# lab-oak/oak

Measured on AMD Instinct MI355X. Metric: turn-steps/s (batched playouts), higher is better.
Workload: dtype u16

## Files before the change

### include/oakgpu.h

```cpp
#ifndef OAKGPU_H
#define OAKGPU_H
#include <stddef.h>
#include <stdint.h>

#ifdef __cplusplus
extern "C" {
#endif

#define OAKGPU_BATTLE_SIZE 384
#define OAKGPU_DURATIONS_SIZE 8
#define OAKGPU_ACTIONS_SIZE 16
#define OAKGPU_MAX_CHOICES 9
#define OAKGPU_TEAMS_SIZE 60

typedef struct oakgpu_ctx oakgpu_ctx;
typedef struct oakgpu_net oakgpu_net;

int oakgpu_create(oakgpu_ctx **out, int device);
void oakgpu_destroy(oakgpu_ctx *ctx);
const char *oakgpu_last_error(void);
int oakgpu_set_stream(oakgpu_ctx *ctx, void *hip_stream);
void *oakgpu_get_stream(oakgpu_ctx *ctx);
int oakgpu_synchronize(oakgpu_ctx *ctx);
int oakgpu_set_kernel_timing(oakgpu_ctx *ctx, int on);
int oakgpu_get_leaf_kernel_ms(oakgpu_ctx *ctx, float ms[3]);
int oakgpu_set_playouts_per_lane(oakgpu_ctx *ctx, int k);
int oakgpu_set_regroup(oakgpu_ctx *ctx, int rounds, int suspend_below, int shrink);
int oakgpu_set_tail_pack(oakgpu_ctx *ctx, int below, int waves, int lanes);
int oakgpu_set_queue_order(oakgpu_ctx *ctx, int on);
int oakgpu_set_spread(oakgpu_ctx *ctx, int lanes);
int oakgpu_set_migration(oakgpu_ctx *ctx, int mode, int long_steps, int adopters);
int oakgpu_set_migration_window(oakgpu_ctx *ctx, int window);
int oakgpu_set_standstill_skip(oakgpu_ctx *ctx, int on);
#define OAKGPU_MOVE_CARRY_DEFAULT 32
int oakgpu_set_move_carry(oakgpu_ctx *ctx, int below);
#define OAKGPU_MOVE_CARRY_DRY_DEFAULT 0
int oakgpu_set_move_carry_dry(oakgpu_ctx *ctx, int below);
#define OAKGPU_CTL_FAST_FORWARDED 44
#define OAKGPU_CTL_SKIPPED_STEPS 45
int oakgpu_get_queue_counters(oakgpu_ctx *ctx, uint32_t *out64);
int oakgpu_device_count(void);

int oakgpu_rollout_dev(oakgpu_ctx *ctx, const uint8_t *battles, const uint8_t *durations,
                       const uint8_t *results_in, uint8_t *prng_state, uint32_t n, uint32_t max_steps,
                       int prep, uint8_t *results_out, uint32_t *steps_out, float *values_out,
                       uint8_t *battles_out, uint8_t *durations_out);
int oakgpu_rollout(oakgpu_ctx *ctx, const uint8_t *battles, const uint8_t *durations,
                   const uint8_t *results_in, uint8_t *prng_state, uint32_t n, uint32_t max_steps, int prep,
                   uint8_t *results_out, uint32_t *steps_out, float *values_out, uint8_t *battles_out,
                   uint8_t *durations_out);

typedef struct {
  const uint8_t *battles, *durations, *results_in;
  uint8_t *prng_state;
  uint32_t n;
  uint8_t *results_out;
  uint32_t *steps_out;
  float *values_out;
  uint8_t *battles_out, *durations_out;
} oakgpu_rollout_batch;
int oakgpu_rollout_group_dev(oakgpu_ctx *ctx, const oakgpu_rollout_batch *batches, uint32_t count, uint32_t max_steps,
                             int prep);
int oakgpu_rollout_group(oakgpu_ctx *ctx, const oakgpu_rollout_batch *batches, uint32_t count, uint32_t max_steps, int prep);
int oakgpu_queue_order(oakgpu_ctx *ctx, const oakgpu_rollout_batch *batches, uint32_t count, uint32_t *order_out, uint32_t *suspects_out);

int oakgpu_mt19937_fill(uint32_t seed, uint64_t skip, uint64_t *out, size_t count);
int oakgpu_rollout_draws_dev(oakgpu_ctx *ctx, const uint8_t *battles, uint32_t battle_stride, const uint8_t *durations,
                             uint32_t durations_stride, const uint8_t *results_in, uint32_t results_stride,
                             const uint64_t *draws, uint32_t n_draws, const uint32_t *offsets, uint32_t n,
                             uint32_t max_steps, int prep, uint8_t *results_out, uint32_t *steps_out, float *values_out,
                             uint8_t *battles_out, uint8_t *durations_out, uint32_t *used_out);
int oakgpu_rollout_shared_device(oakgpu_ctx *ctx, const uint8_t *battle, const uint8_t *durations, uint8_t result,
                                 const uint64_t *draws, uint32_t n_draws, uint32_t n, uint32_t max_steps, int prep,
                                 uint8_t *results_out, uint32_t *steps_out, float *values_out, uint8_t *battles_out,
                                 uint8_t *durations_out, uint32_t *offsets_out, uint64_t *draws_consumed);

int oakgpu_update_dev(oakgpu_ctx *ctx, uint8_t *battles, const uint8_t *c1, const uint8_t *c2,
                      uint8_t *durations, uint8_t *actions, const uint8_t *overrides, uint32_t n,
                      uint8_t *results);
int oakgpu_update(oakgpu_ctx *ctx, uint8_t *battles, const uint8_t *c1, const uint8_t *c2, uint8_t *durations,
                  uint8_t *actions, const uint8_t *overrides, uint32_t n, uint8_t *results);

int oakgpu_choices_dev(oakgpu_ctx *ctx, const uint8_t *battles, const uint8_t *results, int player,
                       uint8_t *out, uint8_t *counts, uint32_t n);
int oakgpu_choices(oakgpu_ctx *ctx, const uint8_t *battles, const uint8_t *results, int player, uint8_t *out,
                   uint8_t *counts, uint32_t n);

int oakgpu_poke_engine_eval_dev(oakgpu_ctx *ctx, const uint8_t *battles, uint32_t n, float root_score, float *values,
                                float *scores);
int oakgpu_poke_engine_eval(oakgpu_ctx *ctx, const uint8_t *battles, uint32_t n, float root_score, float *values,
                            float *scores);

int oakgpu_tree_step_dev(oakgpu_ctx *ctx, uint8_t *battles, uint8_t *durations, uint8_t *results, const uint8_t *c1,
                         const uint8_t *c2, uint32_t n, uint32_t rolls, uint8_t *actions, uint8_t *p1_choices,
                         uint8_t *p1_counts, uint8_t *p2_choices, uint8_t *p2_counts);

typedef struct {
  uint64_t iterations;
  uint32_t batch;
  float ucb_c;
  int32_t bandit;
  int32_t eval;
  uint32_t max_depth;
  uint32_t root_rolls;
  uint32_t other_rolls;
  uint64_t seed;
  int32_t matrix_ucb;
  uint32_t mucb_delay;
  uint32_t mucb_minimum;
  float mucb_c;
  float exp3_alpha;
  uint64_t duration_us;
} oakgpu_search_params;
#define OAKGPU_E_ROOT_MISMATCH (-2)
#define OAKGPU_EXP3_ALPHA_DEFAULT (-1.0f)
#define OAKGPU_SEARCH_PARAMS_INIT {0, 0, 0.0f, 0, 0, 0, 3, 1, 0, 0, 0, 0, 0.0f, OAKGPU_EXP3_ALPHA_DEFAULT, 0}
typedef struct {
  uint8_t m, n;
  uint8_t p1_choices[9], p2_choices[9];
  uint64_t visit_matrix[81];
// ... 557 lines not shown
```

### oak_amd/_lib.py

```python
import ctypes as C
import os

_HERE = os.path.dirname(os.path.abspath(__file__))
LIB_PATH = os.environ.get("OAKGPU_LIB") or os.path.join(_HERE, "liboakgpu.so")

SYMBOLS = [
    "oakgpu_create", "oakgpu_destroy", "oakgpu_last_error", "oakgpu_set_stream", "oakgpu_get_stream", "oakgpu_synchronize", "oakgpu_set_kernel_timing", "oakgpu_get_leaf_kernel_ms", "oakgpu_set_playouts_per_lane", "oakgpu_set_regroup", "oakgpu_set_tail_pack", "oakgpu_set_queue_order", "oakgpu_queue_order", "oakgpu_set_spread", "oakgpu_set_migration", "oakgpu_set_migration_window", "oakgpu_set_standstill_skip", "oakgpu_set_move_carry", "oakgpu_set_move_carry_dry", "oakgpu_get_queue_counters",
    "oakgpu_device_count", "oakgpu_rollout_dev", "oakgpu_rollout", "oakgpu_rollout_group_dev", "oakgpu_rollout_group",
    "oakgpu_mt19937_fill", "oakgpu_rollout_draws_dev", "oakgpu_rollout_shared_device", "oakgpu_update_dev", "oakgpu_update",
    "oakgpu_choices_dev", "oakgpu_choices", "oakgpu_init_battles_dev", "oakgpu_init_battles",
    "oakgpu_set_ou_pools", "oakgpu_random_ou_battles_dev",
    "oakgpu_net_load", "oakgpu_net_load_memory", "oakgpu_net_free", "oakgpu_net_shape", "oakgpu_net_set_main_precision", "oakgpu_net_main_precision", "oakgpu_net_policy_form",
    "oakgpu_net_load_discrete", "oakgpu_net_load_discrete_memory", "oakgpu_net_is_discrete", "oakgpu_leaf_eval_discrete_raw_dev",
    "oakgpu_leaf_eval_dev", "oakgpu_leaf_eval", "oakgpu_leaf_eval_cached_dev", "oakgpu_leaf_cache_last_count", "oakgpu_leaf_embed_forms", "oakgpu_leaf_eval_policy_dev", "oakgpu_leaf_eval_policy",
    "oakgpu_heap_create", "oakgpu_heap_destroy", "oakgpu_heap_empty", "oakgpu_heap_clear", "oakgpu_heap_kind", "oakgpu_heap_nodes", "oakgpu_heap_update",
    "oakgpu_heap_root_stats", "oakgpu_heap_child_stats", "oakgpu_search_heap", "oakgpu_search_agent_heap", "oakgpu_heap_check_shards", "oakgpu_heap_selftest",
    "oakgpu_tree_step_dev", "oakgpu_search", "oakgpu_search_many", "oakgpu_search_agent", "oakgpu_agent_networks_clear", "oakgpu_bandit_replay", "oakgpu_bandit_select_run", "oakgpu_solve_matrix",
    "oakgpu_segment_mean_dev", "oakgpu_comm_unique_id", "oakgpu_comm_create", "oakgpu_comm_destroy", "oakgpu_all_gather_dev",
    "oakgpu_root_steps_create", "oakgpu_root_steps_destroy", "oakgpu_root_steps_launch_dev", "oakgpu_root_steps_capacity", "oakgpu_root_steps_reserve",
    "oakgpu_endless_battle_check", "oakgpu_frames_size", "oakgpu_frames_write", "oakgpu_frames_read", "oakgpu_selfplay_game", "oakgpu_selfplay_games", "oakgpu_poke_engine_eval_dev", "oakgpu_poke_engine_eval",
    "oakgpu_replay_index", "oakgpu_replay_records_dev", "oakgpu_replay_records", "oakgpu_engine_switches",
    "oakgpu_corpus_create", "oakgpu_corpus_destroy", "oakgpu_corpus_info", "oakgpu_frames_encode_dev", "oakgpu_frames_sample_dev", "oakgpu_encode_battles_dev",
    "oakgpu_frames_encode", "oakgpu_frames_sample",
    "oakgpu_corpus_frame_bases", "oakgpu_corpus_chunks", "oakgpu_corpus_states_dev", "oakgpu_corpus_states", "oakgpu_corpus_inference_dev", "oakgpu_corpus_loss_dev",
    "oakgpu_corpus_inference", "oakgpu_corpus_evaluate",
    "oakgpu_party_table_create", "oakgpu_party_table_destroy", "oakgpu_party_table_fill_dev", "oakgpu_party_table_fill", "oakgpu_leaf_eval_table_dev",
    "oakgpu_leaf_eval_policy_table_dev", "oakgpu_party_table_last_misses", "oakgpu_party_table_rows", "oakgpu_party_table_width", "oakgpu_party_key", "oakgpu_party_variant",
    "oakgpu_set_search_party_table", "oakgpu_search_party_table_stats", "oakgpu_leaf_eval_table", "oakgpu_leaf_eval_policy_table",
    "oakgpu_policy_games_dev", "oakgpu_policy_games", "oakgpu_policy_games_last_stats",
    "oakgpu_forest_create", "oakgpu_forest_destroy", "oakgpu_forest_check", "oakgpu_forest_search_dev", "oakgpu_forest_search", "oakgpu_forest_nodes",
    "oakgpu_forest_last_stats", "oakgpu_search_stream", "oakgpu_agent_params",
    "oakgpu_forest_selfplay_check", "oakgpu_forest_selfplay_dev", "oakgpu_forest_selfplay_records", "oakgpu_forest_selfplay", "oakgpu_forest_selfplay_last_stats",
    "oakgpu_selfplay_pick_host",
    "oakgpu_forest_match_check", "oakgpu_forest_match_dev", "oakgpu_forest_match", "oakgpu_forest_match_last_stats", "oakgpu_match_pick_host",
    "oakgpu_forest_match_set_records", "oakgpu_forest_match_records",
    "oakgpu_forest_create_kept", "oakgpu_forest_create_kept_check", "oakgpu_forest_kept_tree_bytes", "oakgpu_forest_advance_dev", "oakgpu_forest_advance",
    "oakgpu_forest_search_kept_dev", "oakgpu_forest_search_kept", "oakgpu_forest_keep_stats", "oakgpu_forest_mismatch", "oakgpu_forest_node_counts",
    "oakgpu_forest_selfplay_nodes_kept", "oakgpu_forest_selfplay_keep_stats",
    "oakgpu_nash_solve_dev", "oakgpu_solve_matrices", "oakgpu_nash_soft_host", "oakgpu_nash_round_host", "oakgpu_nash_width4_max_entry",
    "oakgpu_forest_selfplay_last_traffic",
    "oakgpu_forest_budgets_check", "oakgpu_forest_search_budgets_dev", "oakgpu_forest_search_budgets", "oakgpu_forest_search_budgets_kept_dev",
    "oakgpu_forest_search_budgets_kept", "oakgpu_forest_last_rows", "oakgpu_forest_selfplay_fast_stats", "oakgpu_forest_selfplay_set_partition",
    "oakgpu_selfplay_prelude_host",
    "oakgpu_frames_symmetries_dev", "oakgpu_trainer_check", "oakgpu_trainer_create", "oakgpu_trainer_destroy", "oakgpu_trainer_shape",
    "oakgpu_trainer_forward_dev", "oakgpu_trainer_gradients_dev", "oakgpu_trainer_adam_dev", "oakgpu_trainer_step_dev", "oakgpu_trainer_report",
    "oakgpu_trainer_read", "oakgpu_trainer_set_gradients", "oakgpu_trainer_net_bytes", "oakgpu_trainer_forward", "oakgpu_trainer_gradients",
    "oakgpu_trainer_step",
    "oakgpu_build_tables", "oakgpu_build_net_check", "oakgpu_build_net_load", "oakgpu_build_net_destroy", "oakgpu_build_net_shape", "oakgpu_build_teams_check",
    "oakgpu_build_provide_check", "oakgpu_build_rollout_dev", "oakgpu_build_provide_dev", "oakgpu_build_records_dev", "oakgpu_build_rollout",
    "oakgpu_build_provide", "oakgpu_build_records",
    "oakgpu_build_traj_check", "oakgpu_build_corpus_create", "oakgpu_build_corpus_destroy", "oakgpu_build_corpus_scan_dev", "oakgpu_build_corpus_info",
    "oakgpu_build_traj_dev", "oakgpu_build_traj_sample_dev", "oakgpu_build_targets_dev", "oakgpu_build_state_dense_dev", "oakgpu_build_traj",
    "oakgpu_build_traj_sample", "oakgpu_build_targets", "oakgpu_build_state_dense",
    "oakgpu_build_trainer_check", "oakgpu_build_trainer_create", "oakgpu_build_trainer_destroy", "oakgpu_build_trainer_shape", "oakgpu_build_trainer_forward_dev",
    "oakgpu_build_trainer_accumulate_dev", "oakgpu_build_trainer_zero_gradients_dev", "oakgpu_build_trainer_adam_dev", "oakgpu_build_trainer_average_dev",
    "oakgpu_build_trainer_report", "oakgpu_build_trainer_read", "oakgpu_build_trainer_set_gradients", "oakgpu_build_trainer_net_bytes",
]


def nash_mode(solve_nash):
    if isinstance(solve_nash, str):
        if solve_nash not in ("host", "device"):
            raise ValueError("solve_nash: True / False, \"host\", \"device\" or 0 / 1 / 2")
        return 2 if solve_nash == "device" else 1
    return 2 if (not isinstance(solve_nash, bool) and solve_nash == 2) else int(bool(solve_nash))


class RolloutBatch(C.Structure):
    _fields_ = [("battles", C.c_void_p), ("durations", C.c_void_p), ("results_in", C.c_void_p), ("prng_state", C.c_void_p),
                ("n", C.c_uint32), ("results_out", C.c_void_p), ("steps_out", C.c_void_p), ("values_out", C.c_void_p),
                ("battles_out", C.c_void_p), ("durations_out", C.c_void_p)]


class SearchParams(C.Structure):
    _fields_ = [("iterations", C.c_uint64), ("batch", C.c_uint32), ("ucb_c", C.c_float), ("bandit", C.c_int32),
                ("eval", C.c_int32), ("max_depth", C.c_uint32), ("root_rolls", C.c_uint32), ("other_rolls", C.c_uint32),
                ("seed", C.c_uint64), ("matrix_ucb", C.c_int32), ("mucb_delay", C.c_uint32), ("mucb_minimum", C.c_uint32),
                ("mucb_c", C.c_float), ("exp3_alpha", C.c_float), ("duration_us", C.c_uint64)]


class Agent(C.Structure):
    _fields_ = [("budget", C.c_char_p), ("bandit", C.c_char_p), ("eval", C.c_char_p), ("matrix_ucb", C.c_char_p),
                ("discrete", C.c_int), ("table", C.c_int)]


class SearchOutput(C.Structure):
    _fields_ = [("m", C.c_uint8), ("n", C.c_uint8), ("p1_choices", C.c_uint8 * 9), ("p2_choices", C.c_uint8 * 9),
                ("visit_matrix", C.c_uint64 * 81), ("value_matrix", C.c_double * 81), ("iterations", C.c_uint64),
                ("empirical_value", C.c_double), ("initial_value", C.c_double), ("p1_empirical", C.c_double * 9),
                ("p2_empirical", C.c_double * 9), ("nodes", C.c_uint64), ("total_depth", C.c_uint64),
# ... 100 lines not shown
    _fields_ = [("p1", Seat), ("p2", Seat), ("max_turns", C.c_uint32), ("poll", C.c_uint32), ("compact_below", C.c_float),
                ("log_turns", C.c_uint32)]


class MatchSeat(C.Structure):
    _fields_ = [("search", SearchParams), ("net", C.c_void_p), ("policy_mode", C.c_char * 16), ("policy_temp", C.c_double), ("policy_min", C.c_double)]


class ForestMatchParams(C.Structure):
    _fields_ = [("p1", MatchSeat), ("p2", MatchSeat), ("max_turns", C.c_uint32), ("early_stop", C.c_double), ("log_turns", C.c_uint32),
                ("solve_nash", C.c_int32)]


class MatchTurn(C.Structure):
    _fields_ = [("c1", C.c_uint8), ("c2", C.c_uint8), ("m", C.c_uint8), ("n", C.c_uint8), ("zero", C.c_uint32), ("ev_p1", C.c_double),
                ("ev_p2", C.c_double)]


class ForestOutputs(C.Structure):
    _fields_ = [(name, C.c_void_p) for name in ("m", "n", "p1_choices", "p2_choices", "visit_matrix", "value_matrix", "iterations", "nodes",
                                                "total_depth", "initial_value", "p1_logit", "p2_logit", "p1_prior", "p2_prior", "stream")]


class ForestBandit(C.Structure):
    _fields_ = [("scores", C.c_float * 9), ("priors", C.c_float * 9), ("visits", C.c_uint32 * 9), ("k", C.c_uint8), ("pad", C.c_uint8 * 3)]


class ForestNode(C.Structure):
    _fields_ = [("p1", ForestBandit), ("p2", ForestBandit)]


class ForestTraceHead(C.Structure):
    _fields_ = [("levels", C.c_uint32), ("leaf", C.c_uint32), ("initialised", C.c_uint8), ("result_type", C.c_uint8), ("pad", C.c_uint8 * 2),
                ("value", C.c_float), ("logits", C.c_float * 18)]


class ForestTraceLevel(C.Structure):
    _fields_ = [("node", C.c_uint32), ("i", C.c_uint8), ("j", C.c_uint8), ("pad", C.c_uint8 * 2)]


PKMN_SYMBOLS = [
    "pkmn_gen1_battle_update", "pkmn_gen1_battle_choices", "pkmn_gen1_battle_options_set",
    "pkmn_gen1_battle_options_chance_actions", "pkmn_gen1_battle_options_chance_durations",
    "pkmn_result_type", "pkmn_result_p1", "pkmn_result_p2",
]

_lib = None


class OakGpuError(RuntimeError):
    pass


def load():
    global _lib
    if _lib is not None:
        return _lib
    if not os.path.exists(LIB_PATH):
        raise OakGpuError("liboakgpu.so not built: run `python -c 'import __graft_entry__ as g; g.build()'` "
                          "(hipcc --offload-arch=gfx950); there is no CPU fallback")
    lib = C.CDLL(LIB_PATH)
    vp, u32, u64, i32 = C.c_void_p, C.c_uint32, C.c_uint64, C.c_int
    lib.oakgpu_create.argtypes = [C.POINTER(vp), i32]
    lib.oakgpu_destroy.argtypes = [vp]
    lib.oakgpu_destroy.restype = None
    lib.oakgpu_last_error.restype = C.c_char_p
    lib.oakgpu_set_stream.argtypes = [vp, vp]
    lib.oakgpu_get_stream.argtypes = [vp]
    lib.oakgpu_get_stream.restype = vp
    lib.oakgpu_synchronize.argtypes = [vp]
    lib.oakgpu_set_kernel_timing.argtypes = [vp, i32]
    lib.oakgpu_get_leaf_kernel_ms.argtypes = [vp, C.POINTER(C.c_float)]
    lib.oakgpu_set_playouts_per_lane.argtypes = [vp, i32]
    lib.oakgpu_set_regroup.argtypes = [vp, i32, i32, i32]
    lib.oakgpu_set_tail_pack.argtypes = [vp, i32, i32, i32]
    lib.oakgpu_set_queue_order.argtypes = [vp, i32]
    lib.oakgpu_queue_order.argtypes = [vp, C.POINTER(RolloutBatch), u32, vp, C.POINTER(u32)]
    lib.oakgpu_set_spread.argtypes = [vp, i32]
    lib.oakgpu_set_migration.argtypes = [vp, i32, i32, i32]
    lib.oakgpu_set_migration_window.argtypes = [vp, i32]
    lib.oakgpu_set_standstill_skip.argtypes = [vp, i32]
    lib.oakgpu_set_move_carry.argtypes = [vp, i32]
    lib.oakgpu_set_move_carry_dry.argtypes = [vp, i32]
    lib.oakgpu_get_queue_counters.argtypes = [vp, vp]
    lib.oakgpu_rollout_dev.argtypes = [vp, vp, vp, vp, vp, u32, u32, i32, vp, vp, vp, vp, vp]
    lib.oakgpu_rollout.argtypes = [vp, vp, vp, vp, vp, u32, u32, i32, vp, vp, vp, vp, vp]
    lib.oakgpu_rollout_group_dev.argtypes = [vp, C.POINTER(RolloutBatch), u32, u32, i32]
    lib.oakgpu_rollout_group.argtypes = [vp, C.POINTER(RolloutBatch), u32, u32, i32]
    lib.oakgpu_mt19937_fill.argtypes = [u32, u64, vp, C.c_size_t]
    lib.oakgpu_rollout_draws_dev.argtypes = [vp, vp, u32, vp, u32, vp, u32, vp, u32, vp, u32, u32, i32, vp, vp, vp, vp, vp, vp]
    lib.oakgpu_rollout_shared_device.argtypes = [vp, vp, vp, C.c_uint8, vp, u32, u32, u32, i32, vp, vp, vp, vp, vp, vp, vp]
    lib.oakgpu_poke_engine_eval_dev.argtypes = [vp, vp, u32, C.c_float, vp, vp]
    lib.oakgpu_poke_engine_eval.argtypes = [vp, vp, u32, C.c_float, vp, vp]
    lib.oakgpu_tree_step_dev.argtypes = [vp, vp, vp, vp, vp, vp, u32, u32, vp, vp, vp, vp, vp]
    lib.oakgpu_search.argtypes = [vp, vp, vp, vp, C.c_uint8, C.POINTER(SearchParams), C.POINTER(SearchOutput)]
    lib.oakgpu_heap_create.argtypes = [C.POINTER(vp)]
    lib.oakgpu_heap_destroy.argtypes = [vp]
    lib.oakgpu_heap_destroy.restype = None
    lib.oakgpu_heap_empty.argtypes = [vp]
    lib.oakgpu_heap_clear.argtypes = [vp]
    lib.oakgpu_heap_clear.restype = None
    lib.oakgpu_heap_kind.argtypes = [vp]
    lib.oakgpu_heap_nodes.argtypes = [vp]
    lib.oakgpu_heap_nodes.restype = u64
    lib.oakgpu_heap_update.argtypes = [vp, C.c_uint8, C.c_uint8, vp]
    lib.oakgpu_heap_root_stats.argtypes = [vp, i32, vp, vp, vp, vp]
    lib.oakgpu_heap_check_shards.argtypes = [vp]
    lib.oakgpu_heap_check_shards.restype = u64
    lib.oakgpu_heap_selftest.argtypes = [u32, u32, u64, i32, C.POINTER(u64 * 4)]
    lib.oakgpu_heap_child_stats.argtypes = [vp, C.c_uint8, C.c_uint8, vp, i32, vp, vp, vp, vp]
    lib.oakgpu_search_heap.argtypes = [vp, vp, vp, vp, vp, C.c_uint8, C.POINTER(SearchParams), C.POINTER(SearchOutput), C.POINTER(SearchOutput)]
    lib.oakgpu_search_many.argtypes = [C.POINTER(vp), vp, C.POINTER(vp), vp, vp, vp, C.POINTER(SearchParams), u32, i32, C.POINTER(SearchOutput)]
    lib.oakgpu_search_agent_heap.argtypes = [vp, vp, vp, vp, C.c_uint8, C.POINTER(Agent), u32, u64, C.POINTER(SearchOutput), C.POINTER(SearchOutput)]
    lib.oakgpu_segment_mean_dev.argtypes = [vp, vp, u32, u32, vp]
    lib.oakgpu_root_steps_create.argtypes = [vp, u32, u32, u32, u32, C.POINTER(vp)]
    lib.oakgpu_root_steps_destroy.argtypes = [vp]
    lib.oakgpu_root_steps_destroy.restype = None
    lib.oakgpu_root_steps_launch_dev.argtypes = [vp, vp, vp, vp, vp, C.c_int, vp]
    lib.oakgpu_root_steps_capacity.argtypes = [vp, C.POINTER(u32)]
    lib.oakgpu_root_steps_reserve.argtypes = [vp, u64]
    lib.oakgpu_comm_unique_id.argtypes = [vp]
    lib.oakgpu_comm_create.argtypes = [vp, vp, i32, i32, C.POINTER(vp)]
    lib.oakgpu_comm_destroy.argtypes = [vp]
    lib.oakgpu_comm_destroy.restype = None
    lib.oakgpu_all_gather_dev.argtypes = [vp, vp, vp, vp, C.c_size_t]
    lib.oakgpu_endless_battle_check.argtypes = [vp]
    lib.oakgpu_frames_size.restype = C.c_size_t
    lib.oakgpu_frames_size.argtypes = [C.POINTER(FrameUpdate), u32]
    lib.oakgpu_frames_write.argtypes = [vp, C.c_uint8, C.POINTER(FrameUpdate), u32, vp, C.c_size_t, C.POINTER(C.c_size_t)]
    lib.oakgpu_frames_read.argtypes = [vp, C.c_size_t, vp, C.POINTER(C.c_uint8), C.POINTER(FrameUpdate), u32, C.POINTER(u32), C.POINTER(C.c_size_t)]
    lib.oakgpu_replay_index.argtypes = [vp, C.c_size_t, vp, vp, vp, u32, C.POINTER(u32), C.POINTER(C.c_size_t)]
    lib.oakgpu_replay_records_dev.argtypes = [vp, vp, vp, vp, vp, u32, vp, vp, vp]
    lib.oakgpu_replay_records.argtypes = [vp, vp, C.c_size_t, vp, u32, C.POINTER(u32), C.POINTER(C.c_size_t), vp, vp]
    lib.oakgpu_engine_switches.argtypes = [C.POINTER(C.c_int * 4)]
    lib.oakgpu_corpus_create.argtypes = [vp, vp, C.c_size_t, C.POINTER(vp)]
    lib.oakgpu_corpus_destroy.argtypes = [vp]
    lib.oakgpu_corpus_destroy.restype = None
    lib.oakgpu_corpus_info.argtypes = [vp, C.POINTER(CorpusStats)]
    lib.oakgpu_frames_encode_dev.argtypes = [vp, vp, vp, u32, C.POINTER(EncodedFrames)]
    lib.oakgpu_frames_sample_dev.argtypes = [vp, vp, u32, u64, u32, u32, vp, C.POINTER(EncodedFrames)]
    lib.oakgpu_encode_battles_dev.argtypes = [vp, vp, vp, vp, u32, vp, vp, vp, vp, vp]
    lib.oakgpu_frames_encode.argtypes = [vp, vp, vp, u32, C.POINTER(EncodedFrames), C.POINTER(u32)]
    lib.oakgpu_frames_sample.argtypes = [vp, vp, u32, u64, u32, u32, vp, C.POINTER(EncodedFrames), C.POINTER(u32)]
    lib.oakgpu_corpus_frame_bases.argtypes = [vp, vp]
    lib.oakgpu_corpus_chunks.argtypes = [vp, vp, u32, u32, vp, u32, C.POINTER(u32)]
    lib.oakgpu_corpus_states_dev.argtypes = [vp, vp, u32, u32, u32, vp, vp, vp, vp, vp, vp, vp, vp, vp]
    lib.oakgpu_corpus_states.argtypes = [vp, vp, u32, u32, u32, vp, vp, vp, vp, vp, vp, vp, vp, vp]
    lib.oakgpu_corpus_inference_dev.argtypes = [vp, vp, vp, u32, u32, u32, C.POINTER(CorpusEval)]
    lib.oakgpu_corpus_loss_dev.argtypes = [vp, vp, vp, u32, u32, u32, C.POINTER(LossParams), C.POINTER(CorpusEval), C.POINTER(CorpusTerms)]
    lib.oakgpu_corpus_inference.argtypes = [vp, vp, vp, u32, u32, u32, C.POINTER(CorpusEval)]
    lib.oakgpu_corpus_evaluate.argtypes = [vp, vp, vp, C.POINTER(LossParams), u32, C.POINTER(CorpusLosses), C.POINTER(CorpusLosses)]
    lib.oakgpu_selfplay_game.argtypes = [vp, vp, vp, u64, C.POINTER(SelfplayParams), vp, C.c_size_t, C.POINTER(C.c_size_t), C.POINTER(u32),
                                         C.POINTER(C.c_uint8)]
    lib.oakgpu_selfplay_games.argtypes = [C.POINTER(vp), vp, vp, C.POINTER(u64), C.POINTER(SelfplayParams), u32, i32, vp, C.c_size_t, C.POINTER(C.c_size_t),
                                          C.POINTER(u32), C.POINTER(C.c_uint8)]
    lib.oakgpu_search_agent.argtypes = [vp, vp, vp, C.c_uint8, C.POINTER(Agent), u32, u64, C.POINTER(SearchOutput)]
    lib.oakgpu_agent_networks_clear.argtypes = [vp]
    lib.oakgpu_agent_networks_clear.restype = None
    lib.oakgpu_solve_matrix.argtypes = [vp, i32, i32, i32, vp, vp, vp]
    lib.oakgpu_nash_solve_dev.argtypes = [vp, vp, u32, vp]
    lib.oakgpu_solve_matrices.argtypes = [vp, vp, vp, vp, u32, i32, vp, vp, vp]
    lib.oakgpu_nash_soft_host.argtypes = [vp, vp, vp, u32, i32, vp, vp, vp, vp]
    lib.oakgpu_nash_round_host.argtypes = [vp, vp, vp, u32, vp, vp]
    lib.oakgpu_nash_width4_max_entry.argtypes = []
    lib.oakgpu_bandit_select_run.argtypes = [i32, C.c_float, C.c_float, u32, vp, vp, vp, u32, vp, vp, vp, vp]
    lib.oakgpu_bandit_replay.argtypes = [i32, C.c_float, C.c_float, u32, vp, u32, vp, vp, vp, vp, vp, vp]
# ... 167 lines not shown
```

### oak_amd/csrc/gen1_regs.hpp

```cpp
#pragma once
#include "gen1_device.hpp"

namespace oak {

#ifdef OAKGPU_SITE_PROFILE
static __device__ unsigned long long g_site_prof[32 * 4];
__device__ __forceinline__ unsigned long long *site_lds() {
  __shared__ unsigned long long s_prof[32 * 4];
  return s_prof;
}
__device__ __forceinline__ void site_zero() {
  unsigned long long *p = site_lds();
  for (int i = threadIdx.x; i < 32 * 4; i += blockDim.x) p[i] = 0;
  __syncthreads();
}
__device__ __forceinline__ void site_flush() {
  __syncthreads();
  unsigned long long *p = site_lds();
  for (int i = threadIdx.x; i < 32 * 4; i += blockDim.x) if (p[i]) atomicAdd(&g_site_prof[i], p[i]);
}
__device__ __forceinline__ void site_add(int id, long long dt) {
  const uint64_t ex = __ballot(1);
  const uint32_t lane = __lane_id();
  if ((ex & ((1ull << lane) - 1)) == 0) {
    unsigned long long *p = site_lds();
    __hip_atomic_fetch_add(&p[id * 4 + 0], 1ull, __ATOMIC_RELAXED, __HIP_MEMORY_SCOPE_WORKGROUP);
    __hip_atomic_fetch_add(&p[id * 4 + 1], (unsigned long long)__popcll(ex), __ATOMIC_RELAXED, __HIP_MEMORY_SCOPE_WORKGROUP);
    __hip_atomic_fetch_add(&p[id * 4 + 2], (unsigned long long)dt, __ATOMIC_RELAXED, __HIP_MEMORY_SCOPE_WORKGROUP);
    __hip_atomic_fetch_add(&p[id * 4 + 3], (unsigned long long)dt * __popcll(ex), __ATOMIC_RELAXED, __HIP_MEMORY_SCOPE_WORKGROUP);
  }
}
struct SiteScope {
  int id; long long t0;
  __device__ __forceinline__ SiteScope(int i) : id(i), t0(clock64()) {}
  __device__ __forceinline__ ~SiteScope() { site_add(id, clock64() - t0); }
};
#define OAK_SCOPE(id) SiteScope oak_scope_##id(id)
#define OAK_T0(v) long long v = clock64()
#define OAK_T1(id, v) site_add(id, clock64() - v)
#define OAK_T1K(id, v) site_add(id + prof_k, clock64() - v)
#define OAK_SET_K(eng, k) (eng).prof_k = (int)(k)
#define OAK_PROF_ZERO() site_zero()
#define OAK_PROF_FLUSH() site_flush()
#else
#define OAK_SCOPE(id)
#define OAK_T0(v)
#define OAK_T1(id, v)
#define OAK_T1K(id, v)
#define OAK_SET_K(eng, k)
#define OAK_PROF_ZERO()
#define OAK_PROF_FLUSH()
#endif
enum { PS_REFILL = 0, PS_STEP, PS_LEGAL_DRAW, PS_ORDER, PS_EXEC_MOVE, PS_SWITCH_IN, PS_BEFORE_MOVE, PS_EXEC_SELECTED_PRE,
       PS_RUN_MOVE, PS_GATES_HIT, PS_STATUS_BODIES, PS_DAMAGE, PS_SECONDARY_APPLY, PS_FAINT_RESIDUAL, PS_PUBLISH,
       PS_CALC_DAMAGE, PS_APPLY_HITS, PS_DAMAGE_TAIL, PS_HEAVY, PS_H_CONVERSION, PS_H_HAZE, PS_H_HEAL, PS_H_MIMIC,
       PS_H_POISON, PS_H_SUBSTITUTE, PS_H_TRANSFORM, PS_H_BIDE, PS_H_SLEEP, PS_H_DISABLE, PS_EXEC_MOVE_K0, PS_EXEC_MOVE_K1, PS_COUNT };

struct SideR {
  uint32_t a0, a1, a2;
  uint32_t bo;
  uint32_t vlo, vhi;
  uint32_t m01, m23;
  uint32_t p0, p1, p2, p3, p4, p5;
  uint32_t o0, o1;
  uint32_t dur;
  uint32_t misc;
};

#define OAK_FOR_SIDE_FIELDS(X) X(a0) X(a1) X(a2) X(bo) X(vlo) X(vhi) X(m01) X(m23) X(p0) X(p1) X(p2) X(p3) X(p4) X(p5) X(o0) X(o1) X(dur) X(misc)

__device__ __forceinline__ void swap_sides(SideR &a, SideR &b) {
#define X(f) asm("v_swap_b32 %0, %1" : "+v"(a.f), "+v"(b.f));
  OAK_FOR_SIDE_FIELDS(X)
#undef X
}
__device__ __forceinline__ void cswap_sides(bool c, SideR &a, SideR &b) {
#define X(f) { uint32_t t = c ? b.f : a.f; b.f = c ? a.f : b.f; a.f = t; }
  OAK_FOR_SIDE_FIELDS(X)
#undef X
}
__device__ __forceinline__ void sides_by_player(bool c, const SideR &a, const SideR &b, SideR &p1, SideR &p2) {
#define X(f) p1.f = c ? b.f : a.f; p2.f = c ? a.f : b.f;
  OAK_FOR_SIDE_FIELDS(X)
#undef X
}

template <int STRIDE, bool TRACK_ACTIONS, bool GIN_LDS = false>
struct EngineR {
  lds_u32 *m;
  Tables T;
  SideR S, F;
  uint64_t actS, actF;
#ifdef OAKGPU_SITE_PROFILE
  int prof_k = 0;
#endif
  uint64_t rng;
  uint32_t turn, last_damage;
  uint32_t lm;

  static constexpr int PARTY_WORDS = 24;
  template <bool L, class Dummy = void> struct GinPtr { typedef const uint32_t *type; };
  template <class Dummy> struct GinPtr<true, Dummy> { typedef const lds_u32 *type; };
  typedef typename GinPtr<GIN_LDS>::type gin_t;
  gin_t gin;
  __device__ __forceinline__ uint4 gin4(int off) const {
    typedef uint32_t v4 __attribute__((ext_vector_type(4)));
    if constexpr (GIN_LDS) { const v4 t = *(const OAK_LDS v4 *)(gin + off); return make_uint4(t.x, t.y, t.z, t.w); }
    else return *(const uint4 *)(gin + off);
  }
  __device__ __forceinline__ uint32_t pw(uint32_t side, uint32_t i, int k) const { return m[((side * 6 + i) * 2 + k) * STRIDE]; }
  __device__ __forceinline__ void set_pw(uint32_t side, uint32_t i, int k, uint32_t v) { m[((side * 6 + i) * 2 + k) * STRIDE] = v; }
  __device__ __forceinline__ uint32_t gdw(uint32_t side, uint32_t i, int k) const { return gin[side * 46 + i * 6 + k]; }
  static __device__ __forceinline__ uint32_t pack_pp(uint32_t d2, uint32_t d3, uint32_t d4) {
    return (d2 >> 24) | (((d3 >> 8) & 0xFF) << 8) | ((d3 >> 24) << 16) | (((d4 >> 8) & 0xFF) << 24);
  }
  static __device__ __forceinline__ uint32_t absp(const SideR &x) { return (x.misc >> 8) & 1; }
  static __device__ __forceinline__ uint32_t hp(const SideR &x) { return x.p4 >> 16; }
  static __device__ __forceinline__ void set_hp(SideR &x, uint32_t v) { x.p4 = (x.p4 & 0xFFFF) | (v << 16); }
  static __device__ __forceinline__ uint32_t maxhp(const SideR &x) { return x.p0 & 0xFFFF; }
  static __device__ __forceinline__ uint32_t status(const SideR &x) { return x.p5 & 0xFF; }
  static __device__ __forceinline__ void set_status(SideR &x, uint32_t v) { x.p5 = (x.p5 & ~0xFFu) | (v & 0xFF); }
  static __device__ __forceinline__ uint32_t level(const SideR &x) { return x.p5 >> 24; }
  static __device__ __forceinline__ uint32_t species_stored(const SideR &x) { return (x.p5 >> 8) & 0xFF; }
  static __device__ __forceinline__ uint32_t types(const SideR &x) { return x.a2 >> 24; }
  static __device__ __forceinline__ uint32_t spe(const SideR &x) { return x.a1 >> 16; }
  static __device__ __forceinline__ uint32_t last_sel(const SideR &x) { return (x.o1 >> 16) & 0xFF; }
  static __device__ __forceinline__ void set_last_sel(SideR &x, uint32_t v) { x.o1 = (x.o1 & ~(0xFFu << 16)) | ((v & 0xFF) << 16); }
  static __device__ __forceinline__ uint32_t last_used(const SideR &x) { return x.o1 >> 24; }
  static __device__ __forceinline__ void set_last_used(SideR &x, uint32_t v) { x.o1 = (x.o1 & 0x00FFFFFFu) | (v << 24); }
  static __device__ __forceinline__ uint32_t order0(const SideR &x) { return x.o0 & 0xFF; }
  static __device__ __forceinline__ uint64_t amoves(const SideR &x) { return (uint64_t)x.m01 | ((uint64_t)x.m23 << 32); }
  static __device__ __forceinline__ void set_amoves(SideR &x, uint64_t v) { x.m01 = (uint32_t)v; x.m23 = (uint32_t)(v >> 32); }
  static __device__ __forceinline__ uint32_t active_move(const SideR &x, uint32_t slot) {
    return (uint32_t)(amoves(x) >> (16 * (slot - 1))) & 0xFFFF;
  }
  static __device__ __forceinline__ uint64_t smoves(const SideR &x) {
    return (uint64_t)(x.p2 >> 16) | ((uint64_t)x.p3 << 16) | ((uint64_t)(x.p4 & 0xFFFF) << 48);
  }
  static __device__ __forceinline__ void set_smoves(SideR &x, uint64_t v) {
    x.p2 = (x.p2 & 0xFFFF) | ((uint32_t)(v & 0xFFFF) << 16);
    x.p3 = (uint32_t)(v >> 16);
    x.p4 = (x.p4 & 0xFFFF0000u) | (uint32_t)(v >> 48);
  }
  static __device__ __forceinline__ uint32_t astat(const SideR &x, int idx) {
    return idx == 0 ? x.a0 >> 16 : idx == 1 ? x.a1 & 0xFFFF : idx == 2 ? x.a1 >> 16 : x.a2 & 0xFFFF;
  }
  static __device__ __forceinline__ void set_astat(SideR &x, int idx, uint32_t v) {
    if (idx == 0) x.a0 = (x.a0 & 0xFFFF) | (v << 16);
    else if (idx == 1) x.a1 = (x.a1 & 0xFFFF0000u) | v;
    else if (idx == 2) x.a1 = (x.a1 & 0xFFFF) | (v << 16);
    else x.a2 = (x.a2 & 0xFFFF0000u) | v;
  }
  static __device__ __forceinline__ uint32_t conf_left(const SideR &x) { return (x.vlo >> 18) & 7; }
  static __device__ __forceinline__ void set_conf_left(SideR &x, uint32_t v) { x.vlo = (x.vlo & ~(7u << 18)) | ((v & 7) << 18); }
  static __device__ __forceinline__ uint32_t attacks(const SideR &x) { return (x.vlo >> 21) & 7; }
  static __device__ __forceinline__ void set_attacks(SideR &x, uint32_t v) { x.vlo = (x.vlo & ~(7u << 21)) | ((v & 7) << 21); }
  static __device__ __forceinline__ uint32_t vstate(const SideR &x) { return (x.vlo >> 24) | ((x.vhi & 0xFF) << 8); }
  static __device__ __forceinline__ void set_vstate(SideR &x, uint32_t v) {
    x.vlo = (x.vlo & 0x00FFFFFFu) | ((v & 0xFF) << 24);
    x.vhi = (x.vhi & ~0xFFu) | ((v >> 8) & 0xFF);
  }
  static __device__ __forceinline__ uint32_t sub_hp(const SideR &x) { return (x.vhi >> 8) & 0xFF; }
  static __device__ __forceinline__ void set_sub_hp(SideR &x, uint32_t v) { x.vhi = (x.vhi & ~(0xFFu << 8)) | ((v & 0xFF) << 8); }
  static __device__ __forceinline__ uint32_t transform_id(const SideR &x) { return (x.vhi >> 16) & 15; }
  static __device__ __forceinline__ void set_transform_id(SideR &x, uint32_t v) { x.vhi = (x.vhi & ~(15u << 16)) | ((v & 15) << 16); }
  static __device__ __forceinline__ uint32_t disable_left(const SideR &x) { return (x.vhi >> 20) & 15; }
  static __device__ __forceinline__ void set_disable_left(SideR &x, uint32_t v) { x.vhi = (x.vhi & ~(15u << 20)) | ((v & 15) << 20); }
  static __device__ __forceinline__ uint32_t disable_move(const SideR &x) { return (x.vhi >> 24) & 7; }
  static __device__ __forceinline__ void set_disable_move(SideR &x, uint32_t v) { x.vhi = (x.vhi & ~(7u << 24)) | ((v & 7) << 24); }
  static __device__ __forceinline__ uint32_t toxic_ctr(const SideR &x) { return x.vhi >> 27; }
  static __device__ __forceinline__ void set_toxic_ctr(SideR &x, uint32_t v) { x.vhi = (x.vhi & ~(31u << 27)) | ((v & 31) << 27); }
  static __device__ __forceinline__ int boost_get(const SideR &x, int idx) {
    uint32_t n = (x.bo >> (4 * idx)) & 15;
    return (int)((n ^ 8) - 8);
  }
  static __device__ __forceinline__ void boost_put(SideR &x, int idx, int v) {
    x.bo = (x.bo & ~(15u << (4 * idx))) | (((uint32_t)v & 15) << (4 * idx));
  }
  static __device__ __forceinline__ uint32_t dget(const SideR &x, int sh, int bits) { return (x.dur >> sh) & ((1u << bits) - 1); }
  static __device__ __forceinline__ void dset(SideR &x, int sh, int bits, uint32_t v) {
    uint32_t mask = ((1u << bits) - 1) << sh;
    x.dur = (x.dur & ~mask) | ((v << sh) & mask);
  }
  static __device__ __forceinline__ void clear_binding(SideR &x) { x.vlo &= ~V_BINDING; dset(x, 28, 3, 0); }
  static __device__ __forceinline__ void status_modify(uint32_t st, SideR &x) {
    if (st & ST_PAR) { uint32_t s = (x.a1 >> 16) / 4; set_astat(x, 2, s < 1 ? 1 : s); }
    else if (st & ST_BRN) { uint32_t a = (x.a0 >> 16) / 2; set_astat(x, 0, a < 1 ? 1 : a); }
  }

  __device__ __forceinline__ void act_set(bool self, int sh, int bits, uint32_t v) {
    if constexpr (TRACK_ACTIONS) {
      uint64_t mask = ((1ull << bits) - 1) << sh;
      uint64_t &a = self ? actS : actF;
      a = (a & ~mask) | (((uint64_t)v << sh) & mask);
    }
  }
  __device__ __forceinline__ void act_bool(bool self, int sh, bool v) { act_set(self, sh, 2, v ? 2u : 1u); }

  __device__ __forceinline__ uint32_t rng_next() {
    rng = 0x5D588B656C078965ull * rng + 0x0000000000269EC3ull;
    return (uint32_t)(rng >> 32);
  }
  __device__ __forceinline__ uint32_t rng_range(uint32_t from, uint32_t to) {
    return from + __umulhi(rng_next(), to - from);
  }
  __device__ __forceinline__ bool rng_chance(uint32_t num) { return (rng_next() >> 24) < num; }

  __device__ __forceinline__ Move move_data(uint32_t id) const { return Move{T.mv[id]}; }
  __device__ __forceinline__ uint32_t chart(uint32_t atk_type, uint32_t def_type) const { return T.chart[atk_type * 15 + def_type]; }
  static __device__ __forceinline__ bool has_type(uint32_t ty, uint32_t t) { return (ty & 15) == t || (ty >> 4) == t; }
  __device__ __forceinline__ uint32_t fast_div24(uint32_t x, uint32_t d) const { return d == 1 ? x : __umulhi(x, T.rcp[d]); }
  __device__ __forceinline__ uint32_t fast_mod(uint32_t x, uint32_t n) const {
    return n == 1 ? 0 : mod_rcp(x, n, T.rcp[n]);
  }
  static __device__ __forceinline__ uint32_t mod_rcp(uint32_t x, uint32_t n, uint32_t rc) {
    const uint32_t r = x - __umulhi(x, rc) * n;
    return r < r + n ? r : r + n;
  }
  __device__ __forceinline__ uint32_t scale_boost(uint32_t x, int stage) const { return __umulhi(x << 3, T.boost[stage + 6]); }

  __device__ __forceinline__ uint32_t unmodified_stat(const SideR &x, int idx) {
    if (!(x.vlo & V_TRANSFORM))
      return idx == 0 ? x.p0 >> 16 : idx == 1 ? x.p1 & 0xFFFF : idx == 2 ? x.p1 >> 16 : x.p2 & 0xFFFF;
    const uint32_t id = transform_id(x), sd = id >> 3, pi = (id & 7) - 1;
    const uint32_t d = gdw(sd, pi, idx == 0 ? 0 : idx == 3 ? 2 : 1);
    return (idx == 0 || idx == 2) ? d >> 16 : d & 0xFFFF;
  }

  __device__ __forceinline__ void writeback_stored(const SideR &x) {
    const uint32_t sd = absp(x), pi = order0(x) - 1;
    set_pw(sd, pi, 0, pack_pp(x.p2, x.p3, x.p4));
    set_pw(sd, pi, 1, (x.p4 >> 16) | ((x.p5 & 0xFF) << 16));
  }
  __device__ __forceinline__ void alive_from_lds(SideR &x) {
    const uint32_t sd = absp(x);
    uint32_t hpmask = 0;
#pragma unroll
    for (int i = 0; i < 6; ++i) hpmask |= ((pw(sd, i, 1) & 0xFFFF) != 0 ? 1u : 0u) << i;
    const uint64_t ord = (uint64_t)x.o0 | ((uint64_t)(x.o1 & 0xFFFF) << 32);
    uint32_t alive = 0;
#pragma unroll
    for (int k = 0; k < 6; ++k) {
      const uint32_t id = (uint32_t)(ord >> (8 * k)) & 0xFF;
      alive |= (id != 0 ? (hpmask >> ((id - 1) & 7)) & 1u : 0u) << k;
    }
    x.misc = (x.misc & ~63u) | alive;
  }
  __device__ __forceinline__ void load_stored(SideR &x) {
    const uint32_t id = order0(x);
    const uint32_t keep = id != 0 ? 0xFFFFFFFFu : 0u;
    const uint32_t sd = absp(x), pi = (id != 0 ? id : 1u) - 1;
    const uint32_t pp = pw(sd, pi, 0), hs = pw(sd, pi, 1);
    x.p0 = gdw(sd, pi, 0) & keep;
    x.p1 = gdw(sd, pi, 1) & keep;
    x.p2 = ((gdw(sd, pi, 2) & 0x00FFFFFFu) | ((pp & 0xFF) << 24)) & keep;
    x.p3 = ((gdw(sd, pi, 3) & 0x00FF00FFu) | (((pp >> 8) & 0xFF) << 8) | (((pp >> 16) & 0xFF) << 24)) & keep;
    x.p4 = ((gdw(sd, pi, 4) & 0x000000FFu) | ((pp >> 24) << 8) | ((hs & 0xFFFF) << 16)) & keep;
    x.p5 = ((gdw(sd, pi, 5) & 0xFFFFFF00u) | ((hs >> 16) & 0xFF)) & keep;
  }
  __device__ __forceinline__ void load_battle_global(const uint8_t *battle384, uint32_t dur0, uint32_t dur1) {
    gin = (gin_t)battle384;
#pragma unroll
    for (uint32_t sd = 0; sd < 2; ++sd)
#pragma unroll
      for (uint32_t i = 0; i < 6; ++i) {
        const uint32_t d2 = gdw(sd, i, 2), d3 = gdw(sd, i, 3), d4 = gdw(sd, i, 4), d5 = gdw(sd, i, 5);
        set_pw(sd, i, 0, pack_pp(d2, d3, d4));
        set_pw(sd, i, 1, (d4 >> 16) | ((d5 & 0xFF) << 16));
      }
    { const uint4 v = gin4(36); S.a0 = v.x; S.a1 = v.y; S.a2 = v.z; S.bo = v.w; }
    { const uint4 v = gin4(40); S.vlo = v.x; S.vhi = v.y; S.m01 = v.z; S.m23 = v.w; }
    S.o0 = gin[44]; S.o1 = gin[45];
    F.a0 = gin[82]; F.a1 = gin[83];
    { const uint4 v = gin4(84); F.a2 = v.x; F.bo = v.y; F.vlo = v.z; F.vhi = v.w; }
    { const uint4 v = gin4(88); F.m01 = v.x; F.m23 = v.y; F.o0 = v.z; F.o1 = v.w; }
    { const uint4 v = gin4(92); turn = v.x & 0xFFFF; last_damage = v.x >> 16; lm = v.y; rng = (uint64_t)v.z | ((uint64_t)v.w << 32); }
    S.dur = dur0; F.dur = dur1;
    S.misc = 0; F.misc = 1u << 8;
    actS = actF = 0;
    alive_from_lds(S);
    alive_from_lds(F);
    load_stored(S);
    load_stored(F);
  }
  __device__ __forceinline__ void store_battle_global(uint8_t *battle384) { store_battle_global(battle384, S, F); }
  __device__ __forceinline__ void store_battle_global(uint8_t *battle384, const SideR &S, const SideR &F) {
    if (order0(S) != 0) writeback_stored(S);
    if (order0(F) != 0) writeback_stored(F);
    uint32_t *g = (uint32_t *)battle384;
#pragma unroll
    for (uint32_t sd = 0; sd < 2; ++sd)
#pragma unroll
      for (uint32_t i = 0; i < 6; ++i) {
        const uint32_t pp = pw(sd, i, 0), hs = pw(sd, i, 1);
        uint32_t *d = g + sd * 46 + i * 6;
        d[0] = gdw(sd, i, 0);
        d[1] = gdw(sd, i, 1);
        d[2] = (gdw(sd, i, 2) & 0x00FFFFFFu) | ((pp & 0xFF) << 24);
        d[3] = (gdw(sd, i, 3) & 0x00FF00FFu) | (((pp >> 8) & 0xFF) << 8) | (((pp >> 16) & 0xFF) << 24);
        d[4] = (gdw(sd, i, 4) & 0x000000FFu) | ((pp >> 24) << 8) | ((hs & 0xFFFF) << 16);
        d[5] = (gdw(sd, i, 5) & 0xFFFFFF00u) | ((hs >> 16) & 0xFF);
      }
    *(uint4 *)(g + 36) = make_uint4(S.a0, S.a1, S.a2, S.bo);
    *(uint4 *)(g + 40) = make_uint4(S.vlo, S.vhi, S.m01, S.m23);
    g[44] = S.o0; g[45] = S.o1;
    g[82] = F.a0; g[83] = F.a1;
    *(uint4 *)(g + 84) = make_uint4(F.a2, F.bo, F.vlo, F.vhi);
    *(uint4 *)(g + 88) = make_uint4(F.m01, F.m23, F.o0, F.o1);
    *(uint4 *)(g + 92) = make_uint4(turn | (last_damage << 16), lm, (uint32_t)rng, (uint32_t)(rng >> 32));
  }
  __device__ __forceinline__ void randomize_hidden_side(SideR &x) {
    const uint32_t hi = (uint32_t)(rng >> 32), lo = (uint32_t)rng;
    auto mod = [&](uint32_t mm) { uint32_t two32 = (0xFFFFFFFFu % mm + 1) % mm; return ((hi % mm) * two32 + (lo % mm)) % mm; };
    const uint32_t d = x.dur;
    const uint32_t confusion = (d >> 18) & 7, disable = (d >> 21) & 15, attacking = (d >> 25) & 7, binding = (d >> 28) & 7;
    if (confusion) {
      const uint32_t one = confusion == 1;
      set_conf_left(x, (mod((6 - (confusion + one)) & 0xFF) + 1 + one) & 0xFF);
    }
    if (disable) set_disable_left(x, (mod((9 - disable) & 0xFF) + 1) & 0xFF);
    if (attacking && (x.vlo & (V_BIDE | V_THRASHING))) set_attacks(x, attacking == 3 ? 1u : 4u - (attacking + mod(2)));
    if (binding) {
      const uint32_t idx = mod(40);
      uint32_t a;
      if (binding == 1) a = idx < 15 ? 1 : idx < 30 ? 2 : idx < 36 ? 3 : 4;
      else if (binding == 2) a = idx < 24 ? 1 : idx < 32 ? 2 : 3;
      else if (binding == 3) a = idx < 20 ? 1 : 2;
      else a = 1;
      set_attacks(x, a);
    }
    const uint64_t ord = (uint64_t)x.o0 | ((uint64_t)(x.o1 & 0xFFFF) << 32);
    for (int i = 0; i < 6; ++i) {
      const uint32_t sleep = (d >> (3 * i)) & 7;
      if (!sleep) continue;
      const uint32_t draw = (mod((8 - sleep) & 0xFF) + 1) & 0xFF;
      if (i == 0) {
        const uint32_t st = status(x);
        if ((st & 7) && !(st & 0x80)) set_status(x, (st & 0xF8) | draw);
      } else {
        const uint32_t id = (uint32_t)(ord >> (8 * i)) & 0xFF;
        const uint32_t hs = pw(absp(x), id - 1, 1), st = (hs >> 16) & 0xFF;
        if ((st & 7) && !(st & 0x80)) set_pw(absp(x), id - 1, 1, (hs & 0xFFFF) | (((st & 0xF8) | draw) << 16));
      }
    }
  }
  __device__ __forceinline__ void randomize_hidden() { randomize_hidden_side(S); randomize_hidden_side(F); }
  __device__ __forceinline__ uint32_t lm_index(uint32_t ap) const { return (lm >> (16 * ap)) & 0xFF; }
  __device__ __forceinline__ void set_lm_index(uint32_t ap, uint32_t v) { lm = (lm & ~(0xFFu << (16 * ap))) | ((v & 0xFF) << (16 * ap)); }
  __device__ __forceinline__ uint32_t lm_counterable(uint32_t ap) const { return (lm >> (16 * ap + 8)) & 0xFF; }
  __device__ __forceinline__ void set_lm_counterable(uint32_t ap, uint32_t v) { lm = (lm & ~(0xFFu << (16 * ap + 8))) | ((v & 0xFF) << (16 * ap + 8)); }

  __device__ __forceinline__ void switch_in(SideR &x, SideR &y, uint32_t slot) {
    if (order0(x) != 0) {
      if (status(x) == ST_TOX) set_status(x, ST_PSN);
      writeback_stored(x);
    }
    uint64_t o = (uint64_t)x.o0 | ((uint64_t)(x.o1 & 0xFFFF) << 32);
    const uint32_t sh = 8 * (slot - 1);
    const uint64_t b0 = o & 0xFF, bk = (o >> sh) & 0xFF;
    o = (o & ~(0xFFull << sh)) | (b0 << sh);
    o = (o & ~0xFFull) | bk;
    x.o0 = (uint32_t)o;
    x.o1 = (x.o1 & 0xFFFF0000u) | (uint32_t)(o >> 32);
    const uint32_t al = x.misc & 63, a0b = al & 1, akb = (al >> (slot - 1)) & 1;
    uint32_t nal = (al & ~(1u | (1u << (slot - 1)))) | akb | (a0b << (slot - 1));
    if (slot == 1) nal = al;
    x.misc = (x.misc & ~63u) | nal;
    uint32_t d = x.dur;
    const uint32_t s0 = d & 7, sk = (d >> (3 * (slot - 1))) & 7;
    d = (d & ~7u) | sk;
    if (slot != 1) d = (d & ~(7u << (3 * (slot - 1)))) | (s0 << (3 * (slot - 1)));
    x.dur = d & ((1u << 18) - 1);
    set_last_used(x, 0);
    set_last_used(y, 0);
    load_stored(x);
    x.a0 = x.p0;
    x.a1 = x.p1;
    x.a2 = (x.p2 & 0xFFFF) | (((x.p5 >> 8) & 0xFF) << 16) | (((x.p5 >> 16) & 0xFF) << 24);
    x.bo = 0;
    x.vlo = 0;
    x.vhi = 0;
    x.m01 = (x.p2 >> 16) | (x.p3 << 16);
    x.m23 = (x.p3 >> 16) | (x.p4 << 16);
    status_modify(x.p5 & 0xFF, x);
    clear_binding(y);
  }

  __device__ __forceinline__ void select_move(SideR &x, uint32_t choice) {
    if ((choice & 3) == C_PASS) return;
    if (x.vlo & (V_RECHARGING | V_RAGE)) return;
    x.vlo &= ~V_FLINCH;
    if (x.vlo & (V_THRASHING | V_CHARGING)) return;
    if ((choice & 3) == C_SWITCH) return;
    if (x.vlo & (V_BIDE | V_BINDING)) return;
    const uint32_t data = choice >> 2;
    set_last_sel(x, data == 0 ? (uint32_t)M_Struggle : active_move(x, data) & 0xFF);
    set_lm_index(absp(x), data);
  }

  __device__ __forceinline__ bool check_crit(Move mv) {
    uint32_t chance = (T.sp0[species_stored(S)] >> 24) / 2;
    if (S.vlo & V_FOCUSENERGY) chance = chance / 2;
    else { chance *= 2; if (chance > 255) chance = 255; }
    if (mv.effect() == E_HighCritical) { chance *= 4; if (chance > 255) chance = 255; }
    else chance = chance / 2;
    bool crit = rng_chance(chance);
    act_bool(true, AC_CRIT, crit);
    return crit;
  }

  __device__ __forceinline__ bool calc_damage(const SideR &tgt, uint32_t bp, uint32_t type, bool explode, bool crit) {
    const bool special = type >= 8;
    uint32_t atk, def;
    if (crit) {
      atk = unmodified_stat(S, special ? 3 : 0);
      def = unmodified_stat(tgt, special ? 3 : 1);
    } else {
      atk = special ? S.a2 & 0xFFFF : S.a0 >> 16;
      def = (special ? tgt.a2 & 0xFFFF : tgt.a1 & 0xFFFF) * ((tgt.vlo & (special ? V_LIGHTSCREEN : V_REFLECT)) ? 2u : 1u);
    }
    if (atk > 255 || def > 255) {
      atk = (atk / 4) & 255; if (atk < 1) atk = 1;
      def = (def / 4) & 255; if (def < 1) def = 1;
    }
    uint32_t lvl = level(S) * (crit ? 2u : 1u);
    if (explode) { def = def / 2; if (def < 1) def = 1; }
    if (def == 0) return false;
    uint32_t d = (lvl * 2 / 5) + 2;
    d *= bp;
    d *= atk;
    d = fast_div24(d, def);
    d /= 50;
    if (d > 997) d = 997;
    d += 2;
    last_damage = d;
    return true;
  }

  __device__ __forceinline__ void adjust_damage(Move mv) {
    const uint32_t ft = types(F), t1 = ft & 15, t2 = ft >> 4;
    uint32_t d = last_damage;
    if (has_type(types(S), mv.type())) d = (d + d / 2) & 0xFFFF;
    const uint32_t e1 = chart(mv.type(), t1), e2 = chart(mv.type(), t2);
    if (e1 != 2) d = (d * e1 / 2) & 0xFFFF;
    if (t1 != t2 && e2 != 2) d = (d * e2 / 2) & 0xFFFF;
    last_damage = d;
  }

  __device__ __forceinline__ void randomize_damage() {
    if (last_damage <= 1) return;
    uint32_t roll = (S.misc >> 16) & 0xFF;
    if (roll == 0) roll = rng_range(217, 256);
    act_set(true, AC_DAMAGE, 8, roll);
    last_damage = last_damage * roll / 255;
  }
// ... 724 lines not shown
  }
  __device__ __forceinline__ void hand_over(uint32_t &pc, uint32_t &qc) {
    next_actor();
    const uint32_t t = pc; pc = qc; qc = t;
  }
  __device__ __forceinline__ uint32_t turn_finish(uint32_t r) { return r ? r : turn_epilogue(); }

  __device__ uint32_t update_frame(uint32_t cS, uint32_t cF) {
    uint32_t pc = 0, qc = 0;
    uint32_t r = turn_prologue(cS, cF, pc, qc);
    if (r) return r;
#pragma unroll 1
    for (int k = 0; k < 2; ++k) {
      OAK_SET_K(*this, k);
      r = act(pc);
      const bool last = r != 0 || (qc & 3) == C_PASS;
      hand_over(pc, qc);
      if (last) break;
    }
    return turn_finish(r);
  }
  __device__ __forceinline__ uint32_t update(uint32_t c1, uint32_t c2) {
    const uint32_t r = update_frame(c1, c2);
    normalize();
    return r;
  }

  struct Legal { uint32_t n, sw, mv, forced; };
  __device__ __forceinline__ Legal legal(const SideR &x, uint32_t request) const {
    const uint32_t sw = (x.misc >> 1) & 31;
    if (request == C_PASS) return Legal{1, 0, 0, 0};
    if (request == C_SWITCH) {
      const uint32_t n = (uint32_t)__popc(sw);
      return n ? Legal{n, sw, 0, 0} : Legal{1, 0, 0, 0};
    }
    if (x.vlo & (V_RECHARGING | V_RAGE | V_THRASHING | V_CHARGING)) return Legal{1, 0, 0, C_MOVE};
    const uint64_t am = amoves(x);
    if (x.vlo & (V_BIDE | V_BINDING)) {
      const uint32_t sel = last_sel(x);
      uint32_t forced = C_MOVE;
#pragma unroll
      for (int i = 3; i >= 0; --i) {
        const uint32_t id = (uint32_t)(am >> (16 * i)) & 0xFF;
        if (id != 0 && id == sel) forced = ((uint32_t)(i + 1) << 2) | C_MOVE;
      }
      return Legal{1, 0, 0, forced};
    }
    const uint32_t dm = disable_move(x);
    uint32_t mv = 0;
    bool open = true;
#pragma unroll
    for (uint32_t i = 0; i < 4; ++i) {
      const uint32_t ms = (uint32_t)(am >> (16 * i)) & 0xFFFF;
      open = open && (ms & 0xFF) != 0;
      mv |= (open && (ms >> 8) != 0 && dm != i + 1 ? 1u : 0u) << i;
    }
    const uint32_t nm = (uint32_t)__popc(mv);
    return Legal{(uint32_t)__popc(sw) + (nm ? nm : 1u), sw, mv, C_MOVE};
  }
  __device__ __forceinline__ uint32_t nth_choice(const Legal &L, uint32_t r) const {
    static_assert(C_MOVE == 1 && C_SWITCH == 2, "the choice bytes below");
    const uint32_t nsw = (uint32_t)__popc(L.sw);
    const uint32_t list = (uint32_t)T.bits[L.sw] | ((uint32_t)T.bits[L.mv] << (3 * nsw));
    const uint32_t c = (((list >> (3 * r)) & 7) << 2) + (r < nsw ? 10u : 5u);
    return (r >= nsw && L.mv == 0) ? L.forced : c;
  }
  __device__ __forceinline__ uint32_t draw_p2(uint32_t hi, uint32_t n) const { return fast_mod(hi, n); }
  __device__ __forceinline__ uint32_t draw_p1(uint32_t hi, uint32_t lo, uint32_t n) const {
    constexpr uint32_t TWO32 = (1u << 9) | (1u << 15) | (4u << 18) | (4u << 21) | (4u << 27);
    const uint32_t rc = T.rcp[n];
    const uint32_t t = mod_rcp(hi, n, rc) * ((TWO32 >> (3 * n)) & 7) + mod_rcp(lo, n, rc);
    return n == 1 ? 0 : t - __umulhi(t, rc) * n;
  }
  __device__ __forceinline__ bool inert_side(const SideR &x, const SideR &y, uint32_t &sel, bool &sel_forced, bool &par) const {
    constexpr uint32_t locked = V_RECHARGING | V_RAGE | V_THRASHING | V_CHARGING | V_BIDE;
    const uint32_t st = status(x);
    const Legal L = legal(x, C_MOVE);
    const bool struggle = !(x.vlo & (locked | V_BINDING)) && L.sw == 0 && L.mv == 0;
    sel = struggle ? (uint32_t)M_Struggle : last_sel(x);
    sel_forced = struggle || (x.vlo & locked) != 0;
    par = false;
    if (st == ST_FRZ) return (x.misc & 63) == 1 || (x.vlo & locked) != 0;
    constexpr uint32_t busy = V_FLINCH | V_RECHARGING | V_CONFUSION | V_BIDE | V_THRASHING | V_CHARGING | V_INVULNERABLE | V_MULTIHIT | V_BINDING;
    if ((st != 0 && st != ST_PAR) || !(struggle || (x.vlo & V_RAGE)) || (x.vlo & busy) != 0 || disable_left(x) != 0 || disable_move(x) != 0 ||
        dget(x, 25, 3) != 0 || dget(x, 28, 3) != 0) return false;
    const Move mv = move_data(sel);
    const uint32_t eff = mv.effect(), ft = types(y);
    const bool plain = mv.bp() != 0 && sel != M_Counter && eff != E_SpecialDamage && eff != E_SuperFang && eff != E_OHKO && eff != E_Charge &&
                       eff != E_Metronome && eff != E_MirrorMove && eff != E_Thrashing && eff != E_Explode && eff != E_JumpKick;
    const bool type_immune = chart(mv.type(), ft & 15) == 0 || chart(mv.type(), ft >> 4) == 0;
    par = st == ST_PAR;
    return plain && type_immune && last_used(x) == sel && lm_counterable(absp(x)) == 0 && (!par || last_damage == 0);
  }
  __device__ __forceinline__ int inert_standstill(uint32_t result) const {
    if (!(result == mk_result(0, C_MOVE, C_MOVE) && turn >= 1 && turn < 1000 && (S.misc & 1) && (F.misc & 1) && hp(S) > 0 && hp(F) > 0 &&
          ((S.vlo | F.vlo) & (V_BINDING | V_LEECHSEED)) == 0)) return -1;
    uint32_t mS, mF;
    bool fS, fF, pS, pF;
    if (!inert_side(S, F, mS, fS, pS) || !inert_side(F, S, mF, fF, pF)) return -1;
    bool tie = false;
    if (spe(S) == spe(F)) {
      if (!(fS && fF)) return -1;
      tie = (mS == M_QuickAttack) == (mF == M_QuickAttack) && (mS == M_Counter) == (mF == M_Counter);
    }
    return (int)tie + (int)pS + (int)pF;
  }
  __device__ __forceinline__ void rng_jump(uint32_t n) {
    uint64_t accA = 1, accC = 0, curA = 0x5D588B656C078965ull, curC = 0x0000000000269EC3ull;
    for (; n; n >>= 1) {
      if (n & 1) { accA *= curA; accC = accC * curA + curC; }
      curC *= curA + 1;
      curA *= curA;
    }
    rng = accA * rng + accC;
  }
  __device__ __forceinline__ void random_choices(uint32_t result, uint32_t hi, uint32_t lo, uint32_t &cS, uint32_t &cF) const {
    const bool s_p1 = absp(S) == 0;
    const uint32_t req1 = (result >> 4) & 3, req2 = (result >> 6) & 3;
    const Legal LS = legal(S, s_p1 ? req1 : req2), LF = legal(F, s_p1 ? req2 : req1);
    const uint32_t r1 = draw_p1(hi, lo, s_p1 ? LS.n : LF.n), r2 = draw_p2(hi, s_p1 ? LF.n : LS.n);
    cS = nth_choice(LS, s_p1 ? r1 : r2);
    cF = nth_choice(LF, s_p1 ? r2 : r1);
  }
  __device__ __forceinline__ uint32_t random_step(uint32_t result, uint32_t hi, uint32_t lo) {
    OAK_SCOPE(PS_STEP);
    OAK_T0(t_ld);
    uint32_t cS, cF;
    random_choices(result, hi, lo, cS, cF);
    OAK_T1(PS_LEGAL_DRAW, t_ld);
    return update_frame(cS, cF);
  }

  struct Choices { uint32_t n; uint64_t lo; uint32_t hi;
    __device__ __forceinline__ void push(uint32_t c) {
      lo |= n < 8 ? (uint64_t)c << (8 * n) : 0ull;
      hi |= n >= 8 ? c : 0u;
      ++n;
    }
    __device__ __forceinline__ uint32_t get(uint32_t i) const {
      const uint32_t a = (uint32_t)(lo >> (8 * (i & 7))) & 0xFF;
      return i < 8 ? a : hi;
    }
  };
  __device__ __forceinline__ Choices choices(const SideR &x, uint32_t request) const {
    Choices c{0, 0, 0};
    if (request == C_PASS) { c.push(0); return c; }
    const uint32_t alive = x.misc & 63;
    if (request == C_SWITCH) {
#pragma unroll
      for (uint32_t slot = 2; slot <= 6; ++slot)
        if ((alive >> (slot - 1)) & 1) c.push((slot << 2) | C_SWITCH);
      if (c.n == 0) c.push(0);
      return c;
    }
    if (x.vlo & (V_RECHARGING | V_RAGE | V_THRASHING | V_CHARGING)) { c.push(C_MOVE); return c; }
    if (x.vlo & (V_BIDE | V_BINDING)) {
      const uint32_t sel = last_sel(x);
#pragma unroll
      for (uint32_t i = 1; i <= 4; ++i) {
        const uint32_t ms = active_move(x, i);
        if ((ms & 0xFF) && (ms & 0xFF) == sel) { c.push((i << 2) | C_MOVE); return c; }
      }
      c.push(C_MOVE);
      return c;
    }
#pragma unroll
    for (uint32_t slot = 2; slot <= 6; ++slot)
      if ((alive >> (slot - 1)) & 1) c.push((slot << 2) | C_SWITCH);
// ... 15 lines not shown
```

### oak_amd/csrc/oakgpu.hip

```cpp
#include <hip/hip_runtime.h>
#include <stdint.h>
#include <stdio.h>
#include <stdlib.h>
#include <string.h>
#include <algorithm>
#include <random>
#include <mutex>
#include <string>
#include <type_traits>
#include <vector>

#include "../../include/oakgpu.h"
#include "gen1_device.hpp"
#include "gen1_regs.hpp"
#include "record_walk.hpp"
#include "oakgpu_internal.h"
#include "fast_prng.hpp"

namespace oak {
using namespace walk;

constexpr int STATE_WORDS = 96;
constexpr int TABLE_LDS_PAD = TABLE_PAD;

// ... 304 lines not shown
__device__ __forceinline__ const BatchDesc *find_batch(const lds_u32 *cold, uint32_t idx) {
  const uint32_t count = cold[(offsetof(ColdArgs, g) + offsetof(GroupArgs, count)) / 4];
  const lds_u32 *starts = cold + offsetof(ColdArgs, starts) / 4;
  uint32_t lo = 0, hi = count;
  while (hi - lo > 1) {
    const uint32_t mid = (lo + hi) >> 1;
    if (starts[mid] <= idx) lo = mid; else hi = mid;
  }
  return cold_ptr<const BatchDesc *>(cold, offsetof(ColdArgs, g) + offsetof(GroupArgs, table)) + lo;
}

#ifdef OAKGPU_TIMELINE
static __device__ unsigned long long g_timeline[5 * 16384];
#define OAK_TL(slot, v) do { const unsigned long long tl_v = (v); if (wl == 0 && blockIdx.x < 16384) g_timeline[5 * blockIdx.x + (slot)] = tl_v; } while (0)
#else
#define OAK_TL(slot, v)
#endif

constexpr uint32_t QUEUE_MAX_ROUNDS = 16;
__device__ __forceinline__ void clear_launch_words(uint32_t *ctl, uint32_t *heads, uint32_t keep, uint32_t tid, uint32_t threads) {
  for (uint32_t i = tid; i < 63; i += threads) if ((i & ~1u) != keep) ctl[i] = 0;
  for (uint32_t i = tid; i < QUEUE_MAX_ROUNDS * QUEUE_HEADS; i += threads) heads[i * QUEUE_HEAD_STRIDE] = 0;
}
__global__ __launch_bounds__(256) void k_clear_launch_words(uint32_t *ctl, uint32_t *heads) { clear_launch_words(ctl, heads, 64, threadIdx.x, 256); }

constexpr uint32_t ORDER_BLOCK = 256, ORDER_PER_BLOCK = 1024;
__global__ __launch_bounds__(ORDER_BLOCK) void k_queue_order(GroupArgs g, uint32_t *order, uint32_t *ctl, uint32_t *heads, uint32_t pair) {
  constexpr uint32_t PER = ORDER_PER_BLOCK / ORDER_BLOCK, GROUPS = ORDER_PER_BLOCK / 64;
  __shared__ uint32_t starts[MAX_GROUP + 1];
  __shared__ uint32_t wave_s[GROUPS], wave_o[GROUPS], base_s, base_o;
  if (blockIdx.x == 0) clear_launch_words(ctl, heads, pair, threadIdx.x, ORDER_BLOCK);
  for (uint32_t i = threadIdx.x; i < g.count; i += ORDER_BLOCK) starts[i] = g.table[i].start;
  if (threadIdx.x == 0) starts[g.count] = 0xFFFFFFFFu;
  __syncthreads();
  const uint32_t wl = threadIdx.x & 63, wib = threadIdx.x >> 6;
  uint64_t ms[PER], mo[PER];
#pragma unroll
  for (uint32_t j = 0; j < PER; ++j) {
    const uint32_t idx = blockIdx.x * ORDER_PER_BLOCK + j * ORDER_BLOCK + threadIdx.x;
    bool suspect = false;
    if (idx < g.total) {
      uint32_t lo = 0, hi = g.count;
      while (hi - lo > 1) { const uint32_t mid = (lo + hi) >> 1; if (starts[mid] <= idx) lo = mid; else hi = mid; }
      const BatchDesc &bd = g.table[lo];
      const uint32_t *b = (const uint32_t *)(bd.battles + (size_t)(idx - bd.start) * 384);
      uint32_t w[12];
#pragma unroll
      for (int k = 0; k < 12; ++k) w[k] = b[((k / 6) * SIDE_SZ + (k % 6) * PK_SZ + P_STATUS) / 4];
#pragma unroll
      for (int k = 0; k < 12; ++k) {
        const uint32_t sp = (w[k] >> 8) & 0xFF, ty = (w[k] >> 16) & 0xFF;
        suspect |= sp != 0 && ((ty & 15) == T_Ghost || (ty >> 4) == T_Ghost || sp == 132 );
      }
    }
    ms[j] = __ballot(suspect);
    mo[j] = __ballot(idx < g.total && !suspect);
    if (wl == 0) { wave_s[j * (ORDER_BLOCK / 64) + wib] = (uint32_t)__popcll(ms[j]); wave_o[j * (ORDER_BLOCK / 64) + wib] = (uint32_t)__popcll(mo[j]); }
  }
  __syncthreads();
  if (threadIdx.x == 0) {
    uint32_t ts = 0, to = 0;
    for (uint32_t q = 0; q < GROUPS; ++q) { const uint32_t a = wave_s[q], c = wave_o[q]; wave_s[q] = ts; wave_o[q] = to; ts += a; to += c; }
    base_s = ts ? atomicAdd(ctl + pair, ts) : 0;
    base_o = to ? atomicAdd(ctl + pair + 1, to) : 0;
  }
  __syncthreads();
  const uint64_t below = (1ull << wl) - 1;
#pragma unroll
  for (uint32_t j = 0; j < PER; ++j) {
    const uint32_t idx = blockIdx.x * ORDER_PER_BLOCK + j * ORDER_BLOCK + threadIdx.x, grp = j * (ORDER_BLOCK / 64) + wib;
    if ((ms[j] >> wl) & 1) order[base_s + wave_s[grp] + (uint32_t)__popcll(ms[j] & below)] = idx;
    else if ((mo[j] >> wl) & 1) order[g.total - 1 - (base_o + wave_o[grp] + (uint32_t)__popcll(mo[j] & below))] = idx;
  }
}

#ifndef OAK_LONG_STEPS
#define OAK_LONG_STEPS 200
#endif
constexpr uint32_t LONG_STEPS = OAK_LONG_STEPS;
#ifndef OAK_PRIO_STILL
#define OAK_PRIO_STILL 24
#endif
constexpr uint32_t PRIO_STILL = OAK_PRIO_STILL;
template <int BLK, int WPS>
__global__ __launch_bounds__(BLK, WPS) void k_rollout_queue(GroupArgs g_in, RoundArgs q_in) {
  extern __shared__ __align__(16) uint8_t smem[];
  lds_u32 *party = (lds_u32 *)smem;
  using ER = EngineR<BLK, false>;
  Tables T = stage_default_tables((lds_u8 *)smem + ER::PARTY_WORDS * BLK * 4);
  lds_u32 *cold = (lds_u32 *)((lds_u8 *)smem + ER::PARTY_WORDS * BLK * 4 + TABLE_LDS_PAD);
  if (threadIdx.x == 0) {
    struct { GroupArgs g; RoundArgs q; } c{g_in, q_in};
    const uint32_t *src = (const uint32_t *)&c;
#pragma unroll
    for (uint32_t i = 0; i < offsetof(ColdArgs, starts) / 4; ++i) cold[i] = src[i];
  }
  for (uint32_t i = threadIdx.x; i < g_in.count; i += BLK) cold[offsetof(ColdArgs, starts) / 4 + i] = g_in.table[i].start;
  __syncthreads();
  const uint32_t tid = threadIdx.x, wl = tid & 63;
  constexpr uint32_t NONE = 0xFFFFFFFFu, DONE = 0xFFFFFFFEu;
#define COLD_U32(off) ((uint32_t)__builtin_amdgcn_readfirstlane((int)cold[(off) / 4]))
#define COLD_QU(field) COLD_U32(offsetof(ColdArgs, q) + offsetof(RoundArgs, field))
#define COLD_GU(field) COLD_U32(offsetof(ColdArgs, g) + offsetof(GroupArgs, field))
  constexpr uint32_t U_RESUME = 1, U_PREP = 2, U_ADOPTER = 4, U_DRY = 8, U_ADOPTING = 16, U_ANY_PLAYING = 32, U_NO_SKIP = 64, U_CARRIED = 128, U_MIGRATE = 1u << 11;
  uint32_t ust = (COLD_QU(list_in) | COLD_U32(offsetof(ColdArgs, q) + offsetof(RoundArgs, list_in) + 4)) != 0 ? U_RESUME : 0u;
#define IS_RESUME ((ust & U_RESUME) != 0)
#define IS_PREP ((ust & U_PREP) != 0)
  const uint32_t total = IS_RESUME ? (uint32_t)__builtin_amdgcn_readfirstlane((int)*COLD_Q(n_in, const uint32_t *)) : COLD_GU(total);
  const uint32_t max_steps = COLD_GU(max_steps), suspend_below = COLD_QU(suspend_below);
  if (!IS_RESUME && COLD_GU(prep) != 0) ust |= U_PREP;
  ust |= (blockIdx.x & 7u) << 8;
  if (COLD_QU(no_skip) != 0) ust |= U_NO_SKIP;
  if (!IS_RESUME && COLD_QU(lanes) == 0) ust |= (COLD_QU(move_carry) & 0xFFu) << 24;
  ER e;
  e.m = party + tid;
  e.T = T;
  FastPrng g;
  g.s0 = g.s1 = 0;
  uint32_t idx = NONE, result = 0, steps = 0;
  { const uint32_t lanes = COLD_QU(lanes); if (lanes && wl >= lanes) idx = DONE; }
#define IS_DRY ((ust & U_DRY) != 0)
  const uint32_t long_steps = COLD_QU(long_steps);
  uint32_t stale = 0;
  { const uint32_t n_adopt = COLD_QU(n_adopters); if (n_adopt != 0) ust |= blockIdx.x < n_adopt ? U_MIGRATE | U_ADOPTER : U_MIGRATE; }
#define IS_ADOPTER ((ust & U_ADOPTER) != 0)
#define IS_ADOPTING ((ust & U_ADOPTING) != 0)
#define ANY_PLAYING ((ust & U_ANY_PLAYING) != 0)
  uint32_t idle_polls = 0, poll_tick = 15;
  constexpr uint32_t SPIN_CAP = 1u << 22;
  constexpr int ERR_WORD = 23;
  OAK_PROF_ZERO();
  OAK_TL(0, wall_clock64());
#ifdef OAKGPU_TIMELINE
  bool tl_dry = false;
  unsigned long long tl_steps = 0;
#endif
  for (;;) {
    bool need = idx == NONE, load = false, from_scratch = IS_RESUME;
    uint64_t mask = __ballot(need);
    if (mask && IS_ADOPTER && ((++poll_tick & 15u) == 0 || !ANY_PLAYING)) {
      uint32_t *ctl = COLD_Q(adopt_ctl, uint32_t *);
      uint32_t h = 0, k = 0, closed = 0;
      if (wl == 0) {
        for (int tries = 0; tries < 8; ++tries) {
          const uint32_t hh = __hip_atomic_load(ctl + 1, __ATOMIC_ACQUIRE, __HIP_MEMORY_SCOPE_AGENT);
          const uint32_t t = __hip_atomic_load(ctl + 0, __ATOMIC_ACQUIRE, __HIP_MEMORY_SCOPE_AGENT);
          if (t) closed |= 2;
          const uint32_t kk = t > hh ? min(t - hh, (uint32_t)__popcll(mask)) : 0u;
          if (!kk) {
            if (__hip_atomic_load(ctl + 2, __ATOMIC_ACQUIRE, __HIP_MEMORY_SCOPE_AGENT) == gridDim.x - COLD_QU(n_adopters) &&
                __hip_atomic_load(ctl + 0, __ATOMIC_ACQUIRE, __HIP_MEMORY_SCOPE_AGENT) == hh &&
                __hip_atomic_load(ctl + 1, __ATOMIC_ACQUIRE, __HIP_MEMORY_SCOPE_AGENT) == hh) closed |= 1;
            break;
          }
          if (atomicCAS(ctl + 1, hh, hh + kk) == hh) { h = hh; k = kk; break; }
        }
      }
      h = (uint32_t)__builtin_amdgcn_readfirstlane((int)h); k = (uint32_t)__builtin_amdgcn_readfirstlane((int)k); closed = (uint32_t)__builtin_amdgcn_readfirstlane((int)closed);
      if (closed & 2) ust |= U_ADOPTING;
      const uint32_t rank = (uint32_t)__popcll(mask & ((1ull << wl) - 1));
      const bool take = need && rank < k;
      uint32_t got = 0;
      if (take && h + rank < COLD_GU(total)) {
        const uint64_t *slot = COLD_Q(adopt_list, const uint64_t *) + h + rank;
        const uint32_t epoch = COLD_QU(epoch);
        uint32_t spins = 0;
        uint64_t tk;
        while ((uint32_t)((tk = __hip_atomic_load(slot, __ATOMIC_RELAXED, __HIP_MEMORY_SCOPE_AGENT)) >> 32) != epoch && ++spins < SPIN_CAP) __builtin_amdgcn_s_sleep(2);
        if ((uint32_t)(tk >> 32) == epoch) got = (uint32_t)tk;
        if (!got) atomicOr(ctl + ERR_WORD, 1u);
      }
      if (k) __builtin_amdgcn_fence(__ATOMIC_ACQUIRE, "agent");
      if (take && got) { idx = got - 1; load = true; from_scratch = true; }
      need = idx == NONE;
      if ((closed & 1) && need) idx = DONE;
      mask = (IS_ADOPTING || (closed & 1)) ? 0 : __ballot(need);
      need = need && mask != 0;
    }
    if (IS_ADOPTING) { mask = 0; need = false; }
    ust = (ust & ~0xFF0000u) | ((ust + 0x10000u) & 0xFF0000u);
    if (mask && !IS_DRY && (REFILL_EVERY <= 1 || ((ust >> 16) & (REFILL_EVERY - 1)) == 0 || (uint32_t)__popcll(mask) >= REFILL_LANES || !ANY_PLAYING)) {
      OAK_SCOPE(PS_REFILL);
      uint64_t rem = mask;
      bool got = false;
      uint32_t my = 0;
      for (;;) {
        const uint32_t shard = (ust >> 8) & 7u, need_n = (uint32_t)__popcll(rem);
        const uint32_t lim = total > shard ? (total - shard + 7u) >> 3 : 0u;
        uint32_t base = 0;
        if (wl == 0) base = atomicAdd(COLD_Q(queue, uint32_t *) + shard * QUEUE_HEAD_STRIDE, need_n);
        base = (uint32_t)__builtin_amdgcn_readfirstlane((int)base);
        const uint32_t avail = base < lim ? (lim - base < need_n ? lim - base : need_n) : 0u;
        const uint32_t rank = (uint32_t)__popcll(rem & ((1ull << wl) - 1));
        if (((rem >> wl) & 1) && rank < avail) { my = shard + ((base + rank) << 3); got = true; }
        if (avail == need_n) break;
        rem = __ballot(need && !got);
        ust = (ust & ~(7u << 8)) | (((shard + 1u) & 7u) << 8);
        ust += 1u << 12;
        if (((ust >> 12) & 15u) >= 8u) { ust |= U_DRY; break; }
      }
#ifdef OAKGPU_TIMELINE
      if (IS_DRY && !tl_dry) { tl_dry = true; OAK_TL(1, wall_clock64()); }
#endif
      if (need) {
        if (got) {
          const uint32_t *order = COLD_Q(order, const uint32_t *);
          idx = IS_RESUME ? COLD_Q(list_in, const uint32_t *)[my] : order ? order[my] : my;
          load = true;
        } else idx = IS_ADOPTER ? NONE : DONE;
      }
    } else if (mask && IS_DRY && !IS_ADOPTER) {
      if (need) idx = DONE;
    }
    if (__ballot(load)) {
      OAK_SCOPE(PS_REFILL);
      if (load) {
        const BatchDesc *bd = find_batch(cold, idx);
        const uint32_t k = idx - bd->start;
        const uint32_t *dsrc = from_scratch ? COLD_Q(sd, const uint32_t *) + 2 * (size_t)idx : (const uint32_t *)bd->durations + 2 * (size_t)k;
        const uint32_t *psrc = (const uint32_t *)bd->prng + 2 * (size_t)k;
        g.s0 = psrc[0];
        g.s1 = psrc[1];
        e.load_battle_global(from_scratch ? COLD_Q(sb, const uint8_t *) + (size_t)idx * 384 : bd->battles + (size_t)k * 384, dsrc[0], dsrc[1]);
        if (IS_PREP && !from_scratch) {
          const uint32_t hi = g.next32(), lo = g.next32();
          e.rng = ((uint64_t)hi << 32) | lo;
          e.randomize_hidden();
        }
        result = from_scratch ? COLD_Q(sres, const uint8_t *)[idx] : bd->results_in[k];
        steps = from_scratch ? bd->steps_out[k] : 0;
        stale = 0;
      }
    }
    if (__ballot(idx != DONE) == 0) break;
    constexpr uint32_t T_PEND = 0x100u, T_DONE = 0x200u;
    const bool mid = (result & T_PEND) != 0;
    bool playing = idx != DONE && idx != NONE && (result & 15) == 0 && steps < max_steps;
    const bool start = playing && !mid;
#ifdef OAKGPU_TIMELINE
    tl_steps += (unsigned long long)__popcll(__ballot(start));
#endif
    if (start && stale >= (8u << 24) && !(ust & U_NO_SKIP)) {
      const int draws = e.inert_standstill(result);
      const uint32_t by_steps = max_steps - steps, by_turn = 1000u - e.turn;
      const uint32_t skip = (by_steps < by_turn ? by_steps : by_turn) - 1u;
      if (draws >= 0 && skip != 0) {
        for (uint32_t k = 0; k < skip; ++k) { (void)g.next32(); (void)g.next32(); }
        e.rng_jump((uint32_t)draws * skip);
        e.turn += skip;
        steps += skip;
        atomicAdd((unsigned long long *)COLD_Q(stats, uint32_t *), 1ull | ((unsigned long long)skip << 32));
      }
    }
    {
      OAK_SCOPE(PS_STEP);
      if (start) {
        OAK_T0(t_ld);
        const uint32_t hi = g.next32(), lo = g.next32();
        uint32_t cS, cF, pc = 0, qc = 0;
        e.random_choices(result, hi, lo, cS, cF);
        OAK_T1(PS_LEGAL_DRAW, t_ld);
        const uint32_t r = e.turn_prologue(cS, cF, pc, qc);
        result = r ? (r | T_DONE) : (T_PEND | (pc << 16) | (qc << 24));
      }
      if ((ust >> 24) != 0 && !(ust & (U_DRY | U_ADOPTING))) ust |= U_CARRIED; else ust &= ~U_CARRIED;
      if ((ust >> 24) != 0 && IS_DRY && !IS_ADOPTER) {
        const uint32_t dry_below = COLD_QU(move_carry_dry);
        if (dry_below != 0 && (uint32_t)__popcll(__ballot(playing)) >= dry_below) ust |= U_CARRIED;
      }
#define CARRYING ((ust & U_CARRIED) != 0)
#pragma unroll 1
      for (uint32_t walk = CARRYING ? 0u : 1u;; ++walk) {
        const uint32_t c = (result >> 16) & 0xFFu;
        if ((result & T_PEND) && (walk != 0 || (c & 3) != C_MOVE)) {
          OAK_SET_K(e, walk ? walk - 1 : 0);
          const uint32_t r = e.act(c);
          e.next_actor();
          const uint32_t next = T_PEND | ((result >> 8) & 0xFF0000u);
          result = (r != 0 || ((next >> 16) & 3) == C_PASS) ? (r | T_DONE) : next;
        }
        if (walk == 2) break;
        if (walk == 1) {
          const uint32_t want = (uint32_t)__popcll(__ballot((result & T_PEND) != 0));
          if (want == 0 || (CARRYING && want < (ust >> 24))) break;
        }
      }
      if (result & T_DONE) {
        result = e.turn_finish(result & 0xFFu);
        ++steps;
        playing = (result & 15) == 0 && steps < max_steps;
        const uint32_t sg = ((e.S.p4 ^ e.F.p4) >> 16) | (((e.S.o0 + e.F.o0) & 0xFFu) << 16);
        stale = sg != (stale & 0xFFFFFFu) ? sg : stale + (stale < 0xFF000000u ? 0x01000000u : 0u);
      }
    }
    if (IS_ADOPTING || __ballot(playing && (steps > LONG_STEPS || stale >= (PRIO_STILL << 24)))) __builtin_amdgcn_s_setprio(3); else __builtin_amdgcn_s_setprio(0);
    if (__ballot(playing) != 0) ust |= U_ANY_PLAYING; else ust &= ~U_ANY_PLAYING;
    if (IS_ADOPTER && !ANY_PLAYING) {
      __builtin_amdgcn_s_sleep(100);
      if (++idle_polls > SPIN_CAP) { if (wl == 0) atomicOr(COLD_Q(adopt_ctl, uint32_t *) + ERR_WORD, 2u); break; }
    }
    const uint64_t still = __ballot(playing);
    const bool suspend = IS_DRY && !(ust & U_CARRIED) && still != 0 && (uint32_t)__popcll(still) < suspend_below;
    const bool lng = (ust & U_MIGRATE) != 0 && !IS_ADOPTER && playing && !(result & T_PEND) && (steps >= (long_steps & 0xFFFFu) || (stale >> 24) >= (long_steps >> 16));
    if (idx != DONE && idx != NONE && (!playing || suspend || lng)) {
      OAK_SCOPE(PS_PUBLISH);
      const bool fin = !playing;
      SideR P1, P2;
      sides_by_player(ER::absp(e.S) != 0, e.S, e.F, P1, P2);
      const BatchDesc *bd = find_batch(cold, idx);
      const uint32_t k = idx - bd->start;
      if (fin) bd->results_out[k] = (uint8_t)result; else COLD_Q(sres, uint8_t *)[idx] = (uint8_t)result;
      bd->steps_out[k] = steps;
      const uint32_t t = result & 15;
      if (fin) bd->values_out[k] = t == R_WIN ? 1.0f : t == R_LOSE ? 0.0f : 0.5f;
      uint32_t *pdst = (uint32_t *)bd->prng + 2 * (size_t)k;
      pdst[0] = g.s0;
      pdst[1] = g.s1;
      uint32_t *ddst = fin ? (bd->durations_out ? (uint32_t *)bd->durations_out + 2 * (size_t)k : nullptr) : COLD_Q(sd, uint32_t *) + 2 * (size_t)idx;
      if (ddst) {
        ddst[0] = P1.dur;
        ddst[1] = P2.dur;
      }
      uint8_t *bdst = fin ? (bd->battles_out ? bd->battles_out + (size_t)k * 384 : nullptr) : COLD_Q(sb, uint8_t *) + (size_t)idx * 384;
      if (bdst) e.store_battle_global(bdst, P1, P2);
      idx = fin ? NONE : idx;
    }
    const uint64_t dm = __ballot(lng);
    if (dm) {
      __builtin_amdgcn_fence(__ATOMIC_RELEASE, "agent");
      uint32_t *ctl = COLD_Q(adopt_ctl, uint32_t *);
      const uint32_t leader = (uint32_t)__ffsll((unsigned long long)dm) - 1;
      uint32_t base = 0;
      if (wl == leader) base = atomicAdd(ctl + 0, (uint32_t)__popcll(dm));
      base = (uint32_t)__builtin_amdgcn_readlane((int)base, (int)leader);
      if (lng) {
        __hip_atomic_store(COLD_Q(adopt_list, uint64_t *) + base + (uint32_t)__popcll(dm & ((1ull << wl) - 1)), (uint64_t)(idx + 1) | ((uint64_t)COLD_QU(epoch) << 32),
                           __ATOMIC_RELAXED, __HIP_MEMORY_SCOPE_AGENT);
        idx = NONE;
      }
    }
    if (suspend) {
      const uint32_t leader = (uint32_t)__ffsll((unsigned long long)still) - 1;
      uint32_t base = 0;
      if (wl == leader) base = atomicAdd(COLD_Q(count_out, uint32_t *), (uint32_t)__popcll(still));
      base = (uint32_t)__builtin_amdgcn_readlane((int)base, (int)leader);
      if (playing) COLD_Q(list_out, uint32_t *)[base + (uint32_t)__popcll(still & ((1ull << wl) - 1))] = idx;
      break;
    }
  }
  if ((ust & U_MIGRATE) != 0 && !IS_ADOPTER && wl == 0) atomicAdd(COLD_Q(adopt_ctl, uint32_t *) + 2, 1u);
  OAK_TL(2, wall_clock64());
#ifdef OAKGPU_TIMELINE
  OAK_TL(4, tl_steps);
#endif
  OAK_PROF_FLUSH();
}
#undef COLD_Q
#undef COLD_U32
#undef COLD_QU
#undef COLD_GU
#undef IS_RESUME
#undef IS_PREP
#undef IS_DRY
#undef IS_ADOPTER
#undef IS_ADOPTING
#undef ANY_PLAYING
#undef CARRYING

struct RootStepArgs {
  const uint8_t *root_battles, *root_durations, *root_results;
  uint8_t *lane_prng;
  const uint4 *cin_state;
  const uint32_t *cin_count;
  uint4 *cout_state;
  uint32_t *cout_count;
  unsigned long long *acc;
  unsigned long long *turn_steps;
  uint32_t *queue;
  uint32_t *err;
  uint32_t n_fresh, reps, seg, slice_mask, max_steps, fper;
  uint32_t acc_stride, pad;
};
#ifndef OAK_ROOT_REFILL_EVERY
#define OAK_ROOT_REFILL_EVERY 8
#endif
#ifndef OAK_ROOT_REFILL_LANES
#define OAK_ROOT_REFILL_LANES 16
#endif
constexpr uint32_t ROOT_REFILL_EVERY = OAK_ROOT_REFILL_EVERY, ROOT_REFILL_LANES = OAK_ROOT_REFILL_LANES;
constexpr int ROOT_SHARDS = 8;
constexpr int CTL_STRIDE = 64;
constexpr int CARRY_VEC = 18;
constexpr int ROOT_STEP_COLD_BYTES = ((sizeof(RootStepArgs) + 15) & ~15) + ROOT_SHARDS * 4;
constexpr int ROOT_STEP_LDS_BYTES = 24 * 64 * 4 + TABLE_LDS_PAD + ROOT_STEP_COLD_BYTES;
template <int WPS>
__global__ __launch_bounds__(64, WPS) void k_root_step(RootStepArgs a_in) {
  extern __shared__ __align__(16) uint8_t smem[];
  lds_u32 *party = (lds_u32 *)smem;
  using ER = EngineR<64, false>;
  Tables T = stage_default_tables((lds_u8 *)smem + ER::PARTY_WORDS * 64 * 4);
  lds_u32 *cold = (lds_u32 *)((lds_u8 *)smem + ER::PARTY_WORDS * 64 * 4 + TABLE_LDS_PAD);
  if (threadIdx.x == 0) {
    const uint32_t *src = (const uint32_t *)&a_in;
#pragma unroll
    for (uint32_t i = 0; i < sizeof(RootStepArgs) / 4; ++i) cold[i] = src[i];
  }
  lds_u32 *sh_carry = cold + ((sizeof(RootStepArgs) + 15) & ~15) / 4;
  if (threadIdx.x < ROOT_SHARDS) {
    const uint32_t c = a_in.cin_count[threadIdx.x * CTL_STRIDE];
    sh_carry[threadIdx.x] = c < a_in.seg ? c : a_in.seg;
  }
  __syncthreads();
#define RS_PTR(field, type) cold_ptr<type>(cold, offsetof(RootStepArgs, field))
#define RS_U32(field) ((uint32_t)__builtin_amdgcn_readfirstlane((int)cold[offsetof(RootStepArgs, field) / 4]))
  const uint32_t wl = threadIdx.x;
  constexpr uint32_t NONE = 0xFFFFFFFFu, DONE = 0xFFFFFFFEu;
  const uint32_t seg = RS_U32(seg), max_steps = RS_U32(max_steps), slice_mask = RS_U32(slice_mask);
  const uint32_t home = blockIdx.x & (ROOT_SHARDS - 1);
  uint32_t shard = home, exhausted = 0, iter = 0xFFFFFFFFu;
  bool any_playing = false;
  ER e;
  e.m = party + wl;
  e.T = T;
  FastPrng g;
  g.s0 = g.s1 = 0;
  uint32_t root = NONE, result = 0, steps = 0, executed = 0;
  bool dry = false;
  for (;;) {
    bool load = false;
    uint32_t my = 0, my_carry = 0, my_shard = 0;
    const uint64_t mask = __ballot(root == NONE);
    ++iter;
    if (mask && !dry && (ROOT_REFILL_EVERY <= 1 || (iter & (ROOT_REFILL_EVERY - 1)) == 0 || (uint32_t)__popcll(mask) >= ROOT_REFILL_LANES || !any_playing)) {
      uint64_t rem = mask;
      while (rem) {
        const uint32_t need = (uint32_t)__popcll(rem);
        const uint32_t carry_s = (uint32_t)__builtin_amdgcn_readfirstlane((int)sh_carry[shard]);
        const uint32_t n_fresh = RS_U32(n_fresh), fper = RS_U32(fper), flo = shard * fper;
        const uint32_t fresh_s = flo < n_fresh ? (n_fresh - flo < fper ? n_fresh - flo : fper) : 0u;
        const uint32_t tot = carry_s + fresh_s;
        uint32_t base = 0;
        if (wl == 0) base = atomicAdd(RS_PTR(queue, uint32_t *) + shard * CTL_STRIDE, need);
        base = (uint32_t)__builtin_amdgcn_readfirstlane((int)base);
        const uint32_t avail = base < tot ? (tot - base < need ? tot - base : need) : 0u;
        const uint32_t rank = (uint32_t)__popcll(rem & ((1ull << wl) - 1));
        if (((rem >> wl) & 1) && rank < avail) { my = base + rank; my_carry = carry_s; my_shard = shard; load = true; }
        if (avail == need) break;
        rem = __ballot(root == NONE && !load);
        shard = (shard + 1) & (ROOT_SHARDS - 1);
        if (++exhausted >= (uint32_t)ROOT_SHARDS) { dry = true; break; }
      }
    }
    if (dry && root == NONE && !load) root = DONE;
    if (__ballot(load)) {
      if (load && my < my_carry) {
        const uint4 *rec = RS_PTR(cin_state, const uint4 *) + (size_t)CARRY_VEC * ((size_t)my_shard * seg + my);
        uint4 v[CARRY_VEC];
#pragma unroll
        for (int q = 0; q < CARRY_VEC; ++q) v[q] = rec[q];
        auto w = [&](int i) -> uint32_t { const uint4 &q = v[i >> 2]; return (i & 3) == 0 ? q.x : (i & 3) == 1 ? q.y : (i & 3) == 2 ? q.z : q.w; };
        int o = 0;
#define X(f) e.S.f = w(o++);
        OAK_FOR_SIDE_FIELDS(X)
#undef X
#define X(f) e.F.f = w(o++);
        OAK_FOR_SIDE_FIELDS(X)
#undef X
        e.rng = (uint64_t)w(36) | ((uint64_t)w(37) << 32);
        e.turn = w(38) & 0xFFFF; e.last_damage = w(38) >> 16; e.lm = w(39);
#pragma unroll
        for (int q = 0; q < 24; ++q) e.m[q * 64] = w(40 + q);
        g.s0 = w(64); g.s1 = w(65); steps = w(66); root = w(67); result = w(68);
        e.actS = e.actF = 0;
        e.gin = (const uint32_t *)(RS_PTR(root_battles, const uint8_t *) + (size_t)root * 384);
      } else if (load) {
        const uint32_t ln = my_shard * RS_U32(fper) + (my - my_carry);
        root = ln / RS_U32(reps);
        uint32_t *ps = (uint32_t *)RS_PTR(lane_prng, uint8_t *) + 2 * (size_t)ln;
        FastPrng lane;
        lane.s0 = ps[0]; lane.s1 = ps[1];
        const uint32_t hi = lane.next32(), lo = lane.next32();
        ps[0] = lane.s0; ps[1] = lane.s1;
        g.s0 = hi; g.s1 = (hi | lo) ? lo : 1u;
        const uint32_t *dsrc = (const uint32_t *)RS_PTR(root_durations, const uint8_t *) + 2 * (size_t)root;
        e.load_battle_global(RS_PTR(root_battles, const uint8_t *) + (size_t)root * 384, dsrc[0], dsrc[1]);
        const uint32_t bh = g.next32(), bl = g.next32();
        e.rng = ((uint64_t)bh << 32) | bl;
        e.randomize_hidden();
        result = RS_PTR(root_results, const uint8_t *)[root];
        steps = 0;
      }
    }
    if (__ballot(root != DONE) == 0) break;
    bool playing = root < DONE && (result & 15) == 0 && steps < max_steps;
    bool sliced = false;
    executed += (uint32_t)__popcll(__ballot(playing));
    if (playing) {
      const uint32_t hi = g.next32(), lo = g.next32();
      result = e.random_step(result, hi, lo);
      ++steps;
      playing = (result & 15) == 0 && steps < max_steps;
      sliced = playing && (steps & slice_mask) == 0;
    }
    any_playing = __ballot(playing && !sliced) != 0;
    const uint64_t cm = __ballot(sliced);
    uint32_t slot = 0;
    if (cm) {
      const uint32_t leader = (uint32_t)__ffsll((unsigned long long)cm) - 1;
      uint32_t base = 0;
      if (wl == leader) base = atomicAdd(RS_PTR(cout_count, uint32_t *) + home * CTL_STRIDE, (uint32_t)__popcll(cm));
      slot = (uint32_t)__builtin_amdgcn_readlane((int)base, (int)leader) + (uint32_t)__popcll(cm & ((1ull << wl) - 1));
    }
    if (root < DONE && (!playing || sliced)) {
      if (!sliced) {
        const uint32_t t = result & 15;
        const unsigned long long v2 = t == R_WIN ? 2ull : t == R_LOSE ? 0ull : 1ull;
        atomicAdd(RS_PTR(acc, unsigned long long *) + (size_t)home * RS_U32(acc_stride) + root, 1ull | (v2 << 32));
      } else if (slot < seg) {
        uint32_t w[CARRY_VEC * 4];
        int o = 0;
#define X(f) w[o++] = e.S.f;
        OAK_FOR_SIDE_FIELDS(X)
#undef X
#define X(f) w[o++] = e.F.f;
        OAK_FOR_SIDE_FIELDS(X)
#undef X
        w[36] = (uint32_t)e.rng; w[37] = (uint32_t)(e.rng >> 32); w[38] = e.turn | (e.last_damage << 16); w[39] = e.lm;
#pragma unroll
        for (int q = 0; q < 24; ++q) w[40 + q] = e.m[q * 64];
        w[64] = g.s0; w[65] = g.s1; w[66] = steps; w[67] = root; w[68] = result; w[69] = w[70] = w[71] = 0;
        uint4 *rec = RS_PTR(cout_state, uint4 *) + (size_t)CARRY_VEC * ((size_t)home * seg + slot);
#pragma unroll
        for (int q = 0; q < CARRY_VEC; ++q) rec[q] = make_uint4(w[4 * q], w[4 * q + 1], w[4 * q + 2], w[4 * q + 3]);
      } else atomicOr(RS_PTR(err, uint32_t *), 1u);
      root = NONE;
    }
  }
  if (wl == 0 && executed) atomicAdd(RS_PTR(turn_steps, unsigned long long *), (unsigned long long)executed);
#undef RS_PTR
#undef RS_U32
}
__global__ __launch_bounds__(256) void k_root_step_report(const unsigned long long *acc, uint32_t acc_stride, uint32_t n_roots, const uint32_t *cout_count,
                                                          const uint32_t *err, uint32_t seg, unsigned long long *report) {
  const uint32_t r = blockIdx.x * 256 + threadIdx.x;
  if (r < n_roots) {
    unsigned long long a = 0;
#pragma unroll
    for (int s = 0; s < ROOT_SHARDS; ++s) a += acc[(size_t)s * acc_stride + r];
    report[r] = a;
  }
  if (blockIdx.x == 0 && threadIdx.x < 64) {
    uint32_t c = threadIdx.x < ROOT_SHARDS ? cout_count[threadIdx.x * CTL_STRIDE] : 0u;
    if (c > seg) c = seg;
#pragma unroll
    for (int o = 4; o > 0; o >>= 1) c += __shfl_down(c, o);
    if (threadIdx.x == 0) report[n_roots + 1] = (unsigned long long)c | ((unsigned long long)*err << 32);
  }
}

struct BoundaryWave {
  using ER = EngineR<64, true, true>;
  lds_u32 *party, *stage;
  Tables T;
  uint32_t tid, base, lane, cnt;
  __device__ __forceinline__ BoundaryWave(uint8_t *smem, uint32_t n, bool tables = true) {
    party = (lds_u32 *)smem;
    stage = staged_rows(smem);
    T = tables ? stage_default_tables((lds_u8 *)smem + ER::PARTY_WORDS * 64 * 4) : Tables{};
    tid = threadIdx.x, base = blockIdx.x * 64, lane = base + tid;
    cnt = n - base < 64 ? n - base : 64;
  }
  __device__ __forceinline__ uint8_t *row() const { return (uint8_t *)(stage + tid * STAGE_STRIDE); }
  __device__ __forceinline__ ER engine() const { ER e; e.m = party + tid; e.T = T; return e; }
};

template <bool DWORDS>
__global__ __launch_bounds__(64, 2) void k_update(uint8_t *battles, const uint8_t *c1, const uint8_t *c2, uint8_t *durations, uint8_t *actions,
                                                  const uint8_t *overrides, uint32_t n, uint8_t *results) {
  extern __shared__ __align__(16) uint8_t smem[];
  const BoundaryWave w(smem, n);
  const bool live = w.tid < w.cnt;
  uint32_t *d = (uint32_t *)durations + 2 * (size_t)w.lane;
  uint32_t d0 = 0, d1 = 0, pc1 = 0, pc2 = 0, over1 = 0, over2 = 0;
  if (live) {
    d0 = d[0], d1 = d[1], pc1 = c1[w.lane], pc2 = c2[w.lane];
    if (overrides) over1 = overrides[(size_t)w.lane * 16], over2 = overrides[(size_t)w.lane * 16 + 8];
  }
  stage_in<DWORDS>(w.stage, battles, w.base, w.cnt);
  __syncthreads();
  if (live) {
    auto e = w.engine();
    e.load_battle_global(w.row(), d0, d1);
    e.S.misc |= over1 << 16;
    e.F.misc |= over2 << 16;
    results[w.lane] = (uint8_t)e.update(pc1, pc2);
    d[0] = e.S.dur;
    d[1] = e.F.dur;
    if (actions) {
      uint64_t *ad = (uint64_t *)actions + 2 * (size_t)w.lane;
      ad[0] = e.actS;
      ad[1] = e.actF;
    }
    e.store_battle_global(w.row());
  }
  __syncthreads();
  stage_out<DWORDS>(w.stage, battles, w.base, w.cnt);
}

template <bool DWORDS>
// ... 337 lines not shown
  __syncthreads();
  if (w.tid < w.cnt) open_battle(w, mine, (uint32_t)sd, (uint32_t)(sd >> 32), first_update != 0, durations, results);
  __syncthreads();
  stage_out<DWORDS>(w.stage, battles, w.base, w.cnt);
}

template <bool DWORDS>
__global__ __launch_bounds__(64, 2) void k_random_ou(uint64_t seed0, uint32_t n, const uint8_t *legal, int n_legal, const uint8_t *pools,
                                                     const uint8_t *sizes, uint8_t *battles, uint8_t *durations, uint8_t *prng, uint8_t *results) {
  extern __shared__ __align__(16) uint8_t smem[];
  const BoundaryWave w(smem, n);
  __syncthreads();
  if (w.tid < w.cnt) {
    FastPrng g;
    g.seed(seed0 + w.lane);
    uint8_t teams[OAKGPU_TEAMS_SIZE];
    for (int i = 0; i < OAKGPU_TEAMS_SIZE; ++i) teams[i] = 0;
    for (int s = 0; s < 2; ++s)
      for (int k = 0; k < 6; ++k) {
        uint32_t sp;
        for (;;) {
          sp = legal[g.next32() % (uint32_t)n_legal];
          bool dup = false;
          for (int j = 0; j < k; ++j) dup |= teams[(s * 6 + j) * 5] == sp;
          if (!dup) break;
        }
        uint8_t *set = teams + (s * 6 + k) * 5;
        set[0] = (uint8_t)sp;
        const uint32_t psz = sizes[sp];
        const uint32_t want = psz < 4 ? psz : 4;
        for (uint32_t mi = 0; mi < want; ++mi) {
          for (;;) {
            uint32_t mvid = pools[sp * 48 + g.next32() % psz];
            bool dup = false;
            for (uint32_t j = 0; j < mi; ++j) dup |= set[1 + j] == mvid;
            if (!dup) { set[1 + mi] = (uint8_t)mvid; break; }
          }
        }
      }
    const uint32_t hi = g.next32(), lo = g.next32();
    open_battle(w, teams, lo, hi, true, durations, results);
    uint32_t *pd = (uint32_t *)prng + 2 * (size_t)w.lane;
    pd[0] = g.s0;
    pd[1] = g.s1;
  }
  __syncthreads();
  stage_out<DWORDS>(w.stage, battles, w.base, w.cnt);
}

}

struct oakgpu_ctx {
  int device;
  hipStream_t stream;
  bool own_stream;
  uint8_t *d_legal, *d_pools, *d_sizes;
  int n_legal;
  int playouts_per_lane;
  uint32_t *d_queue;
  uint32_t *d_heads;
  int rounds;
  int suspend_below;
  int round_shrink;
  uint8_t *d_scratch;
  size_t scratch_n;
  int rounds_auto;
  int concurrent_hint;
  int search_party_table;
  uint64_t search_table_fills = 0, search_table_evals = 0;
  const void *ws2_owner = nullptr;
  int tail_below;
  int tail_waves;
  int tail_lanes;
  int migrate;
  int migrate_steps;
  int migrate_adopters;
  int migrate_window;
  int migrate_used;
  int spread_lanes;
  int queue_order;
  int standstill_skip;
  int move_carry;
  int move_carry_dry;
  uint32_t *d_order;
  size_t order_n;
  uint32_t order_pair = 0;
  uint32_t ticket_epoch = 0;
  bool tickets_dirty = true;
  int n_cu;
  static constexpr int TABLE_SLOTS = 8;
  void *h_table, *d_table;
  hipEvent_t table_ev[TABLE_SLOTS];
  uint64_t table_next;
  struct Block { void *p; size_t cap; };
  std::vector<Block> stage;
  size_t stage_cursor;
  Block ws[3];
  int timing;
  hipEvent_t tev[4];
  bool tev_valid;
  Block replay_ws{nullptr, 0};
  Block games_ws{nullptr, 0};
  void *attachment = nullptr;
  void (*attachment_dtor)(void *) = nullptr;
};

static thread_local std::string g_err;
static int fail(hipError_t e, const char *what) {
  g_err = std::string(what) + ": " + hipGetErrorString(e);
  return (int)e;
}
static int bad(const char *what) {
  g_err = what;
  return -1;
}
int oakgpu_fail_hip(int e, const char *what) { return fail((hipError_t)e, what); }
int oakgpu_fail_msg(const char *what) { return bad(what); }
int oakgpu_ctx_device(const oakgpu_ctx *c) { return c->device; }
int oakgpu_ctx_enter(oakgpu_ctx *c) {
  hipError_t e = hipSetDevice(c->device);
  return e == hipSuccess ? 0 : fail(e, "hipSetDevice");
}
static void *grow_block(oakgpu_ctx *c, oakgpu_ctx::Block &b, size_t bytes) {
  if (b.cap >= bytes && b.p) return b.p;
  if (b.p) {
    (void)hipStreamSynchronize(c->stream);
    (void)hipFree(b.p);
    b.p = nullptr;
    b.cap = 0;
  }
  const size_t cap = (bytes + (1u << 20) - 1) & ~(size_t)((1u << 20) - 1);
  hipError_t e = hipMalloc(&b.p, cap);
  if (e != hipSuccess) { b.p = nullptr; fail(e, "hipMalloc(context buffer)"); return nullptr; }
  b.cap = cap;
  return b.p;
}
void **oakgpu_ctx_timing_events(oakgpu_ctx *c) { return c->timing && c->tev_valid ? (void **)c->tev : nullptr; }
void *oakgpu_ctx_workspace(oakgpu_ctx *c, int slot, size_t bytes) {
  if (slot % 3 == 2) c->ws2_owner = nullptr;
  return grow_block(c, c->ws[slot % 3], bytes ? bytes : 1);
}
void *oakgpu_ctx_games_workspace(oakgpu_ctx *c, size_t bytes) { return grow_block(c, c->games_ws, bytes ? bytes : 1); }
void oakgpu_ctx_set_ws2_owner(oakgpu_ctx *c, const void *table) { c->ws2_owner = table; }
const void *oakgpu_ctx_ws2_owner(const oakgpu_ctx *c) { return c->ws2_owner; }
void oakgpu_ctx_count_search_table(oakgpu_ctx *c, uint64_t fills, uint64_t evals) { c->search_table_fills += fills; c->search_table_evals += evals; }
void oakgpu_stage_begin(oakgpu_ctx *c) { c->stage_cursor = 0; }
void oakgpu_stage_end(oakgpu_ctx *c) { (void)hipStreamSynchronize(c->stream); }
void *oakgpu_stage_get(oakgpu_ctx *c, size_t bytes) {
  if (c->stage_cursor >= c->stage.size()) c->stage.push_back(oakgpu_ctx::Block{nullptr, 0});
  return grow_block(c, c->stage[c->stage_cursor++], bytes ? bytes : 1);
}
void *oakgpu_ctx_stream(const oakgpu_ctx *c) { return (void *)c->stream; }
int oakgpu_ctx_set_concurrent_hint(oakgpu_ctx *c, int on) { const int old = c->concurrent_hint; c->concurrent_hint = on; return old; }
int oakgpu_ctx_search_party_table(const oakgpu_ctx *c) { return c->search_party_table; }
void *oakgpu_ctx_attachment(const oakgpu_ctx *c) { return c->attachment; }
void oakgpu_ctx_set_attachment(oakgpu_ctx *c, void *p, void (*dtor)(void *)) {
  if (c->attachment && c->attachment_dtor) c->attachment_dtor(c->attachment);
  c->attachment = p;
  c->attachment_dtor = dtor;
}
#undef HIPCHK
#define HIPCHK(x) do { hipError_t _e = (x); if (_e != hipSuccess) return fail(_e, #x); } while (0)

namespace {
struct DevBuf {
  void *p = nullptr;
  size_t bytes = 0;
  hipError_t alloc(size_t b, oakgpu_ctx *c) { bytes = b; p = oakgpu_stage_get(c, b); return p ? hipSuccess : hipErrorOutOfMemory; }
};
}

extern "C" {

const char *oakgpu_last_error(void) { return g_err.c_str(); }

int oakgpu_device_count(void) {
  int n = 0;
  if (hipGetDeviceCount(&n) != hipSuccess) return 0;
  return n;
}

static_assert(24 * 64 * 4 + oak::TABLE_LDS_PAD + oak::COLD_LDS_BYTES <= 160 * 1024 / 16, "k_rollout_queue<64, 4>: sixteen workgroups no longer fit in a CU's LDS");
static int set_lds_limits() {
  HIPCHK(hipFuncSetAttribute((const void *)oak::k_rollout_regs<64>, hipFuncAttributeMaxDynamicSharedMemorySize, 24 * 64 * 4 + oak::TABLE_LDS_PAD));
  HIPCHK(hipFuncSetAttribute((const void *)oak::k_rollout_staged, hipFuncAttributeMaxDynamicSharedMemorySize, oak::STAGED_LDS_BYTES));
  HIPCHK(hipFuncSetAttribute((const void *)oak::k_rollout_draws<64>, hipFuncAttributeMaxDynamicSharedMemorySize, 24 * 64 * 4 + oak::TABLE_LDS_PAD));
  HIPCHK(hipFuncSetAttribute((const void *)oak::k_rollout_queue<64, 4>, hipFuncAttributeMaxDynamicSharedMemorySize, 24 * 64 * 4 + oak::TABLE_LDS_PAD + oak::COLD_LDS_BYTES));
#define STAGED_LIMIT(kernel)                                                                                                           \
  HIPCHK(hipFuncSetAttribute((const void *)oak::kernel<false>, hipFuncAttributeMaxDynamicSharedMemorySize, oak::STAGED_LDS_BYTES)); \
  HIPCHK(hipFuncSetAttribute((const void *)oak::kernel<true>, hipFuncAttributeMaxDynamicSharedMemorySize, oak::STAGED_LDS_BYTES))
  STAGED_LIMIT(k_update);
  STAGED_LIMIT(k_choices);
  STAGED_LIMIT(k_tree_step_staged);
  STAGED_LIMIT(k_init);
  STAGED_LIMIT(k_random_ou);
#undef STAGED_LIMIT
  return 0;
}

#define LAUNCH_STAGED(kernel, battles, n, ...)                                                                                          \
  do {                                                                                                                                  \
    if (((uintptr_t)(battles) & 15) == 0) hipLaunchKernelGGL(oak::kernel<false>, dim3(((n) + 63) / 64), dim3(64), oak::STAGED_LDS_BYTES, c->stream, __VA_ARGS__); \
    else hipLaunchKernelGGL(oak::kernel<true>, dim3(((n) + 63) / 64), dim3(64), oak::STAGED_LDS_BYTES, c->stream, __VA_ARGS__);             \
    HIPCHK(hipGetLastError());                                                                                                          \
  } while (0)

int oakgpu_create(oakgpu_ctx **out, int device) {
  if (!out) return bad("oakgpu_create: null out");
  int n = 0;
  HIPCHK(hipGetDeviceCount(&n));
  if (n <= 0) return bad("oakgpu_create: no HIP device (this library has no CPU fallback)");
  if (device < 0 || device >= n) return bad("oakgpu_create: device index out of range");
  HIPCHK(hipSetDevice(device));
  {
    static std::mutex init_mu;
    static bool init_done[64] = {};
    std::lock_guard<std::mutex> lock(init_mu);
    if (device >= 64 || !init_done[device]) {
      if (int r = set_lds_limits()) return r;
      if (int r = oakgpu_leaf_set_lds_limits()) return r;
      hipStream_t s0;
      HIPCHK(hipStreamCreateWithFlags(&s0, hipStreamNonBlocking));
      hipLaunchKernelGGL(oak::k_build_table_image, dim3(1), dim3(64), oak::TABLE_LDS_PAD, s0);
      hipError_t le = hipGetLastError();
      hipError_t se = hipStreamSynchronize(s0);
      (void)hipStreamDestroy(s0);
      if (le != hipSuccess) return fail(le, "k_build_table_image launch");
      if (se != hipSuccess) return fail(se, "k_build_table_image");
      if (device < 64) init_done[device] = true;
    }
  }
  oakgpu_ctx *c = new oakgpu_ctx();
  c->device = device;
  c->own_stream = true;
  c->d_legal = c->d_pools = c->d_sizes = nullptr;
  c->n_legal = 0;
  c->playouts_per_lane = 2;
  if (const char *env = getenv("OAKGPU_PLAYOUTS_PER_LANE")) c->playouts_per_lane = atoi(env) > 0 ? atoi(env) : 1;
  c->d_queue = nullptr;
  c->d_heads = nullptr;
  c->d_scratch = nullptr;
  c->scratch_n = 0;
  c->h_table = c->d_table = nullptr;
  c->table_next = 0;
  c->stage_cursor = 0;
  c->ws[0] = c->ws[1] = c->ws[2] = oakgpu_ctx::Block{nullptr, 0};
  c->timing = 0;
  c->tev_valid = false;
  c->rounds_auto = 1;
  c->concurrent_hint = 0;
  c->search_party_table = 0;
  if (const char *env = getenv("OAKGPU_PARTY_TABLE")) c->search_party_table = atoi(env) != 0;
  if (const char *env = getenv("OAKGPU_ROUNDS_AUTO")) c->rounds_auto = atoi(env) != 0;
  {
    hipDeviceProp_t prop;
    hipError_t pe = hipGetDeviceProperties(&prop, device);
    if (pe != hipSuccess) { delete c; return fail(pe, "hipGetDeviceProperties"); }
    c->n_cu = prop.multiProcessorCount > 0 ? prop.multiProcessorCount : 256;
  }
  c->rounds = 4;
  c->suspend_below = 32;
  c->round_shrink = 3;
  c->tail_below = 0;
  c->tail_waves = 0;
  if (const char *env = getenv("OAKGPU_TAIL_BELOW")) c->tail_below = atoi(env) < 0 ? 0 : atoi(env) > 64 ? 64 : atoi(env);
  if (const char *env = getenv("OAKGPU_TAIL_WAVES")) c->tail_waves = atoi(env) < 0 ? 0 : atoi(env);
  c->spread_lanes = -1;
  if (const char *env = getenv("OAKGPU_SPREAD_LANES")) c->spread_lanes = atoi(env) < -1 ? -1 : atoi(env) > 64 ? 64 : atoi(env);
  c->queue_order = 1;
  if (const char *env = getenv("OAKGPU_QUEUE_ORDER")) c->queue_order = atoi(env) != 0;
  c->standstill_skip = 1;
  if (const char *env = getenv("OAKGPU_STANDSTILL_SKIP")) c->standstill_skip = atoi(env) != 0;
  c->move_carry = OAKGPU_MOVE_CARRY_DEFAULT;
  if (const char *env = getenv("OAKGPU_MOVE_CARRY")) c->move_carry = atoi(env) < 0 ? 0 : atoi(env) > 64 ? 64 : atoi(env);
  c->move_carry_dry = OAKGPU_MOVE_CARRY_DRY_DEFAULT;
  if (const char *env = getenv("OAKGPU_MOVE_CARRY_DRY")) c->move_carry_dry = atoi(env) < 0 ? 0 : atoi(env) > 64 ? 64 : atoi(env);
  c->migrate = 1;
  c->migrate_steps = 300;
  c->migrate_adopters = 0;
  c->migrate_window = 48;
  c->migrate_used = 0;
  if (const char *env = getenv("OAKGPU_MIGRATE")) c->migrate = atoi(env) < 0 ? 0 : atoi(env) > 2 ? 2 : atoi(env);
  if (const char *env = getenv("OAKGPU_MIGRATE_STEPS")) c->migrate_steps = atoi(env) < 1 ? 1 : atoi(env);
  if (const char *env = getenv("OAKGPU_MIGRATE_ADOPTERS")) c->migrate_adopters = atoi(env) < 0 ? 0 : atoi(env);
  if (const char *env = getenv("OAKGPU_MIGRATE_WINDOW")) c->migrate_window = atoi(env) < 0 ? 0 : atoi(env) > 255 ? 255 : atoi(env);
  c->d_order = nullptr;
  c->order_n = 0;
  c->tail_lanes = 0;
  if (const char *env = getenv("OAKGPU_TAIL_LANES")) c->tail_lanes = atoi(env) < 0 ? 0 : atoi(env) > 64 ? 64 : atoi(env);
  if (const char *env = getenv("OAKGPU_ROUNDS")) c->rounds = atoi(env) < 1 ? 1 : atoi(env) > 8 ? 8 : atoi(env);
  if (const char *env = getenv("OAKGPU_SUSPEND_BELOW")) c->suspend_below = atoi(env) < 0 ? 0 : atoi(env) > 64 ? 64 : atoi(env);
  if (const char *env = getenv("OAKGPU_ROUND_SHRINK")) c->round_shrink = atoi(env) < 1 ? 1 : atoi(env);
  hipError_t e = hipStreamCreateWithFlags(&c->stream, hipStreamNonBlocking);
  if (e != hipSuccess) { delete c; return fail(e, "hipStreamCreate"); }
  *out = c;
  return 0;
}

void oakgpu_destroy(oakgpu_ctx *c) {
  if (!c) return;
  (void)hipSetDevice(c->device);
  (void)hipStreamSynchronize(c->stream);
  if (c->attachment && c->attachment_dtor) { c->attachment_dtor(c->attachment); c->attachment = nullptr; }
  if (c->own_stream) (void)hipStreamDestroy(c->stream);
  if (c->d_legal) (void)hipFree(c->d_legal);
  if (c->d_pools) (void)hipFree(c->d_pools);
  if (c->d_sizes) (void)hipFree(c->d_sizes);
  if (c->d_queue) (void)hipFree(c->d_queue);
  if (c->d_heads) (void)hipFree(c->d_heads);
  if (c->d_scratch) (void)hipFree(c->d_scratch);
  if (c->d_order) (void)hipFree(c->d_order);
  for (auto &b : c->stage) if (b.p) (void)hipFree(b.p);
  for (auto &b : c->ws) if (b.p) (void)hipFree(b.p);
  if (c->replay_ws.p) (void)hipFree(c->replay_ws.p);
  if (c->games_ws.p) (void)hipFree(c->games_ws.p);
  if (c->tev_valid) for (auto &e : c->tev) (void)hipEventDestroy(e);
  if (c->h_table) {
    (void)hipHostFree(c->h_table);
    (void)hipFree(c->d_table);
    for (int i = 0; i < oakgpu_ctx::TABLE_SLOTS; ++i) (void)hipEventDestroy(c->table_ev[i]);
  }
  delete c;
}

int oakgpu_set_stream(oakgpu_ctx *c, void *hip_stream) {
  if (!c) return bad("null ctx");
  if (c->own_stream) { (void)hipStreamSynchronize(c->stream); (void)hipStreamDestroy(c->stream); }
  c->stream = (hipStream_t)hip_stream;
  c->own_stream = false;
  return 0;
}

int oakgpu_set_playouts_per_lane(oakgpu_ctx *c, int k) {
  if (!c || k < 1) return bad("oakgpu_set_playouts_per_lane: bad argument");
  c->playouts_per_lane = k;
  return 0;
}

int oakgpu_set_regroup(oakgpu_ctx *c, int rounds, int suspend_below, int shrink) {
  if (!c || rounds < 1 || rounds > 8 || suspend_below < 0 || suspend_below > 64 || shrink < 1)
    return bad("oakgpu_set_regroup: bad argument");
  c->rounds = rounds;
  c->suspend_below = suspend_below;
  c->round_shrink = shrink;
  c->rounds_auto = 0;
  return 0;
}

int oakgpu_set_migration(oakgpu_ctx *c, int mode, int long_steps, int adopters) {
  if (!c || mode < 0 || mode > 2 || long_steps < 1 || adopters < 0) return bad("oakgpu_set_migration: bad argument");
  c->migrate = mode;
  c->migrate_steps = long_steps;
  c->migrate_adopters = adopters;
  return 0;
}

int oakgpu_set_migration_window(oakgpu_ctx *c, int window) {
  if (!c || window < 0 || window > 255) return bad("oakgpu_set_migration_window: window must be 0 (off) .. 255 turn-steps");
  c->migrate_window = window;
  return 0;
}

int oakgpu_get_queue_counters(oakgpu_ctx *c, uint32_t *out64) {
  if (!c || !out64) return bad("oakgpu_get_queue_counters: null argument");
  if (!c->d_queue) { memset(out64, 0, 256); return 0; }
  HIPCHK(hipSetDevice(c->device));
  HIPCHK(hipMemcpyAsync(out64, c->d_queue, 256, hipMemcpyDeviceToHost, c->stream));
  HIPCHK(hipStreamSynchronize(c->stream));
  return 0;
}

int oakgpu_set_spread(oakgpu_ctx *c, int lanes) {
  if (!c || lanes < -1 || lanes > 64) return bad("oakgpu_set_spread: lanes must be -1 (automatic) or 0..64");
  c->spread_lanes = lanes;
  return 0;
}

int oakgpu_set_standstill_skip(oakgpu_ctx *c, int on) {
  if (!c) return bad("null ctx");
  c->standstill_skip = on != 0;
  return 0;
}

int oakgpu_set_move_carry(oakgpu_ctx *c, int below) {
  if (!c || below < 0 || below > 64) return bad("oakgpu_set_move_carry: below must be 0 (off) .. 64 lanes");
  c->move_carry = below;
  return 0;
}

int oakgpu_set_move_carry_dry(oakgpu_ctx *c, int below) {
  if (!c || below < 0 || below > 64) return bad("oakgpu_set_move_carry_dry: below must be 0 (off) .. 64 lanes");
  c->move_carry_dry = below;
  return 0;
}

int oakgpu_set_search_party_table(oakgpu_ctx *c, int on) {
  if (!c) return bad("null ctx");
  const int old = c->search_party_table;
  c->search_party_table = on != 0;
  return old;
}

int oakgpu_search_party_table_stats(oakgpu_ctx *c, uint64_t *fills, uint64_t *evals) {
  if (!c) return bad("null ctx");
  if (fills) *fills = c->search_table_fills;
  if (evals) *evals = c->search_table_evals;
  return 0;
}

int oakgpu_set_queue_order(oakgpu_ctx *c, int on) {
  if (!c) return bad("null ctx");
  c->queue_order = on != 0;
  return 0;
}

int oakgpu_set_tail_pack(oakgpu_ctx *c, int below, int waves, int lanes) {
  if (!c || below < 0 || below > 64 || waves < 0 || lanes < 0 || lanes > 64) return bad("oakgpu_set_tail_pack: bad argument");
  c->tail_below = below;
  c->tail_waves = waves;
  c->tail_lanes = lanes;
  return 0;
}

void *oakgpu_get_stream(oakgpu_ctx *c) { return c ? (void *)c->stream : nullptr; }

int oakgpu_set_kernel_timing(oakgpu_ctx *c, int on) {
  if (!c) return bad("null ctx");
  HIPCHK(hipSetDevice(c->device));
  if (on && !c->tev_valid) {
    for (auto &e : c->tev) HIPCHK(hipEventCreate(&e));
    c->tev_valid = true;
  }
  c->timing = on != 0;
  return 0;
}

int oakgpu_get_leaf_kernel_ms(oakgpu_ctx *c, float ms[3]) {
  if (!c || !ms) return bad("oakgpu_get_leaf_kernel_ms: null argument");
  if (!c->timing || !c->tev_valid) return bad("oakgpu_get_leaf_kernel_ms: kernel timing is off (oakgpu_set_kernel_timing)");
  HIPCHK(hipEventSynchronize(c->tev[3]));
  for (int i = 0; i < 3; ++i) HIPCHK(hipEventElapsedTime(&ms[i], c->tev[i], c->tev[i + 1]));
  return 0;
}

int oakgpu_synchronize(oakgpu_ctx *c) {
  if (!c) return bad("null ctx");
  HIPCHK(hipStreamSynchronize(c->stream));
  if (c->d_queue && c->migrate_used) {
    uint32_t err = 0;
    HIPCHK(hipMemcpy(&err, c->d_queue + 63, 4, hipMemcpyDeviceToHost));
    c->migrate_used = 0;
    if (err) { HIPCHK(hipMemsetAsync(c->d_queue + 63, 0, 4, c->stream)); HIPCHK(hipStreamSynchronize(c->stream)); }
    if (err) return bad("rollout: a bounded wait of the long-playout migration ran out (playouts were lost) -- oakgpu_set_migration(ctx, 0, ...) turns it off");
  }
  return 0;
}

#ifdef OAKGPU_SITE_PROFILE
extern "C" int oakgpu_site_profile(unsigned long long *out, int reset) {
  if (hipMemcpyFromSymbol(out, HIP_SYMBOL(oak::g_site_prof), sizeof(unsigned long long) * 32 * 4) != hipSuccess) return 1;
  if (reset) {
    unsigned long long z[32 * 4] = {};
    if (hipMemcpyToSymbol(HIP_SYMBOL(oak::g_site_prof), z, sizeof z) != hipSuccess) return 1;
  }
  return 0;
}
#endif

#ifdef OAKGPU_TIMELINE
extern "C" int oakgpu_timeline(unsigned long long *out, int waves) {
  return hipMemcpyFromSymbol(out, HIP_SYMBOL(oak::g_timeline), sizeof(unsigned long long) * 5 * (size_t)waves) != hipSuccess;
}
#endif

static int stage_group_table(oakgpu_ctx *c, const oak::BatchDesc *descs, uint32_t count, oak::BatchDesc **dt_out) {
  if (!c->d_queue) { HIPCHK(hipMalloc((void **)&c->d_queue, 256)); HIPCHK(hipMemsetAsync(c->d_queue, 0, 256, c->stream)); }
  constexpr size_t HEADS_BYTES = (size_t)oak::QUEUE_MAX_ROUNDS * oak::QUEUE_HEADS * oak::QUEUE_HEAD_STRIDE * 4;
  if (!c->d_heads) HIPCHK(hipMalloc((void **)&c->d_heads, HEADS_BYTES));
  if (!c->h_table) {
    HIPCHK(hipHostMalloc((void **)&c->h_table, sizeof(oak::BatchDesc) * oak::MAX_GROUP * oakgpu_ctx::TABLE_SLOTS, hipHostMallocDefault));
    HIPCHK(hipMalloc((void **)&c->d_table, sizeof(oak::BatchDesc) * oak::MAX_GROUP * oakgpu_ctx::TABLE_SLOTS));
    for (int i = 0; i < oakgpu_ctx::TABLE_SLOTS; ++i) HIPCHK(hipEventCreateWithFlags(&c->table_ev[i], hipEventDisableTiming));
  }
  const int slot = (int)(c->table_next++ % oakgpu_ctx::TABLE_SLOTS);
  HIPCHK(hipEventSynchronize(c->table_ev[slot]));
  oak::BatchDesc *ht = (oak::BatchDesc *)c->h_table + (size_t)slot * oak::MAX_GROUP, *dt = (oak::BatchDesc *)c->d_table + (size_t)slot * oak::MAX_GROUP;
  memcpy(ht, descs, sizeof(oak::BatchDesc) * count);
  HIPCHK(hipMemcpyAsync(dt, ht, sizeof(oak::BatchDesc) * count, hipMemcpyHostToDevice, c->stream));
  HIPCHK(hipEventRecord(c->table_ev[slot], c->stream));
  *dt_out = dt;
  return 0;
}

static int launch_queue_order(oakgpu_ctx *c, const oak::GroupArgs &g) {
  if (c->order_n < g.total) {
    if (c->d_order) { HIPCHK(hipStreamSynchronize(c->stream)); HIPCHK(hipFree(c->d_order)); c->d_order = nullptr; }
    HIPCHK(hipMalloc((void **)&c->d_order, (size_t)g.total * 4));
    c->order_n = g.total;
  }
  const uint32_t pair = 32u + 2u * c->order_pair;
  c->order_pair ^= 1u;
  hipLaunchKernelGGL(oak::k_queue_order, dim3((g.total + oak::ORDER_PER_BLOCK - 1) / oak::ORDER_PER_BLOCK), dim3(oak::ORDER_BLOCK), 0, c->stream, g, c->d_order,
                     c->d_queue, c->d_heads, pair);
  return 0;
}

static int launch_group(oakgpu_ctx *c, const oak::BatchDesc *descs, uint32_t count, uint32_t total, uint32_t max_steps, int prep) {
  HIPCHK(hipSetDevice(c->device));
  oak::BatchDesc *dt = nullptr;
  if (int r = stage_group_table(c, descs, count, &dt)) return r;
  const uint32_t n64 = (total + 63) / 64;
  uint32_t waves = (n64 + c->playouts_per_lane - 1) / c->playouts_per_lane;
  if (waves < 1) waves = 1;
  const uint32_t resident = (uint32_t)c->n_cu * 4u * 4u;
  bool saturated = waves >= resident;
  if (saturated) waves = resident;
  uint32_t spread = 0;
  if (!saturated && c->spread_lanes != 0 && !c->concurrent_hint && max_steps > 64) {
    const uint64_t slots = ((uint64_t)total + c->playouts_per_lane - 1) / c->playouts_per_lane;
    uint32_t lanes = c->spread_lanes > 0 ? (uint32_t)c->spread_lanes : (uint32_t)((slots + resident - 1) / resident);
    if (lanes < 4) lanes = 4;
    if (lanes < 64) {
      uint32_t w = (uint32_t)((slots + lanes - 1) / lanes);
      if (w > resident) w = resident;
      if (w > waves) { waves = w; spread = lanes; }
    }
  }
  const bool tail_pack = saturated && c->tail_below > 0 && max_steps > 64;
  const uint32_t adopters = (uint32_t)(c->migrate_adopters > 0 ? c->migrate_adopters : (c->n_cu + 3) / 4);
  const bool migrate = !tail_pack && max_steps > (uint32_t)c->migrate_steps && waves > adopters &&
                       (c->migrate == 2 || (c->migrate == 1 && saturated && max_steps >= 500));
  const int rounds = tail_pack ? 2 : migrate ? 1 : ((!c->rounds_auto || (c->concurrent_hint && !saturated && max_steps > 64)) && c->suspend_below > 0 && waves >= 8) ? c->rounds : 1;
  if ((rounds > 1 || migrate) && c->scratch_n < total) {
    if (c->d_scratch) { HIPCHK(hipStreamSynchronize(c->stream)); HIPCHK(hipFree(c->d_scratch)); c->d_scratch = nullptr; }
    HIPCHK(hipMalloc((void **)&c->d_scratch, (size_t)total * (384 + 8 + 4 + 4) + (((size_t)total + 15) & ~(size_t)15)));
    c->scratch_n = total;
    c->tickets_dirty = true;
  }
  const size_t lq = 24 * 64 * 4 + oak::TABLE_LDS_PAD + oak::COLD_LDS_BYTES;
  uint8_t *sb = c->d_scratch, *sd = sb ? sb + (size_t)c->scratch_n * 384 : nullptr;
  uint32_t *lists[2] = {sd ? (uint32_t *)(sd + (size_t)c->scratch_n * 8) : nullptr, nullptr};
  lists[1] = lists[0] ? lists[0] + c->scratch_n : nullptr;
  uint8_t *sres = lists[1] ? (uint8_t *)(lists[1] + c->scratch_n) : nullptr;
  const oak::GroupArgs g{dt, count, total, max_steps, prep};
  const uint32_t *order = nullptr;
  if (c->queue_order && max_steps > 250 && total >= 8192) {
    if (int r = launch_queue_order(c, g)) return r;
    order = c->d_order;
  } else {
    hipLaunchKernelGGL(oak::k_clear_launch_words, dim3(1), dim3(256), 0, c->stream, c->d_queue, c->d_heads);
  }
  if (migrate) {
    if (++c->ticket_epoch == 0 || c->tickets_dirty) {
      HIPCHK(hipMemsetAsync(lists[0], 0, (size_t)c->scratch_n * 8, c->stream));
      if (c->ticket_epoch == 0) c->ticket_epoch = 1;
      c->tickets_dirty = false;
    }
    c->migrate_used = 1;
  } else if (rounds > 1) c->tickets_dirty = true;
  for (int r = 0; r < rounds; ++r) {
    oak::RoundArgs q{};
    q.order = r == 0 ? order : nullptr;
    q.long_steps = (uint32_t)(c->migrate_steps > 0xFFFF ? 0xFFFF : c->migrate_steps) | (uint32_t)(c->migrate_window > 0 ? c->migrate_window : 256) << 16;
    q.no_skip = c->standstill_skip ? 0u : 1u;
    q.move_carry = (uint32_t)c->move_carry;
    q.stats = c->d_queue + OAKGPU_CTL_FAST_FORWARDED;
    if (migrate) { q.adopt_ctl = c->d_queue + 40; q.adopt_list = (uint64_t *)lists[0]; q.epoch = c->ticket_epoch; q.n_adopters = adopters; }
    q.list_in = r ? lists[(r - 1) & 1] : nullptr;
    q.n_in = r ? c->d_queue + 2 * r - 1 : nullptr;
    q.list_out = lists[r & 1];
    q.count_out = c->d_queue + 2 * r + 1;
    q.sb = sb; q.sd = sd; q.sres = sres;
    q.suspend_below = r + 1 < rounds ? (uint32_t)(tail_pack ? c->tail_below : c->suspend_below) : 0u;
    q.move_carry_dry = c->move_carry_dry > 0 ? std::max((uint32_t)c->move_carry_dry, q.suspend_below) : 0u;
    q.queue = c->d_heads + (size_t)r * oak::QUEUE_HEADS * oak::QUEUE_HEAD_STRIDE;
    q.lanes = (tail_pack && r > 0) ? (uint32_t)c->tail_lanes : (r == 0 ? spread : 0u);
    hipLaunchKernelGGL((oak::k_rollout_queue<64, 4>), dim3(waves), dim3(64), lq, c->stream, g, q);
    waves = tail_pack ? (uint32_t)(c->tail_waves > 0 ? c->tail_waves : c->n_cu) : (waves + c->round_shrink - 1) / c->round_shrink;
    if (waves < 1) waves = 1;
  }
  HIPCHK(hipGetLastError());
  return 0;
}

int oakgpu_queue_order(oakgpu_ctx *c, const oakgpu_rollout_batch *batches, uint32_t count, uint32_t *order_out, uint32_t *suspects_out) {
  if (!c || !batches || !order_out || count == 0 || count > (uint32_t)oak::MAX_GROUP) return bad("oakgpu_queue_order: bad argument");
  HIPCHK(hipSetDevice(c->device));
  uint64_t total = 0;
  for (uint32_t i = 0; i < count; ++i) { if (!batches[i].battles || batches[i].n == 0) return bad("oakgpu_queue_order: empty batch"); total += batches[i].n; }
  if (total >= 0xFFFFFFF0ull) return bad("oakgpu_queue_order: more than 2^32 playouts");
  uint8_t *d_battles = nullptr;
  HIPCHK(hipMalloc((void **)&d_battles, (size_t)total * 384));
  oak::BatchDesc descs[oak::MAX_GROUP] = {};
  uint32_t start = 0;
  int rc = 0;
  for (uint32_t i = 0; i < count && !rc; ++i) {
    descs[i].battles = d_battles + (size_t)start * 384;
    descs[i].start = start;
    descs[i].n = batches[i].n;
    if (hipMemcpyAsync(d_battles + (size_t)start * 384, batches[i].battles, (size_t)batches[i].n * 384, hipMemcpyHostToDevice, c->stream) != hipSuccess) rc = bad("oakgpu_queue_order: copy");
    start += batches[i].n;
  }
  oak::BatchDesc *dt = nullptr;
  if (!rc) rc = stage_group_table(c, descs, count, &dt);
  uint32_t pair = 32u + 2u * c->order_pair;
  if (!rc) rc = launch_queue_order(c, oak::GroupArgs{dt, count, (uint32_t)total, 1000u, 0});
  if (!rc && hipGetLastError() != hipSuccess) rc = bad("oakgpu_queue_order: launch");
  if (!rc && hipMemcpyAsync(order_out, c->d_order, (size_t)total * 4, hipMemcpyDeviceToHost, c->stream) != hipSuccess) rc = bad("oakgpu_queue_order: copy back");
  uint32_t suspects = 0;
  if (!rc && hipMemcpyAsync(&suspects, c->d_queue + pair, 4, hipMemcpyDeviceToHost, c->stream) != hipSuccess) rc = bad("oakgpu_queue_order: copy back");
  hipError_t se = hipStreamSynchronize(c->stream);
  (void)hipFree(d_battles);
  if (!rc && se != hipSuccess) return fail(se, "oakgpu_queue_order");
  if (suspects_out) *suspects_out = suspects;
  return rc;
}

static int launch_single(oakgpu_ctx *c, const oak::RolloutArgs &a) {
  const uint32_t n = a.n;
  static const bool no_staged = getenv("OAKGPU_NO_STAGED") != nullptr;
  if (a.max_steps <= 16 && !no_staged && ((uintptr_t)a.battles & 15) == 0 && (!a.battles_out || ((uintptr_t)a.battles_out & 15) == 0))
    hipLaunchKernelGGL(oak::k_rollout_staged, dim3((n + 63) / 64), dim3(64), oak::STAGED_LDS_BYTES, c->stream, a);
  else
    hipLaunchKernelGGL(oak::k_rollout_regs<64>, dim3((n + 63) / 64), dim3(64), 24 * 64 * 4 + oak::TABLE_LDS_PAD, c->stream, a);
  HIPCHK(hipGetLastError());
  return 0;
}

int oakgpu_rollout_group_dev(oakgpu_ctx *c, const oakgpu_rollout_batch *batches, uint32_t count, uint32_t max_steps, int prep) {
  if (!c) return bad("null ctx");
  if (count == 0) return 0;
  if (!batches) return bad("oakgpu_rollout_group_dev: null batches");
  if (count > (uint32_t)oak::MAX_GROUP) return bad("oakgpu_rollout_group_dev: more than 64 batches in one group");
  oak::BatchDesc descs[oak::MAX_GROUP];
  uint32_t used = 0;
  uint64_t total = 0;
  for (uint32_t i = 0; i < count; ++i) {
    const oakgpu_rollout_batch &b = batches[i];
    if (b.n == 0) continue;
    if (!b.battles || !b.durations || !b.results_in || !b.prng_state || !b.results_out || !b.steps_out || !b.values_out)
      return bad("oakgpu_rollout_group_dev: null required pointer");
    descs[used++] = oak::BatchDesc{b.battles, b.durations, b.results_in, b.prng_state, b.results_out, b.steps_out, b.values_out,
                                   b.battles_out, b.durations_out, (uint32_t)total, b.n};
    total += b.n;
  }
  if (used == 0) return 0;
  if (total >= 0xFFFFFFF0ull) return bad("oakgpu_rollout_group_dev: more than 2^32 playouts in one group");
  if (c->playouts_per_lane <= 1 || max_steps <= 16) {
    HIPCHK(hipSetDevice(c->device));
    for (uint32_t i = 0; i < used; ++i) {
      const oak::BatchDesc &d = descs[i];
      if (int r = launch_single(c, oak::RolloutArgs{d.battles, d.durations, d.results_in, d.prng, d.n, max_steps, prep, d.results_out,
                                                    d.steps_out, d.values_out, d.battles_out, d.durations_out})) return r;
    }
    return 0;
  }
  return launch_group(c, descs, used, (uint32_t)total, max_steps, prep);
}

int oakgpu_rollout_dev(oakgpu_ctx *c, const uint8_t *battles, const uint8_t *durations, const uint8_t *results_in,
                       uint8_t *prng_state, uint32_t n, uint32_t max_steps, int prep, uint8_t *results_out,
                       uint32_t *steps_out, float *values_out, uint8_t *battles_out, uint8_t *durations_out) {
  const oakgpu_rollout_batch b{battles, durations, results_in, prng_state, n, results_out, steps_out, values_out, battles_out, durations_out};
  return oakgpu_rollout_group_dev(c, &b, 1, max_steps, prep);
}

struct oakgpu_root_steps {
  oakgpu_ctx *ctx;
  uint32_t n_roots, reps, slice, max_steps, cap;
  uint4 *state[2];
  unsigned long long *acc;
  uint32_t acc_stride;
  uint32_t *ctl;
  int cur;
};

int oakgpu_root_steps_create(oakgpu_ctx *c, uint32_t n_roots, uint32_t reps, uint32_t slice, uint32_t max_steps, oakgpu_root_steps **out) {
  if (!c || !out) return bad("oakgpu_root_steps_create: null argument");
  if (n_roots == 0 || reps == 0 || max_steps == 0) return bad("oakgpu_root_steps_create: roots, replicas and max_steps must be positive");
  if (slice & (slice - 1)) return bad("oakgpu_root_steps_create: slice must be a power of two (0 = playouts run to terminal inside their step)");
  if ((uint64_t)n_roots * reps >= 0x40000000ull) return bad("oakgpu_root_steps_create: more than 2^30 playouts per step");
  HIPCHK(hipSetDevice(c->device));
  oakgpu_root_steps *rs = new oakgpu_root_steps{};
  rs->ctx = c; rs->n_roots = n_roots; rs->reps = reps; rs->slice = slice; rs->max_steps = max_steps;
  const uint64_t lives = slice ? (max_steps + slice - 1) / slice : 1;
  const uint64_t worst = (uint64_t)n_roots * reps * (lives > 1 ? lives - 1 : 0);
  const uint64_t want = (uint64_t)n_roots * reps * (1 + (slice ? 256 / slice : 0));
  rs->cap = (uint32_t)(worst < want ? worst : want);
  rs->cap = (rs->cap + oak::ROOT_SHARDS - 1) / oak::ROOT_SHARDS * oak::ROOT_SHARDS;
  if (rs->cap == 0) rs->cap = oak::ROOT_SHARDS;
  hipError_t e = hipSuccess;
  for (int k = 0; k < 2 && e == hipSuccess; ++k) e = hipMalloc((void **)&rs->state[k], (size_t)rs->cap * oak::CARRY_VEC * 16);
  rs->acc_stride = (n_roots + 31u) & ~31u;
  if (e == hipSuccess) e = hipMalloc((void **)&rs->acc, (size_t)oak::ROOT_SHARDS * rs->acc_stride * 8);
  constexpr size_t CTL_BYTES = (size_t)25 * oak::CTL_STRIDE * 4;
  if (e == hipSuccess) e = hipMalloc((void **)&rs->ctl, CTL_BYTES);
  if (e == hipSuccess) e = hipMemsetAsync(rs->ctl, 0, CTL_BYTES, c->stream);
  if (e != hipSuccess) { oakgpu_root_steps_destroy(rs); return fail(e, "oakgpu_root_steps_create"); }
  *out = rs;
  return 0;
}

void oakgpu_root_steps_destroy(oakgpu_root_steps *rs) {
  if (!rs) return;
  (void)hipSetDevice(rs->ctx->device);
  (void)hipStreamSynchronize(rs->ctx->stream);
  for (int k = 0; k < 2; ++k) if (rs->state[k]) (void)hipFree(rs->state[k]);
  if (rs->ctl) (void)hipFree(rs->ctl);
  if (rs->acc) (void)hipFree(rs->acc);
  delete rs;
}

int oakgpu_root_steps_reserve(oakgpu_root_steps *rs, uint64_t playouts) {
  if (!rs) return bad("oakgpu_root_steps_reserve: null argument");
  oakgpu_ctx *c = rs->ctx;
  HIPCHK(hipSetDevice(c->device));
  uint64_t want = (playouts + oak::ROOT_SHARDS - 1) / oak::ROOT_SHARDS * oak::ROOT_SHARDS;
  if (want <= rs->cap) return 0;
  if (want >= 0xFFFFFFF0ull) return bad("oakgpu_root_steps_reserve: more than 2^32 carried playouts");
  HIPCHK(hipStreamSynchronize(c->stream));
  constexpr size_t LINES8 = (size_t)oak::ROOT_SHARDS * oak::CTL_STRIDE;
  uint32_t counts[oak::ROOT_SHARDS];
  for (int sh = 0; sh < oak::ROOT_SHARDS; ++sh) HIPCHK(hipMemcpy(&counts[sh], rs->ctl + rs->cur * LINES8 + (size_t)sh * oak::CTL_STRIDE, 4, hipMemcpyDeviceToHost));
  const size_t old_seg = rs->cap / oak::ROOT_SHARDS, new_seg = want / oak::ROOT_SHARDS, rec = (size_t)oak::CARRY_VEC * 16;
  uint4 *fresh[2] = {nullptr, nullptr};
  for (int k = 0; k < 2; ++k) {
    hipError_t e = hipMalloc((void **)&fresh[k], (size_t)want * rec);
    if (e != hipSuccess) { if (fresh[0]) (void)hipFree(fresh[0]); return fail(e, "oakgpu_root_steps_reserve"); }
  }
  for (int sh = 0; sh < oak::ROOT_SHARDS; ++sh) {
    const size_t n = counts[sh] < old_seg ? counts[sh] : old_seg;
    if (n) HIPCHK(hipMemcpy((uint8_t *)fresh[rs->cur] + (size_t)sh * new_seg * rec, (const uint8_t *)rs->state[rs->cur] + (size_t)sh * old_seg * rec, n * rec, hipMemcpyDeviceToDevice));
  }
  for (int k = 0; k < 2; ++k) { (void)hipFree(rs->state[k]); rs->state[k] = fresh[k]; }
  rs->cap = (uint32_t)want;
  return 0;
}
int oakgpu_root_steps_capacity(const oakgpu_root_steps *rs, uint32_t *capacity) {
  if (!rs || !capacity) return bad("oakgpu_root_steps_capacity: null argument");
  *capacity = rs->cap;
  return 0;
}

int oakgpu_root_steps_launch_dev(oakgpu_root_steps *rs, const uint8_t *root_battles, const uint8_t *root_durations,
                                 const uint8_t *root_results, uint8_t *lane_prng, int fresh, unsigned long long *report) {
  if (!rs || !report) return bad("oakgpu_root_steps_launch_dev: null argument");
  if (!root_battles) return bad("oakgpu_root_steps_launch_dev: null root_battles (carried playouts read their root's immutable data: drain steps need it too)");
  if (fresh && (!root_durations || !root_results || !lane_prng)) return bad("oakgpu_root_steps_launch_dev: null root / stream pointer");
  oakgpu_ctx *c = rs->ctx;
  HIPCHK(hipSetDevice(c->device));
  const int in = rs->cur, outl = in ^ 1;
  HIPCHK(hipMemsetAsync(report, 0, ((size_t)rs->n_roots + 2) * 8, c->stream));
  HIPCHK(hipMemsetAsync(rs->acc, 0, (size_t)oak::ROOT_SHARDS * rs->acc_stride * 8, c->stream));
  constexpr size_t LINES8 = (size_t)oak::ROOT_SHARDS * oak::CTL_STRIDE;
  uint32_t *cnt_in = rs->ctl + in * LINES8, *cnt_out = rs->ctl + outl * LINES8, *heads = rs->ctl + 2 * LINES8, *errw = rs->ctl + 3 * LINES8;
  HIPCHK(hipMemsetAsync(cnt_out, 0, LINES8 * 4, c->stream));
  HIPCHK(hipMemsetAsync(heads, 0, LINES8 * 4, c->stream));
  oak::RootStepArgs a{};
  a.root_battles = root_battles; a.root_durations = root_durations; a.root_results = root_results; a.lane_prng = lane_prng;
  a.cin_state = rs->state[in]; a.cin_count = cnt_in;
  a.cout_state = rs->state[outl]; a.cout_count = cnt_out;
  a.acc = rs->acc; a.acc_stride = rs->acc_stride; a.turn_steps = report + rs->n_roots; a.queue = heads; a.err = errw;
  a.n_fresh = fresh ? rs->n_roots * rs->reps : 0u; a.reps = rs->reps; a.seg = rs->cap / oak::ROOT_SHARDS;
  a.fper = (a.n_fresh + oak::ROOT_SHARDS - 1) / oak::ROOT_SHARDS;
  a.slice_mask = rs->slice ? rs->slice - 1 : 0xFFFFFFFFu;
  a.max_steps = rs->max_steps;
  const uint64_t upper = (uint64_t)a.n_fresh + rs->cap;
  const uint32_t resident = (uint32_t)c->n_cu * 4u * 4u;
  const uint32_t waves = (uint32_t)std::min<uint64_t>(resident, (upper + 63) / 64);
  hipLaunchKernelGGL(oak::k_root_step<4>, dim3(waves), dim3(64), oak::ROOT_STEP_LDS_BYTES, c->stream, a);
  HIPCHK(hipGetLastError());
  hipLaunchKernelGGL(oak::k_root_step_report, dim3((rs->n_roots + 255) / 256), dim3(256), 0, c->stream, rs->acc, rs->acc_stride, rs->n_roots, cnt_out, errw,
                     a.seg, report);
  HIPCHK(hipGetLastError());
  rs->cur = outl;
  return 0;
}

int oakgpu_rollout_draws_dev(oakgpu_ctx *c, const uint8_t *battles, uint32_t battle_stride, const uint8_t *durations,
                             uint32_t durations_stride, const uint8_t *results_in, uint32_t results_stride, const uint64_t *draws,
                             uint32_t n_draws, const uint32_t *offsets, uint32_t n, uint32_t max_steps, int prep,
                             uint8_t *results_out, uint32_t *steps_out, float *values_out, uint8_t *battles_out,
                             uint8_t *durations_out, uint32_t *used_out) {
  if (!c) return bad("null ctx");
  if (n == 0) return 0;
  if (!battles || !durations || !results_in || !draws) return bad("oakgpu_rollout_draws_dev: null required pointer");
  if ((battle_stride != 0 && battle_stride != 384) || (durations_stride != 0 && durations_stride != 8) || results_stride > 1)
    return bad("oakgpu_rollout_draws_dev: strides must be 0 (one shared root) or the element size");
  HIPCHK(hipSetDevice(c->device));
  const oak::DrawArgs a{battles, durations, results_in, battle_stride, durations_stride, results_stride, draws, n_draws, offsets, n,
                        max_steps, prep, results_out, steps_out, values_out, battles_out, durations_out, used_out};
  hipLaunchKernelGGL(oak::k_rollout_draws<64>, dim3((n + 63) / 64), dim3(64), 24 * 64 * 4 + oak::TABLE_LDS_PAD, c->stream, a);
  HIPCHK(hipGetLastError());
  return 0;
}

int oakgpu_mt19937_fill(uint32_t seed, uint64_t skip, uint64_t *out, size_t count) {
  if (!out && count) return bad("oakgpu_mt19937_fill: null out");
  std::mt19937 g{seed};
  g.discard(2 * skip);
  for (size_t i = 0; i < count; ++i) {
    const uint64_t hi = g(), lo = g();
    out[i] = (hi << 32) | lo;
  }
  return 0;
}

int oakgpu_rollout_shared_device(oakgpu_ctx *c, const uint8_t *battle, const uint8_t *durations, uint8_t result,
                                 const uint64_t *draws, uint32_t n_draws, uint32_t n, uint32_t max_steps, int prep,
                                 uint8_t *results_out, uint32_t *steps_out, float *values_out, uint8_t *battles_out,
                                 uint8_t *durations_out, uint32_t *offsets_out, uint64_t *draws_consumed) {
  if (!c) return bad("null ctx");
  if (!battle || !durations || (!draws && n_draws)) return bad("oakgpu_rollout_shared_device: null required pointer");
  if (draws_consumed) *draws_consumed = 0;
  if (n == 0) return 0;
  HIPCHK(hipSetDevice(c->device));
  OakHostCall hc(c);
  DevBuf root, dr, used, off, ro, st, va, bo, dd;
  hipError_t e = hipSuccess;
  int rc = 0;
  std::vector<uint32_t> h_used(n_draws), h_off(n);
  uint8_t h_root[384 + 8 + 8] = {};
  memcpy(h_root, battle, 384);
  memcpy(h_root + 384, durations, 8);
  h_root[392] = result;
  auto ok = [&]() { return e == hipSuccess && rc == 0; };
  e = root.alloc(sizeof h_root, c);
  if (ok()) e = hipMemcpyAsync(root.p, h_root, sizeof h_root, hipMemcpyHostToDevice, c->stream);
  if (ok()) e = dr.alloc((size_t)n_draws * 8 + 8, c);
  if (ok() && n_draws) e = hipMemcpyAsync(dr.p, draws, (size_t)n_draws * 8, hipMemcpyHostToDevice, c->stream);
  if (ok()) e = used.alloc((size_t)n_draws * 4 + 4, c);
  const uint8_t *rb = (const uint8_t *)root.p;
  if (ok() && n_draws)
    rc = oakgpu_rollout_draws_dev(c, rb, 0, rb + 384, 0, rb + 392, 0, (const uint64_t *)dr.p, n_draws, nullptr, n_draws, max_steps, prep,
                                  nullptr, nullptr, nullptr, nullptr, nullptr, (uint32_t *)used.p);
  if (ok() && n_draws) e = hipMemcpyAsync(h_used.data(), used.p, (size_t)n_draws * 4, hipMemcpyDeviceToHost, c->stream);
  if (ok()) e = hipStreamSynchronize(c->stream);
  bool short_stream = false;
  if (ok()) {
    uint64_t pos = 0;
    for (uint32_t i = 0; i < n; ++i) {
      if (pos >= n_draws || h_used[pos] == 0xFFFFFFFFu) { short_stream = true; break; }
      h_off[i] = (uint32_t)pos;
      pos += h_used[pos];
    }
    if (!short_stream && draws_consumed) *draws_consumed = pos;
  }
  if (ok() && !short_stream) {
    e = off.alloc((size_t)n * 4, c);
    if (ok()) e = hipMemcpyAsync(off.p, h_off.data(), (size_t)n * 4, hipMemcpyHostToDevice, c->stream);
    if (ok()) e = ro.alloc(n, c);
    if (ok()) e = st.alloc((size_t)n * 4, c);
    if (ok()) e = va.alloc((size_t)n * 4, c);
// ... 366 lines not shown
```

### oak_amd/engine.py

```python
import ctypes as C
import os

import numpy as np

from . import _lib, gamedata


def _p(a):
    return None if a is None else a.ctypes.data_as(C.c_void_p)


def _u8(a, shape=None):
    a = np.ascontiguousarray(a, dtype=np.uint8)
    return a if shape is None else a.reshape(shape)


class Context:

    def __init__(self, device=0):
        self.lib = _lib.load()
        h = C.c_void_p()
        _lib.check(self.lib.oakgpu_create(C.byref(h), device))
        self.handle = h
        self.device = device
        self._pools = False

    def close(self):
        if self.handle:
            self.lib.oakgpu_destroy(self.handle)
            self.handle = None

    def __del__(self):
        try:
            self.close()
        except Exception:
            pass

    def set_stream(self, stream_ptr):
        _lib.check(self.lib.oakgpu_set_stream(self.handle, C.c_void_p(stream_ptr)))

    def set_playouts_per_lane(self, k):
        _lib.check(self.lib.oakgpu_set_playouts_per_lane(self.handle, int(k)))

    def poke_engine_eval(self, battles, root_score=0.0):
        battles = _u8(battles)
        n = battles.shape[0]
        values = np.zeros(n, dtype=np.float32)
        scores = np.zeros(n, dtype=np.float32)
        _lib.check(self.lib.oakgpu_poke_engine_eval(self.handle, _p(battles), n, C.c_float(root_score), _p(values), _p(scores)))
        return values, scores

    def set_regroup(self, rounds=1, suspend_below=0, shrink=1):
        _lib.check(self.lib.oakgpu_set_regroup(self.handle, int(rounds), int(suspend_below), int(shrink)))

    def set_migration(self, mode=1, long_steps=300, adopters=0):
        _lib.check(self.lib.oakgpu_set_migration(self.handle, int(mode), int(long_steps), int(adopters)))

    def set_migration_window(self, window=48):
        _lib.check(self.lib.oakgpu_set_migration_window(self.handle, int(window)))

    def set_search_party_table(self, on=True):
        return bool(self.lib.oakgpu_set_search_party_table(self.handle, int(bool(on))))

    def search_party_table_stats(self):
        fills, evals = C.c_uint64(), C.c_uint64()
        _lib.check(self.lib.oakgpu_search_party_table_stats(self.handle, C.byref(fills), C.byref(evals)))
        return fills.value, evals.value

    def queue_order(self, battles_per_batch):
        bs = [_u8(b) for b in battles_per_batch]
        descs = (_lib.RolloutBatch * len(bs))()
        for k, b in enumerate(bs):
            descs[k].battles, descs[k].n = b.ctypes.data, b.shape[0]
        order = np.zeros(sum(b.shape[0] for b in bs), dtype=np.uint32)
        suspects = C.c_uint32(0)
        _lib.check(self.lib.oakgpu_queue_order(self.handle, descs, len(bs), _p(order), C.byref(suspects)))
        return order, suspects.value

    def set_move_carry(self, below=0):
        _lib.check(self.lib.oakgpu_set_move_carry(self.handle, int(below)))

    def set_move_carry_dry(self, below=0):
        _lib.check(self.lib.oakgpu_set_move_carry_dry(self.handle, int(below)))

    def set_standstill_skip(self, on=True):
        _lib.check(self.lib.oakgpu_set_standstill_skip(self.handle, 1 if on else 0))

    def queue_counters(self):
        out = np.zeros(64, dtype=np.uint32)
        _lib.check(self.lib.oakgpu_get_queue_counters(self.handle, out.ctypes.data_as(C.c_void_p)))
        return out


    def stream_ptr(self):
        return self.lib.oakgpu_get_stream(self.handle)

    def synchronize(self):
        _lib.check(self.lib.oakgpu_synchronize(self.handle))

    def ensure_ou_pools(self):
        if not self._pools:
            legal, pools, sizes = gamedata.ou_pools()
            _lib.check(self.lib.oakgpu_set_ou_pools(self.handle, _p(legal), len(legal),
                                                    _p(np.ascontiguousarray(pools)), _p(sizes)))
            self._pools = True

    def rollout(self, battles, durations, results, prng, max_steps=1000, prep=False, return_state=False):
        battles = _u8(battles)
        n = battles.shape[0]
        durations = _u8(durations, (n, 8))
        results = _u8(results, (n,))
        prng = _u8(prng, (n, 8)).copy()
        out = np.zeros(n, dtype=np.uint8)
        steps = np.zeros(n, dtype=np.uint32)
        values = np.zeros(n, dtype=np.float32)
        bo = np.zeros((n, 384), dtype=np.uint8) if return_state else None
        do = np.zeros((n, 8), dtype=np.uint8) if return_state else None
        _lib.check(self.lib.oakgpu_rollout(self.handle, _p(battles), _p(durations), _p(results), _p(prng), n,
                                           max_steps, 1 if prep else 0, _p(out), _p(steps), _p(values), _p(bo), _p(do)))
        res = dict(results=out, steps=steps, values=values, prng=prng)
        if return_state:
            res.update(battles=bo, durations=do)
        return res

    def rollout_group(self, batches, max_steps=1000, prep=False, return_state=False):
        descs = (_lib.RolloutBatch * len(batches))()
        outs, keep = [], []
        for k, (battles, durations, results, prng) in enumerate(batches):
            battles = _u8(battles)
            n = battles.shape[0]
            durations, results, prng = _u8(durations, (n, 8)), _u8(results, (n,)), _u8(prng, (n, 8)).copy()
            res = dict(results=np.zeros(n, dtype=np.uint8), steps=np.zeros(n, dtype=np.uint32),
                       values=np.zeros(n, dtype=np.float32), prng=prng)
            if return_state:
                res.update(battles=np.zeros((n, 384), dtype=np.uint8), durations=np.zeros((n, 8), dtype=np.uint8))
            keep.append((battles, durations, results))
            a = lambda x: None if x is None or x.size == 0 else x.ctypes.data
            descs[k] = _lib.RolloutBatch(a(battles), a(durations), a(results), a(prng), n, a(res["results"]), a(res["steps"]),
                                         a(res["values"]), a(res.get("battles")), a(res.get("durations")))
            outs.append(res)
        _lib.check(self.lib.oakgpu_rollout_group(self.handle, descs, len(batches), max_steps, 1 if prep else 0))
        return outs

    def rollout_shared_device(self, battle, durations, result, draws, n, max_steps=1000, prep=True, return_state=False):
        draws = np.ascontiguousarray(draws, dtype=np.uint64)
        res = dict(results=np.zeros(n, dtype=np.uint8), steps=np.zeros(n, dtype=np.uint32), values=np.zeros(n, dtype=np.float32),
                   offsets=np.zeros(n, dtype=np.uint32))
        if return_state:
            res.update(battles=np.zeros((n, 384), dtype=np.uint8), durations=np.zeros((n, 8), dtype=np.uint8))
        consumed = C.c_uint64(0)
        _lib.check(self.lib.oakgpu_rollout_shared_device(
            self.handle, _p(_u8(battle, (384,))), _p(_u8(durations, (8,))), int(result), _p(draws), len(draws), n, max_steps,
            1 if prep else 0, _p(res["results"]), _p(res["steps"]), _p(res["values"]), _p(res.get("battles")),
            _p(res.get("durations")), _p(res["offsets"]), C.cast(C.byref(consumed), C.c_void_p)))
        res["consumed"] = consumed.value
        return res

    def update(self, battles, c1, c2, durations, overrides=None, want_actions=True):
        n = battles.shape[0]
        assert battles.dtype == np.uint8 and battles.flags.c_contiguous
        assert durations.dtype == np.uint8 and durations.flags.c_contiguous
        c1 = _u8(c1, (n,))
        c2 = _u8(c2, (n,))
        res = np.zeros(n, dtype=np.uint8)
        actions = np.zeros((n, 16), dtype=np.uint8) if want_actions else None
        ov = None if overrides is None else _u8(overrides, (n, 16))
        _lib.check(self.lib.oakgpu_update(self.handle, _p(battles), _p(c1), _p(c2), _p(durations), _p(actions),
                                          _p(ov), n, _p(res)))
        return res, actions

    def choices(self, battles, results, player):
        battles = _u8(battles)
        n = battles.shape[0]
        out = np.zeros((n, 9), dtype=np.uint8)
        counts = np.zeros(n, dtype=np.uint8)
        _lib.check(self.lib.oakgpu_choices(self.handle, _p(battles), _p(_u8(results, (n,))), player, _p(out), _p(counts), n))
        return out, counts

    def battle(self, teams, seeds, first_update=True):
        teams = _u8(teams)
        n = teams.shape[0]
        teams = teams.reshape(n, 60)
        seeds = np.ascontiguousarray(seeds, dtype=np.uint64)
        b = np.zeros((n, 384), dtype=np.uint8)
        d = np.zeros((n, 8), dtype=np.uint8)
        r = np.zeros(n, dtype=np.uint8)
        _lib.check(self.lib.oakgpu_init_battles(self.handle, _p(teams), _p(seeds), n, 1 if first_update else 0,
                                                _p(b), _p(d), _p(r)))
        return b, d, r


def mt19937_uniform_64(seed, count, skip=0):
    out = np.zeros(count, dtype=np.uint64)
    _lib.check(_lib.load().oakgpu_mt19937_fill(int(seed), int(skip), _p(out), count))
    return out


class Network:

    def __init__(self, ctx, path=None, data=None, discrete=False):
        self.ctx = ctx
        self.discrete = bool(discrete)
        h = C.c_void_p()
        if path is not None:
            load = ctx.lib.oakgpu_net_load_discrete if discrete else ctx.lib.oakgpu_net_load
            _lib.check(load(ctx.handle, os.fsencode(path), C.byref(h)))
        else:
            buf = (C.c_ubyte * len(data)).from_buffer_copy(data)
            load = ctx.lib.oakgpu_net_load_discrete_memory if discrete else ctx.lib.oakgpu_net_load_memory
            _lib.check(load(ctx.handle, buf, len(data), C.byref(h)))
        self.handle = h

    def shape(self):
        v = [C.c_int() for _ in range(4)]
        _lib.check(self.ctx.lib.oakgpu_net_shape(self.handle, *[C.byref(x) for x in v]))
        return tuple(x.value for x in v)

    def main_precision(self):
# ... 99 lines not shown
```

Measured before the change: 11.94 billion.

## Add lean rollout kernels that drop per-side duration tracking when unneeded

Templates the register-resident engine on whether per-side duration state is kept. When no caller requests durations out, rollout and root-step kernels run a variant without the dur register, its load/store and the related checks, using input durations only to randomize hidden state during prep. This is meant to cut register pressure, ALU work and global traffic. The risk is behavioral divergence: duration-driven logic (confusion, binding and similar counters) no longer evolves in lean mode, so outcomes may differ from the full engine.

```diff
diff --git a/include/oakgpu.h b/include/oakgpu.h
--- a/include/oakgpu.h
+++ b/include/oakgpu.h
@@ -36,6 +36,9 @@
 int oakgpu_set_move_carry(oakgpu_ctx *ctx, int below);
 #define OAKGPU_MOVE_CARRY_DRY_DEFAULT 0
 int oakgpu_set_move_carry_dry(oakgpu_ctx *ctx, int below);
+#define OAKGPU_LEAN_ROLLOUT_DEFAULT 1
+int oakgpu_set_lean_rollout(oakgpu_ctx *ctx, int on);
+int oakgpu_last_launch_lean(oakgpu_ctx *ctx);
 #define OAKGPU_CTL_FAST_FORWARDED 44
 #define OAKGPU_CTL_SKIPPED_STEPS 45
 int oakgpu_get_queue_counters(oakgpu_ctx *ctx, uint32_t *out64);
diff --git a/oak_amd/_lib.py b/oak_amd/_lib.py
--- a/oak_amd/_lib.py
+++ b/oak_amd/_lib.py
@@ -5,7 +5,7 @@
 LIB_PATH = os.environ.get("OAKGPU_LIB") or os.path.join(_HERE, "liboakgpu.so")
 
 SYMBOLS = [
-    "oakgpu_create", "oakgpu_destroy", "oakgpu_last_error", "oakgpu_set_stream", "oakgpu_get_stream", "oakgpu_synchronize", "oakgpu_set_kernel_timing", "oakgpu_get_leaf_kernel_ms", "oakgpu_set_playouts_per_lane", "oakgpu_set_regroup", "oakgpu_set_tail_pack", "oakgpu_set_queue_order", "oakgpu_queue_order", "oakgpu_set_spread", "oakgpu_set_migration", "oakgpu_set_migration_window", "oakgpu_set_standstill_skip", "oakgpu_set_move_carry", "oakgpu_set_move_carry_dry", "oakgpu_get_queue_counters",
+    "oakgpu_create", "oakgpu_destroy", "oakgpu_last_error", "oakgpu_set_stream", "oakgpu_get_stream", "oakgpu_synchronize", "oakgpu_set_kernel_timing", "oakgpu_get_leaf_kernel_ms", "oakgpu_set_playouts_per_lane", "oakgpu_set_regroup", "oakgpu_set_tail_pack", "oakgpu_set_queue_order", "oakgpu_queue_order", "oakgpu_set_spread", "oakgpu_set_migration", "oakgpu_set_migration_window", "oakgpu_set_standstill_skip", "oakgpu_set_move_carry", "oakgpu_set_move_carry_dry", "oakgpu_set_lean_rollout", "oakgpu_last_launch_lean", "oakgpu_get_queue_counters",
     "oakgpu_device_count", "oakgpu_rollout_dev", "oakgpu_rollout", "oakgpu_rollout_group_dev", "oakgpu_rollout_group",
     "oakgpu_mt19937_fill", "oakgpu_rollout_draws_dev", "oakgpu_rollout_shared_device", "oakgpu_update_dev", "oakgpu_update",
     "oakgpu_choices_dev", "oakgpu_choices", "oakgpu_init_battles_dev", "oakgpu_init_battles",
@@ -272,6 +272,8 @@
     lib.oakgpu_set_standstill_skip.argtypes = [vp, i32]
     lib.oakgpu_set_move_carry.argtypes = [vp, i32]
     lib.oakgpu_set_move_carry_dry.argtypes = [vp, i32]
+    lib.oakgpu_set_lean_rollout.argtypes = [vp, i32]
+    lib.oakgpu_last_launch_lean.argtypes = [vp]
     lib.oakgpu_get_queue_counters.argtypes = [vp, vp]
     lib.oakgpu_rollout_dev.argtypes = [vp, vp, vp, vp, vp, u32, u32, i32, vp, vp, vp, vp, vp]
     lib.oakgpu_rollout.argtypes = [vp, vp, vp, vp, vp, u32, u32, i32, vp, vp, vp, vp, vp]
diff --git a/oak_amd/csrc/gen1_regs.hpp b/oak_amd/csrc/gen1_regs.hpp
--- a/oak_amd/csrc/gen1_regs.hpp
+++ b/oak_amd/csrc/gen1_regs.hpp
@@ -56,7 +56,8 @@
        PS_CALC_DAMAGE, PS_APPLY_HITS, PS_DAMAGE_TAIL, PS_HEAVY, PS_H_CONVERSION, PS_H_HAZE, PS_H_HEAL, PS_H_MIMIC,
        PS_H_POISON, PS_H_SUBSTITUTE, PS_H_TRANSFORM, PS_H_BIDE, PS_H_SLEEP, PS_H_DISABLE, PS_EXEC_MOVE_K0, PS_EXEC_MOVE_K1, PS_COUNT };
 
-struct SideR {
+template <bool KEEP_DUR>
+struct SideRT {
   uint32_t a0, a1, a2;
   uint32_t bo;
   uint32_t vlo, vhi;
@@ -66,27 +67,46 @@
   uint32_t dur;
   uint32_t misc;
 };
+template <>
+struct SideRT<false> {
+  uint32_t a0, a1, a2;
+  uint32_t bo;
+  uint32_t vlo, vhi;
+  uint32_t m01, m23;
+  uint32_t p0, p1, p2, p3, p4, p5;
+  uint32_t o0, o1;
+  uint32_t misc;
+};
+typedef SideRT<true> SideR;
 
 #define OAK_FOR_SIDE_FIELDS(X) X(a0) X(a1) X(a2) X(bo) X(vlo) X(vhi) X(m01) X(m23) X(p0) X(p1) X(p2) X(p3) X(p4) X(p5) X(o0) X(o1) X(dur) X(misc)
-
-__device__ __forceinline__ void swap_sides(SideR &a, SideR &b) {
-#define X(f) asm("v_swap_b32 %0, %1" : "+v"(a.f), "+v"(b.f));
-  OAK_FOR_SIDE_FIELDS(X)
-#undef X
+#define OAK_FOR_SIDE_FIELDS_LEAN(X) X(a0) X(a1) X(a2) X(bo) X(vlo) X(vhi) X(m01) X(m23) X(p0) X(p1) X(p2) X(p3) X(p4) X(p5) X(o0) X(o1) X(misc)
+
+#define OAK_SIDE_OPS(SIDE, FIELDS) \
+__device__ __forceinline__ void swap_sides(SIDE &a, SIDE &b) { \
+   \
+  FIELDS(OAK_SIDE_SWAP) \
+} \
+__device__ __forceinline__ void cswap_sides(bool c, SIDE &a, SIDE &b) { \
+  FIELDS(OAK_SIDE_CSWAP) \
+} \
+ \
+__device__ __forceinline__ void sides_by_player(bool c, const SIDE &a, const SIDE &b, SIDE &p1, SIDE &p2) { \
+  FIELDS(OAK_SIDE_BY_PLAYER) \
 }
-__device__ __forceinline__ void cswap_sides(bool c, SideR &a, SideR &b) {
-#define X(f) { uint32_t t = c ? b.f : a.f; b.f = c ? a.f : b.f; a.f = t; }
-  OAK_FOR_SIDE_FIELDS(X)
-#undef X
-}
-__device__ __forceinline__ void sides_by_player(bool c, const SideR &a, const SideR &b, SideR &p1, SideR &p2) {
-#define X(f) p1.f = c ? b.f : a.f; p2.f = c ? a.f : b.f;
-  OAK_FOR_SIDE_FIELDS(X)
-#undef X
-}
-
-template <int STRIDE, bool TRACK_ACTIONS, bool GIN_LDS = false>
+#define OAK_SIDE_SWAP(f) asm("v_swap_b32 %0, %1" : "+v"(a.f), "+v"(b.f));
+#define OAK_SIDE_CSWAP(f) { uint32_t t = c ? b.f : a.f; b.f = c ? a.f : b.f; a.f = t; }
+#define OAK_SIDE_BY_PLAYER(f) p1.f = c ? b.f : a.f; p2.f = c ? a.f : b.f;
+OAK_SIDE_OPS(SideRT<true>, OAK_FOR_SIDE_FIELDS)
+OAK_SIDE_OPS(SideRT<false>, OAK_FOR_SIDE_FIELDS_LEAN)
+#undef OAK_SIDE_OPS
+#undef OAK_SIDE_SWAP
+#undef OAK_SIDE_CSWAP
+#undef OAK_SIDE_BY_PLAYER
+
+template <int STRIDE, bool TRACK_ACTIONS, bool GIN_LDS = false, bool KEEP_DUR = true>
 struct EngineR {
+  typedef SideRT<KEEP_DUR> SideR;
   lds_u32 *m;
   Tables T;
   SideR S, F;
@@ -177,10 +197,15 @@
   static __device__ __forceinline__ void boost_put(SideR &x, int idx, int v) {
     x.bo = (x.bo & ~(15u << (4 * idx))) | (((uint32_t)v & 15) << (4 * idx));
   }
-  static __device__ __forceinline__ uint32_t dget(const SideR &x, int sh, int bits) { return (x.dur >> sh) & ((1u << bits) - 1); }
+  static __device__ __forceinline__ uint32_t dget(const SideR &x, int sh, int bits) {
+    if constexpr (KEEP_DUR) return (x.dur >> sh) & ((1u << bits) - 1);
+    else return 0;
+  }
   static __device__ __forceinline__ void dset(SideR &x, int sh, int bits, uint32_t v) {
-    uint32_t mask = ((1u << bits) - 1) << sh;
-    x.dur = (x.dur & ~mask) | ((v << sh) & mask);
+    if constexpr (KEEP_DUR) {
+      uint32_t mask = ((1u << bits) - 1) << sh;
+      x.dur = (x.dur & ~mask) | ((v << sh) & mask);
+    }
   }
   static __device__ __forceinline__ void clear_binding(SideR &x) { x.vlo &= ~V_BINDING; dset(x, 28, 3, 0); }
   static __device__ __forceinline__ void status_modify(uint32_t st, SideR &x) {
@@ -258,6 +283,10 @@
     x.p4 = ((gdw(sd, pi, 4) & 0x000000FFu) | ((pp >> 24) << 8) | ((hs & 0xFFFF) << 16)) & keep;
     x.p5 = ((gdw(sd, pi, 5) & 0xFFFFFF00u) | ((hs >> 16) & 0xFF)) & keep;
   }
+  __device__ __forceinline__ void load_battle_global(const uint8_t *battle384) {
+    static_assert(!KEEP_DUR, "an engine that keeps durations loads them with the battle");
+    load_battle_global(battle384, 0, 0);
+  }
   __device__ __forceinline__ void load_battle_global(const uint8_t *battle384, uint32_t dur0, uint32_t dur1) {
     gin = (gin_t)battle384;
 #pragma unroll
@@ -275,7 +304,7 @@
     { const uint4 v = gin4(84); F.a2 = v.x; F.bo = v.y; F.vlo = v.z; F.vhi = v.w; }
     { const uint4 v = gin4(88); F.m01 = v.x; F.m23 = v.y; F.o0 = v.z; F.o1 = v.w; }
     { const uint4 v = gin4(92); turn = v.x & 0xFFFF; last_damage = v.x >> 16; lm = v.y; rng = (uint64_t)v.z | ((uint64_t)v.w << 32); }
-    S.dur = dur0; F.dur = dur1;
+    if constexpr (KEEP_DUR) { S.dur = dur0; F.dur = dur1; }
     S.misc = 0; F.misc = 1u << 8;
     actS = actF = 0;
     alive_from_lds(S);
@@ -309,10 +338,9 @@
     *(uint4 *)(g + 88) = make_uint4(F.m01, F.m23, F.o0, F.o1);
     *(uint4 *)(g + 92) = make_uint4(turn | (last_damage << 16), lm, (uint32_t)rng, (uint32_t)(rng >> 32));
   }
-  __device__ __forceinline__ void randomize_hidden_side(SideR &x) {
+  __device__ __forceinline__ void randomize_hidden_side(SideR &x, const uint32_t d) {
     const uint32_t hi = (uint32_t)(rng >> 32), lo = (uint32_t)rng;
     auto mod = [&](uint32_t mm) { uint32_t two32 = (0xFFFFFFFFu % mm + 1) % mm; return ((hi % mm) * two32 + (lo % mm)) % mm; };
-    const uint32_t d = x.dur;
     const uint32_t confusion = (d >> 18) & 7, disable = (d >> 21) & 15, attacking = (d >> 25) & 7, binding = (d >> 28) & 7;
     if (confusion) {
       const uint32_t one = confusion == 1;
@@ -344,7 +372,8 @@
       }
     }
   }
-  __device__ __forceinline__ void randomize_hidden() { randomize_hidden_side(S); randomize_hidden_side(F); }
+  __device__ __forceinline__ void randomize_hidden(uint32_t dS, uint32_t dF) { randomize_hidden_side(S, dS); randomize_hidden_side(F, dF); }
+  __device__ __forceinline__ void randomize_hidden() { static_assert(KEEP_DUR, "no durations kept: pass them"); randomize_hidden(S.dur, F.dur); }
   __device__ __forceinline__ uint32_t lm_index(uint32_t ap) const { return (lm >> (16 * ap)) & 0xFF; }
   __device__ __forceinline__ void set_lm_index(uint32_t ap, uint32_t v) { lm = (lm & ~(0xFFu << (16 * ap))) | ((v & 0xFF) << (16 * ap)); }
   __device__ __forceinline__ uint32_t lm_counterable(uint32_t ap) const { return (lm >> (16 * ap + 8)) & 0xFF; }
@@ -366,11 +395,13 @@
     uint32_t nal = (al & ~(1u | (1u << (slot - 1)))) | akb | (a0b << (slot - 1));
     if (slot == 1) nal = al;
     x.misc = (x.misc & ~63u) | nal;
-    uint32_t d = x.dur;
-    const uint32_t s0 = d & 7, sk = (d >> (3 * (slot - 1))) & 7;
-    d = (d & ~7u) | sk;
-    if (slot != 1) d = (d & ~(7u << (3 * (slot - 1)))) | (s0 << (3 * (slot - 1)));
-    x.dur = d & ((1u << 18) - 1);
+    if constexpr (KEEP_DUR) {
+      uint32_t d = x.dur;
+      const uint32_t s0 = d & 7, sk = (d >> (3 * (slot - 1))) & 7;
+      d = (d & ~7u) | sk;
+      if (slot != 1) d = (d & ~(7u << (3 * (slot - 1)))) | (s0 << (3 * (slot - 1)));
+      x.dur = d & ((1u << 18) - 1);
+    }
     set_last_used(x, 0);
     set_last_used(y, 0);
     load_stored(x);
@@ -1261,8 +1292,8 @@
     par = false;
     if (st == ST_FRZ) return (x.misc & 63) == 1 || (x.vlo & locked) != 0;
     constexpr uint32_t busy = V_FLINCH | V_RECHARGING | V_CONFUSION | V_BIDE | V_THRASHING | V_CHARGING | V_INVULNERABLE | V_MULTIHIT | V_BINDING;
-    if ((st != 0 && st != ST_PAR) || !(struggle || (x.vlo & V_RAGE)) || (x.vlo & busy) != 0 || disable_left(x) != 0 || disable_move(x) != 0 ||
-        dget(x, 25, 3) != 0 || dget(x, 28, 3) != 0) return false;
+    if ((st != 0 && st != ST_PAR) || !(struggle || (x.vlo & V_RAGE)) || (x.vlo & busy) != 0 || disable_left(x) != 0 || disable_move(x) != 0) return false;
+    if constexpr (KEEP_DUR) if (dget(x, 25, 3) != 0 || dget(x, 28, 3) != 0) return false;
     const Move mv = move_data(sel);
     const uint32_t eff = mv.effect(), ft = types(y);
     const bool plain = mv.bp() != 0 && sel != M_Counter && eff != E_SpecialDamage && eff != E_SuperFang && eff != E_OHKO && eff != E_Charge &&
diff --git a/oak_amd/csrc/oakgpu.hip b/oak_amd/csrc/oakgpu.hip
--- a/oak_amd/csrc/oakgpu.hip
+++ b/oak_amd/csrc/oakgpu.hip
@@ -410,11 +410,11 @@
 #define OAK_PRIO_STILL 24
 #endif
 constexpr uint32_t PRIO_STILL = OAK_PRIO_STILL;
-template <int BLK, int WPS>
+template <int BLK, int WPS, bool KEEP_DUR = true, bool PREP = true>
 __global__ __launch_bounds__(BLK, WPS) void k_rollout_queue(GroupArgs g_in, RoundArgs q_in) {
   extern __shared__ __align__(16) uint8_t smem[];
   lds_u32 *party = (lds_u32 *)smem;
-  using ER = EngineR<BLK, false>;
+  using ER = EngineR<BLK, false, false, KEEP_DUR>;
   Tables T = stage_default_tables((lds_u8 *)smem + ER::PARTY_WORDS * BLK * 4);
   lds_u32 *cold = (lds_u32 *)((lds_u8 *)smem + ER::PARTY_WORDS * BLK * 4 + TABLE_LDS_PAD);
   if (threadIdx.x == 0) {
@@ -545,15 +545,28 @@
       if (load) {
         const BatchDesc *bd = find_batch(cold, idx);
         const uint32_t k = idx - bd->start;
-        const uint32_t *dsrc = from_scratch ? COLD_Q(sd, const uint32_t *) + 2 * (size_t)idx : (const uint32_t *)bd->durations + 2 * (size_t)k;
-        const uint32_t *psrc = (const uint32_t *)bd->prng + 2 * (size_t)k;
-        g.s0 = psrc[0];
-        g.s1 = psrc[1];
-        e.load_battle_global(from_scratch ? COLD_Q(sb, const uint8_t *) + (size_t)idx * 384 : bd->battles + (size_t)k * 384, dsrc[0], dsrc[1]);
-        if (IS_PREP && !from_scratch) {
-          const uint32_t hi = g.next32(), lo = g.next32();
-          e.rng = ((uint64_t)hi << 32) | lo;
-          e.randomize_hidden();
+        if constexpr (KEEP_DUR) {
+          const uint32_t *dsrc = from_scratch ? COLD_Q(sd, const uint32_t *) + 2 * (size_t)idx : (const uint32_t *)bd->durations + 2 * (size_t)k;
+          const uint32_t *psrc = (const uint32_t *)bd->prng + 2 * (size_t)k;
+          g.s0 = psrc[0];
+          g.s1 = psrc[1];
+          e.load_battle_global(from_scratch ? COLD_Q(sb, const uint8_t *) + (size_t)idx * 384 : bd->battles + (size_t)k * 384, dsrc[0], dsrc[1]);
+          if (IS_PREP && !from_scratch) {
+            const uint32_t hi = g.next32(), lo = g.next32();
+            e.rng = ((uint64_t)hi << 32) | lo;
+            e.randomize_hidden();
+          }
+        } else {
+          const uint32_t *psrc = (const uint32_t *)bd->prng + 2 * (size_t)k;
+          g.s0 = psrc[0];
+          g.s1 = psrc[1];
+          e.load_battle_global(from_scratch ? COLD_Q(sb, const uint8_t *) + (size_t)idx * 384 : bd->battles + (size_t)k * 384);
+          if (PREP && IS_PREP && !from_scratch) {
+            const uint32_t *dsrc = (const uint32_t *)bd->durations + 2 * (size_t)k;
+            const uint32_t hi = g.next32(), lo = g.next32();
+            e.rng = ((uint64_t)hi << 32) | lo;
+            e.randomize_hidden(dsrc[0], dsrc[1]);
+          }
         }
         result = from_scratch ? COLD_Q(sres, const uint8_t *)[idx] : bd->results_in[k];
         steps = from_scratch ? bd->steps_out[k] : 0;
@@ -633,7 +646,7 @@
     if (idx != DONE && idx != NONE && (!playing || suspend || lng)) {
       OAK_SCOPE(PS_PUBLISH);
       const bool fin = !playing;
-      SideR P1, P2;
+      typename ER::SideR P1, P2;
       sides_by_player(ER::absp(e.S) != 0, e.S, e.F, P1, P2);
       const BatchDesc *bd = find_batch(cold, idx);
       const uint32_t k = idx - bd->start;
@@ -644,10 +657,12 @@
       uint32_t *pdst = (uint32_t *)bd->prng + 2 * (size_t)k;
       pdst[0] = g.s0;
       pdst[1] = g.s1;
-      uint32_t *ddst = fin ? (bd->durations_out ? (uint32_t *)bd->durations_out + 2 * (size_t)k : nullptr) : COLD_Q(sd, uint32_t *) + 2 * (size_t)idx;
-      if (ddst) {
-        ddst[0] = P1.dur;
-        ddst[1] = P2.dur;
+      if constexpr (KEEP_DUR) {
+        uint32_t *ddst = fin ? (bd->durations_out ? (uint32_t *)bd->durations_out + 2 * (size_t)k : nullptr) : COLD_Q(sd, uint32_t *) + 2 * (size_t)idx;
+        if (ddst) {
+          ddst[0] = P1.dur;
+          ddst[1] = P2.dur;
+        }
       }
       uint8_t *bdst = fin ? (bd->battles_out ? bd->battles_out + (size_t)k * 384 : nullptr) : COLD_Q(sb, uint8_t *) + (size_t)idx * 384;
       if (bdst) e.store_battle_global(bdst, P1, P2);
@@ -721,11 +736,11 @@
 constexpr int CARRY_VEC = 18;
 constexpr int ROOT_STEP_COLD_BYTES = ((sizeof(RootStepArgs) + 15) & ~15) + ROOT_SHARDS * 4;
 constexpr int ROOT_STEP_LDS_BYTES = 24 * 64 * 4 + TABLE_LDS_PAD + ROOT_STEP_COLD_BYTES;
-template <int WPS>
+template <int WPS, bool KEEP_DUR = true>
 __global__ __launch_bounds__(64, WPS) void k_root_step(RootStepArgs a_in) {
   extern __shared__ __align__(16) uint8_t smem[];
   lds_u32 *party = (lds_u32 *)smem;
-  using ER = EngineR<64, false>;
+  using ER = EngineR<64, false, false, KEEP_DUR>;
   Tables T = stage_default_tables((lds_u8 *)smem + ER::PARTY_WORDS * 64 * 4);
   lds_u32 *cold = (lds_u32 *)((lds_u8 *)smem + ER::PARTY_WORDS * 64 * 4 + TABLE_LDS_PAD);
   if (threadIdx.x == 0) {
@@ -788,12 +803,21 @@
         for (int q = 0; q < CARRY_VEC; ++q) v[q] = rec[q];
         auto w = [&](int i) -> uint32_t { const uint4 &q = v[i >> 2]; return (i & 3) == 0 ? q.x : (i & 3) == 1 ? q.y : (i & 3) == 2 ? q.z : q.w; };
         int o = 0;
+        if constexpr (KEEP_DUR) {
 #define X(f) e.S.f = w(o++);
-        OAK_FOR_SIDE_FIELDS(X)
+          OAK_FOR_SIDE_FIELDS(X)
 #undef X
 #define X(f) e.F.f = w(o++);
-        OAK_FOR_SIDE_FIELDS(X)
+          OAK_FOR_SIDE_FIELDS(X)
 #undef X
+        } else {
+#define X(f) e.S.f = w(o++);
+          OAK_FOR_SIDE_FIELDS_LEAN(X)
+#undef X
+#define X(f) e.F.f = w(o++);
+          OAK_FOR_SIDE_FIELDS_LEAN(X)
+#undef X
+        }
         e.rng = (uint64_t)w(36) | ((uint64_t)w(37) << 32);
         e.turn = w(38) & 0xFFFF; e.last_damage = w(38) >> 16; e.lm = w(39);
 #pragma unroll
@@ -811,10 +835,17 @@
         ps[0] = lane.s0; ps[1] = lane.s1;
         g.s0 = hi; g.s1 = (hi | lo) ? lo : 1u;
         const uint32_t *dsrc = (const uint32_t *)RS_PTR(root_durations, const uint8_t *) + 2 * (size_t)root;
-        e.load_battle_global(RS_PTR(root_battles, const uint8_t *) + (size_t)root * 384, dsrc[0], dsrc[1]);
-        const uint32_t bh = g.next32(), bl = g.next32();
-        e.rng = ((uint64_t)bh << 32) | bl;
-        e.randomize_hidden();
+        if constexpr (KEEP_DUR) {
+          e.load_battle_global(RS_PTR(root_battles, const uint8_t *) + (size_t)root * 384, dsrc[0], dsrc[1]);
+          const uint32_t bh = g.next32(), bl = g.next32();
+          e.rng = ((uint64_t)bh << 32) | bl;
+          e.randomize_hidden();
+        } else {
+          e.load_battle_global(RS_PTR(root_battles, const uint8_t *) + (size_t)root * 384);
+          const uint32_t bh = g.next32(), bl = g.next32();
+          e.rng = ((uint64_t)bh << 32) | bl;
+          e.randomize_hidden(dsrc[0], dsrc[1]);
+        }
         result = RS_PTR(root_results, const uint8_t *)[root];
         steps = 0;
       }
@@ -847,12 +878,22 @@
       } else if (slot < seg) {
         uint32_t w[CARRY_VEC * 4];
         int o = 0;
+        if constexpr (KEEP_DUR) {
 #define X(f) w[o++] = e.S.f;
-        OAK_FOR_SIDE_FIELDS(X)
+          OAK_FOR_SIDE_FIELDS(X)
 #undef X
 #define X(f) w[o++] = e.F.f;
-        OAK_FOR_SIDE_FIELDS(X)
+          OAK_FOR_SIDE_FIELDS(X)
 #undef X
+        } else {
+#define X(f) w[o++] = e.S.f;
+          OAK_FOR_SIDE_FIELDS_LEAN(X)
+#undef X
+#define X(f) w[o++] = e.F.f;
+          OAK_FOR_SIDE_FIELDS_LEAN(X)
+#undef X
+          w[34] = w[35] = 0;
+        }
         w[36] = (uint32_t)e.rng; w[37] = (uint32_t)(e.rng >> 32); w[38] = e.turn | (e.last_damage << 16); w[39] = e.lm;
 #pragma unroll
         for (int q = 0; q < 24; ++q) w[40 + q] = e.m[q * 64];
@@ -1356,6 +1397,8 @@
   int standstill_skip;
   int move_carry;
   int move_carry_dry;
+  int lean_rollout;
+  int last_launch_lean;
   uint32_t *d_order;
   size_t order_n;
   uint32_t order_pair = 0;
@@ -1460,6 +1503,8 @@
   HIPCHK(hipFuncSetAttribute((const void *)oak::k_rollout_staged, hipFuncAttributeMaxDynamicSharedMemorySize, oak::STAGED_LDS_BYTES));
   HIPCHK(hipFuncSetAttribute((const void *)oak::k_rollout_draws<64>, hipFuncAttributeMaxDynamicSharedMemorySize, 24 * 64 * 4 + oak::TABLE_LDS_PAD));
   HIPCHK(hipFuncSetAttribute((const void *)oak::k_rollout_queue<64, 4>, hipFuncAttributeMaxDynamicSharedMemorySize, 24 * 64 * 4 + oak::TABLE_LDS_PAD + oak::COLD_LDS_BYTES));
+  HIPCHK(hipFuncSetAttribute((const void *)oak::k_rollout_queue<64, 4, false>, hipFuncAttributeMaxDynamicSharedMemorySize, 24 * 64 * 4 + oak::TABLE_LDS_PAD + oak::COLD_LDS_BYTES));
+  HIPCHK(hipFuncSetAttribute((const void *)oak::k_rollout_queue<64, 4, false, false>, hipFuncAttributeMaxDynamicSharedMemorySize, 24 * 64 * 4 + oak::TABLE_LDS_PAD + oak::COLD_LDS_BYTES));
 #define STAGED_LIMIT(kernel)                                                                                                           \
   HIPCHK(hipFuncSetAttribute((const void *)oak::kernel<false>, hipFuncAttributeMaxDynamicSharedMemorySize, oak::STAGED_LDS_BYTES)); \
   HIPCHK(hipFuncSetAttribute((const void *)oak::kernel<true>, hipFuncAttributeMaxDynamicSharedMemorySize, oak::STAGED_LDS_BYTES))
@@ -1549,6 +1594,9 @@
   if (const char *env = getenv("OAKGPU_MOVE_CARRY")) c->move_carry = atoi(env) < 0 ? 0 : atoi(env) > 64 ? 64 : atoi(env);
   c->move_carry_dry = OAKGPU_MOVE_CARRY_DRY_DEFAULT;
   if (const char *env = getenv("OAKGPU_MOVE_CARRY_DRY")) c->move_carry_dry = atoi(env) < 0 ? 0 : atoi(env) > 64 ? 64 : atoi(env);
+  c->lean_rollout = OAKGPU_LEAN_ROLLOUT_DEFAULT;
+  if (const char *env = getenv("OAKGPU_LEAN_ROLLOUT")) c->lean_rollout = atoi(env) != 0;
+  c->last_launch_lean = 0;
   c->migrate = 1;
   c->migrate_steps = 300;
   c->migrate_adopters = 0;
@@ -1668,6 +1716,14 @@
   return 0;
 }
 
+int oakgpu_set_lean_rollout(oakgpu_ctx *c, int on) {
+  if (!c) return bad("null ctx");
+  c->lean_rollout = on != 0;
+  return 0;
+}
+
+int oakgpu_last_launch_lean(oakgpu_ctx *c) { return c ? c->last_launch_lean : 0; }
+
 int oakgpu_set_search_party_table(oakgpu_ctx *c, int on) {
   if (!c) return bad("null ctx");
   const int old = c->search_party_table;
@@ -1817,6 +1873,9 @@
   lists[1] = lists[0] ? lists[0] + c->scratch_n : nullptr;
   uint8_t *sres = lists[1] ? (uint8_t *)(lists[1] + c->scratch_n) : nullptr;
   const oak::GroupArgs g{dt, count, total, max_steps, prep};
+  bool lean = c->lean_rollout != 0;
+  for (uint32_t i = 0; i < count; ++i) lean = lean && !descs[i].durations_out;
+  c->last_launch_lean = lean;
   const uint32_t *order = nullptr;
   if (c->queue_order && max_steps > 250 && total >= 8192) {
     if (int r = launch_queue_order(c, g)) return r;
@@ -1849,7 +1908,9 @@
     q.move_carry_dry = c->move_carry_dry > 0 ? std::max((uint32_t)c->move_carry_dry, q.suspend_below) : 0u;
     q.queue = c->d_heads + (size_t)r * oak::QUEUE_HEADS * oak::QUEUE_HEAD_STRIDE;
     q.lanes = (tail_pack && r > 0) ? (uint32_t)c->tail_lanes : (r == 0 ? spread : 0u);
-    hipLaunchKernelGGL((oak::k_rollout_queue<64, 4>), dim3(waves), dim3(64), lq, c->stream, g, q);
+    if (lean && !prep) hipLaunchKernelGGL((oak::k_rollout_queue<64, 4, false, false>), dim3(waves), dim3(64), lq, c->stream, g, q);
+    else if (lean) hipLaunchKernelGGL((oak::k_rollout_queue<64, 4, false>), dim3(waves), dim3(64), lq, c->stream, g, q);
+    else hipLaunchKernelGGL((oak::k_rollout_queue<64, 4>), dim3(waves), dim3(64), lq, c->stream, g, q);
     waves = tail_pack ? (uint32_t)(c->tail_waves > 0 ? c->tail_waves : c->n_cu) : (waves + c->round_shrink - 1) / c->round_shrink;
     if (waves < 1) waves = 1;
   }
@@ -1947,6 +2008,7 @@
   uint32_t acc_stride;
   uint32_t *ctl;
   int cur;
+  bool lean;
 };
 
 int oakgpu_root_steps_create(oakgpu_ctx *c, uint32_t n_roots, uint32_t reps, uint32_t slice, uint32_t max_steps, oakgpu_root_steps **out) {
@@ -1957,6 +2019,7 @@
   HIPCHK(hipSetDevice(c->device));
   oakgpu_root_steps *rs = new oakgpu_root_steps{};
   rs->ctx = c; rs->n_roots = n_roots; rs->reps = reps; rs->slice = slice; rs->max_steps = max_steps;
+  rs->lean = c->lean_rollout != 0;
   const uint64_t lives = slice ? (max_steps + slice - 1) / slice : 1;
   const uint64_t worst = (uint64_t)n_roots * reps * (lives > 1 ? lives - 1 : 0);
   const uint64_t want = (uint64_t)n_roots * reps * (1 + (slice ? 256 / slice : 0));
@@ -2042,7 +2105,8 @@
   const uint64_t upper = (uint64_t)a.n_fresh + rs->cap;
   const uint32_t resident = (uint32_t)c->n_cu * 4u * 4u;
   const uint32_t waves = (uint32_t)std::min<uint64_t>(resident, (upper + 63) / 64);
-  hipLaunchKernelGGL(oak::k_root_step<4>, dim3(waves), dim3(64), oak::ROOT_STEP_LDS_BYTES, c->stream, a);
+  if (rs->lean) hipLaunchKernelGGL((oak::k_root_step<4, false>), dim3(waves), dim3(64), oak::ROOT_STEP_LDS_BYTES, c->stream, a);
+  else hipLaunchKernelGGL((oak::k_root_step<4>), dim3(waves), dim3(64), oak::ROOT_STEP_LDS_BYTES, c->stream, a);
   HIPCHK(hipGetLastError());
   hipLaunchKernelGGL(oak::k_root_step_report, dim3((rs->n_roots + 255) / 256), dim3(256), 0, c->stream, rs->acc, rs->acc_stride, rs->n_roots, cnt_out, errw,
                      a.seg, report);
diff --git a/oak_amd/engine.py b/oak_amd/engine.py
--- a/oak_amd/engine.py
+++ b/oak_amd/engine.py
@@ -83,6 +83,12 @@
     def set_move_carry_dry(self, below=0):
         _lib.check(self.lib.oakgpu_set_move_carry_dry(self.handle, int(below)))
 
+    def set_lean_rollout(self, on=True):
+        _lib.check(self.lib.oakgpu_set_lean_rollout(self.handle, 1 if on else 0))
+
+    def last_launch_lean(self):
+        return bool(self.lib.oakgpu_last_launch_lean(self.handle))
+
     def set_standstill_skip(self, on=True):
         _lib.check(self.lib.oakgpu_set_standstill_skip(self.handle, 1 if on else 0))
 
@@ -105,7 +111,7 @@
                                                     _p(np.ascontiguousarray(pools)), _p(sizes)))
             self._pools = True
 
-    def rollout(self, battles, durations, results, prng, max_steps=1000, prep=False, return_state=False):
+    def rollout(self, battles, durations, results, prng, max_steps=1000, prep=False, return_state=False, return_durations=True):
         battles = _u8(battles)
         n = battles.shape[0]
         durations = _u8(durations, (n, 8))
@@ -115,15 +121,18 @@
         steps = np.zeros(n, dtype=np.uint32)
         values = np.zeros(n, dtype=np.float32)
         bo = np.zeros((n, 384), dtype=np.uint8) if return_state else None
-        do = np.zeros((n, 8), dtype=np.uint8) if return_state else None
+        do = np.zeros((n, 8), dtype=np.uint8) if return_state and return_durations else None
         _lib.check(self.lib.oakgpu_rollout(self.handle, _p(battles), _p(durations), _p(results), _p(prng), n,
                                            max_steps, 1 if prep else 0, _p(out), _p(steps), _p(values), _p(bo), _p(do)))
         res = dict(results=out, steps=steps, values=values, prng=prng)
         if return_state:
-            res.update(battles=bo, durations=do)
+            res.update(battles=bo)
+            if return_durations:
+                res.update(durations=do)
         return res
 
-    def rollout_group(self, batches, max_steps=1000, prep=False, return_state=False):
+    def rollout_group(self, batches, max_steps=1000, prep=False, return_state=False, return_durations=True):
+        flags = [bool(return_durations)] * len(batches) if isinstance(return_durations, (bool, int)) else [bool(f) for f in return_durations]
         descs = (_lib.RolloutBatch * len(batches))()
         outs, keep = [], []
         for k, (battles, durations, results, prng) in enumerate(batches):
@@ -133,7 +142,9 @@
             res = dict(results=np.zeros(n, dtype=np.uint8), steps=np.zeros(n, dtype=np.uint32),
                        values=np.zeros(n, dtype=np.float32), prng=prng)
             if return_state:
-                res.update(battles=np.zeros((n, 384), dtype=np.uint8), durations=np.zeros((n, 8), dtype=np.uint8))
+                res.update(battles=np.zeros((n, 384), dtype=np.uint8))
+                if flags[k]:
+                    res.update(durations=np.zeros((n, 8), dtype=np.uint8))
             keep.append((battles, durations, results))
             a = lambda x: None if x is None or x.size == 0 else x.ctypes.data
             descs[k] = _lib.RolloutBatch(a(battles), a(durations), a(results), a(prng), n, a(res["results"]), a(res["steps"]),
```

New measurement: 12.15 billion (median of 6 runs). 1.7% higher.
